# fnothaft/adam

Hardware: AMD Instinct MI355X
Metric: BQSR bases/sec (observe+apply) at 1/2/4/8 MI355X; % HBM roofline (higher is better)
Workload: dtype u8 in, int64 counts, f64 recalibration; 1 GPU; cfg2: synthetic 10M x 100 bp reads, 1 read group, no known sites (per GPU); reads_per_gpu=10000000, bases_per_gpu=1000000000, reads_total=10000000, read_groups=1, known_sites=0, parallelism=dp1: read shards per GPU, RCCL int64 table all-reduce

## Files before the change

adam_amd/_capi.py:

```python
from __future__ import annotations

import ctypes
import os
import threading

_HERE = os.path.dirname(os.path.abspath(__file__))
LIB_PATH = os.environ.get("ADAM_BQSR_LIB") or os.path.join(_HERE, "libadam_bqsr.so")

BQSR_OK = 0
STAGE_RESET, STAGE_KERNEL, STAGE_FOLD, STAGE_PREP, STAGE_LUT, STAGE_NO_LUT = 1, 2, 4, 8, 16, 32
STATUS_NAMES = ["OK", "NULL_RG", "MD_PARSE", "CIGAR_SHORT", "BAD_REVCOMP_BASE", "EMPTY_TABLE", "MISSING_KEY",
                "QUAL_RANGE", "NULL_FIELD", "SEQ_SHORT", "CIGAR_INVALID", "INVALID_ARG", "DEVICE", "UNSUPPORTED",
                "SAM_PARSE", "PILEUP", "ATTRIBUTE"]
(NULL_RG, MD_PARSE, CIGAR_SHORT, BAD_REVCOMP_BASE, EMPTY_TABLE, MISSING_KEY, QUAL_RANGE, NULL_FIELD, SEQ_SHORT,
 CIGAR_INVALID, INVALID_ARG, DEVICE, UNSUPPORTED, SAM_PARSE, PILEUP, ATTRIBUTE) = range(1, 17)

EXPORTS = [
    "bqsr_abi_version", "bqsr_last_error", "bqsr_last_error_read", "bqsr_status_name", "bqsr_context_create",
    "bqsr_context_destroy", "bqsr_context_tune", "bqsr_sites_create", "bqsr_sites_destroy", "bqsr_batch_create", "bqsr_batch_destroy",
    "bqsr_batch_reads", "bqsr_batch_bases", "bqsr_batch_dims", "bqsr_batch_relayout", "bqsr_batch_layout_times", "bqsr_batch_wrap_device", "bqsr_table_words",
    "bqsr_table_create", "bqsr_table_destroy", "bqsr_table_dims", "bqsr_table_device_ptr", "bqsr_table_download",
    "bqsr_table_upload", "bqsr_observe", "bqsr_observe_records", "bqsr_table_merge", "bqsr_finalize",
    "bqsr_lut_destroy", "bqsr_lut_stats", "bqsr_lut_shifts", "bqsr_apply", "bqsr_apply_records",
    "bqsr_stage_records", "bqsr_staged_destroy", "bqsr_staged_bytes", "bqsr_staged_reads", "bqsr_staged_bases",
    "bqsr_batch_create_staged", "bqsr_batch_upload_async", "bqsr_em_fold_async", "bqsr_batch_em_copy_async",
    "bqsr_finalize_device", "bqsr_observe_stage", "bqsr_apply_stage", "bqsr_job_reset_async", "bqsr_job_result", "bqsr_copy_async",
    "bqsr_job_errors_export_async", "bqsr_job_errors_import_async", "bqsr_job_status_async", "bqsr_job_status_get",
    "bqsr_copy_dyn_async", "bqsr_compact_outputs_async", "bqsr_batch_exception_count_ptr",
    "bqsr_sort_order", "bqsr_sam_sort",
    "bqsr_sam_flagstat", "bqsr_flagstat_arrow", "bqsr_flagstat_arrow_device",
    "bqsr_bgzf_inflate", "bqsr_sam_bam_form", "bqsr_sam_markdup_path",
    "bqsr_sam_pileup_prepare", "bqsr_sam_pileup_columns", "bqsr_arrow_pileup_prepare", "bqsr_arrow_pileup_columns",
    "bqsr_pileup_kernel_times",
    "bqsr_pileup_agg_create", "bqsr_pileup_agg_destroy", "bqsr_pileup_agg_add_host", "bqsr_sam_pileup_agg_add",
    "bqsr_arrow_pileup_agg_add", "bqsr_pileup_agg_run", "bqsr_pileup_agg_fetch", "bqsr_pileup_agg_kernel_times",
    "bqsr_sam_bam_prepare", "bqsr_sam_bam_records", "bqsr_sam_bam_header", "bqsr_bgzf_compress",
    "bqsr_bam_kernel_times",
    "bqsr_bgzf_deflate", "bqsr_bgzf_deflate_host", "bqsr_sam_bam_members", "bqsr_deflate_code_lengths",
    "bqsr_bgzf_deflate_times",
    "bqsr_compare_create", "bqsr_compare_destroy", "bqsr_compare_check_terms", "bqsr_compare_sam", "bqsr_compare_sides",
    "bqsr_compare_values", "bqsr_compare_baseqs", "bqsr_compare_rows", "bqsr_compare_kernel_times",
    "bqsr_sam_tag_counts", "bqsr_arrow_tag_counts", "bqsr_sam_tag_values", "bqsr_arrow_tag_values",
    "bqsr_tag_values_fetch", "bqsr_tags_kernel_times",
]


class NativeLibraryMissing(RuntimeError):
    pass


class BQSRError(RuntimeError):

    def __init__(self, status: int, message: str = "", read: int = -1):
        name = STATUS_NAMES[status] if 0 <= status < len(STATUS_NAMES) else str(status)
        super().__init__("%s: %s" % (name, message))
        self.status = status
        self.name = name
        self.read = read


class Dims(ctypes.Structure):
    _fields_ = [("n_rg", ctypes.c_int32), ("max_len", ctypes.c_int32)]


class FinalStats(ctypes.Structure):
    _fields_ = [("average_reported_error", ctypes.c_double), ("global_error", ctypes.c_double),
                ("global_obs", ctypes.c_int64), ("global_mm", ctypes.c_int64), ("n_groups", ctypes.c_int32)]


class DeviceReads(ctypes.Structure):
    _fields_ = [("n_reads", ctypes.c_int64), ("n_slots", ctypes.c_int64), ("meta", ctypes.c_void_p),
                ("align", ctypes.c_void_p), ("qual", ctypes.c_void_p), ("bases", ctypes.c_void_p),
                ("cigar", ctypes.c_void_p), ("md", ctypes.c_void_p), ("dims", Dims),
                ("slots_aligned", ctypes.c_int32)]


_lib = None
_lock = threading.Lock()


def lib():
    global _lib
    if _lib is not None:
        return _lib
    with _lock:
        if _lib is not None:
            return _lib
        if not os.path.exists(LIB_PATH):
            raise NativeLibraryMissing("%s is not built; run __graft_entry__.build()" % LIB_PATH)
        try:
            import torch
            if torch.cuda.is_available():
                torch.cuda.init()
        except ImportError:
            pass
        L = ctypes.CDLL(LIB_PATH)
        vp, i32, i64, dbl = ctypes.c_void_p, ctypes.c_int32, ctypes.c_int64, ctypes.c_double
        pp = ctypes.POINTER(ctypes.c_void_p)
        sig = {
            "bqsr_abi_version": (ctypes.c_int, []),
            "bqsr_last_error": (ctypes.c_char_p, []),
            "bqsr_last_error_read": (i64, []),
            "bqsr_status_name": (ctypes.c_char_p, [ctypes.c_int]),
            "bqsr_context_create": (ctypes.c_int, [ctypes.c_int, pp]),
            "bqsr_context_destroy": (None, [vp]),
            "bqsr_context_tune": (ctypes.c_int, [vp, ctypes.c_int, i64]),
            "bqsr_batch_relayout": (ctypes.c_int, [vp, vp, ctypes.POINTER(dbl)]),
            "bqsr_batch_layout_times": (ctypes.c_int, [vp, ctypes.POINTER(dbl), ctypes.POINTER(dbl)]),
            "bqsr_sites_create": (ctypes.c_int, [vp, vp, vp, vp, i32, pp]),
            "bqsr_sites_destroy": (None, [vp]),
            "bqsr_batch_create": (ctypes.c_int, [vp, vp, vp, pp]),
            "bqsr_batch_destroy": (None, [vp]),
            "bqsr_batch_reads": (i64, [vp]),
            "bqsr_batch_bases": (i64, [vp]),
            "bqsr_batch_slots": (i64, [vp]),
            "bqsr_batch_dims": (Dims, [vp]),
            "bqsr_batch_wrap_device": (ctypes.c_int, [vp, ctypes.POINTER(DeviceReads), pp]),
            "bqsr_stage_records": (ctypes.c_int, [vp, vp, pp]),
            "bqsr_staged_destroy": (None, [vp]),
            "bqsr_staged_bytes": (i64, [vp]),
            "bqsr_staged_reads": (i64, [vp]),
            "bqsr_staged_bases": (i64, [vp]),
            "bqsr_batch_create_staged": (ctypes.c_int, [vp, vp, pp]),
            "bqsr_batch_upload_async": (ctypes.c_int, [vp, vp, vp]),
            "bqsr_batch_set_window": (ctypes.c_int, [vp, i32, i32]),
            "bqsr_batch_reads_per_tile": (i32, [vp]),
            "bqsr_table_words": (i64, [Dims]),
            "bqsr_table_create": (ctypes.c_int, [vp, Dims, vp, pp]),
            "bqsr_table_destroy": (None, [vp]),
            "bqsr_table_dims": (Dims, [vp]),
            "bqsr_table_device_ptr": (vp, [vp]),
            "bqsr_table_download": (ctypes.c_int, [vp, vp]),
            "bqsr_table_upload": (ctypes.c_int, [vp, vp]),
            "bqsr_observe": (ctypes.c_int, [vp, vp, vp, vp, ctypes.POINTER(dbl), vp]),
            "bqsr_observe_async": (ctypes.c_int, [vp, vp, vp, vp, vp]),
            "bqsr_observe_result": (ctypes.c_int, [vp, ctypes.POINTER(dbl), vp]),
            "bqsr_observe_stage": (ctypes.c_int, [vp, vp, vp, vp, i32, vp]),
            "bqsr_table_zero_async": (ctypes.c_int, [vp, vp]),
            "bqsr_batch_em_device_ptr": (vp, [vp]),
            "bqsr_apply_stage": (ctypes.c_int, [vp, vp, vp, vp, vp, vp, vp, i64, i32, vp]),
            "bqsr_observe_records": (ctypes.c_int, [vp, vp, vp, Dims, pp, ctypes.POINTER(dbl)]),
            "bqsr_table_merge": (ctypes.c_int, [vp, vp, ctypes.POINTER(dbl), dbl]),
            "bqsr_finalize": (ctypes.c_int, [vp, vp, dbl, pp]),
            "bqsr_finalize_async": (ctypes.c_int, [vp, vp, dbl, pp, vp]),
            "bqsr_finalize_result": (ctypes.c_int, [vp, vp]),
            "bqsr_finalize_device": (ctypes.c_int, [vp, vp, vp, pp, vp]),
            "bqsr_batch_em_copy_async": (ctypes.c_int, [vp, vp, vp]),
            "bqsr_em_fold_async": (ctypes.c_int, [vp, vp, i64, vp, vp]),
            "bqsr_lut_destroy": (None, [vp]),
            "bqsr_lut_stats": (ctypes.c_int, [vp, ctypes.POINTER(FinalStats)]),
            "bqsr_lut_group": (ctypes.c_int, [vp, i32, ctypes.POINTER(i64), ctypes.POINTER(i64)]),
            "bqsr_lut_shifts": (ctypes.c_int, [vp, i32, i32, i32, i32, vp, ctypes.POINTER(i32)]),
            "bqsr_phred_threshold_table": (i32, [vp, i32, ctypes.POINTER(i32)]),
            "bqsr_apply": (ctypes.c_int, [vp, vp, vp, vp, vp, vp, vp, i64, ctypes.POINTER(i64), vp]),
            "bqsr_apply_async": (ctypes.c_int, [vp, vp, vp, vp, vp, vp, vp, i64, vp]),
            "bqsr_apply_result": (ctypes.c_int, [vp, ctypes.POINTER(i64), vp]),
            "bqsr_apply_records": (ctypes.c_int, [vp, vp, vp, vp, vp]),
            "bqsr_job_reset_async": (ctypes.c_int, [vp, vp, vp]),
            "bqsr_job_result": (ctypes.c_int, [vp, vp, ctypes.POINTER(dbl), ctypes.POINTER(i64), vp]),
            "bqsr_copy_async": (ctypes.c_int, [vp, vp, vp, i64, vp]),
            "bqsr_copy_dyn_async": (ctypes.c_int, [vp, vp, vp, vp, i32, i64, i64, vp]),
            "bqsr_compact_outputs_async": (ctypes.c_int, [vp, vp, vp, vp, vp, vp, i64, vp, vp, vp, vp]),
            "bqsr_batch_exception_count_ptr": (vp, [vp]),
            "bqsr_job_errors_export_async": (ctypes.c_int, [vp, i64, vp, vp]),
            "bqsr_job_errors_import_async": (ctypes.c_int, [vp, vp, vp]),
            "bqsr_job_status_async": (ctypes.c_int, [vp, vp, i32, vp]),
            "bqsr_job_status_get": (ctypes.c_int, [vp, i32, i32, ctypes.POINTER(dbl), ctypes.POINTER(i64)]),
        }
        for name, (res, args) in sig.items():
            f = getattr(L, name)
            f.restype = res
            f.argtypes = args
        _lib = L
    return _lib


def check(status: int):
    if status != BQSR_OK:
        L = lib()
        raise BQSRError(status, L.bqsr_last_error().decode(), L.bqsr_last_error_read())
```

adam_amd/bqsr.py:

```python
from __future__ import annotations

import contextlib
import ctypes
from typing import Dict, Iterable, List, Optional, Sequence, Tuple

import numpy as np

from . import _capi
from ._capi import BQSRError, Dims, check, lib
from .records import (F_DUPLICATE, F_HAS_MD, F_MAPPED, F_PRIMARY, ADAMRecord, RecordBatch)

MAX_REASONABLE_QSCORE = 60


class Context:

    _by_device: Dict[int, "Context"] = {}

    def __init__(self, device: int = 0):
        h = ctypes.c_void_p()
        check(lib().bqsr_context_create(device, ctypes.byref(h)))
        self.handle = h
        self.device = device

    @classmethod
    def get(cls, device: int = 0) -> "Context":
        if device not in cls._by_device:
            cls._by_device[device] = Context(device)
        return cls._by_device[device]

    _KNOBS = {"order": 1, "fronts": 2, "key_major": 3, "bgzf": 5, "flagstat_grid": 6, "pileup_grid": 7}
    _DEFAULTS = {"order": -1, "fronts": -1, "key_major": 0, "bgzf": 1, "flagstat_grid": 0, "pileup_grid": 0}

    def tune(self, **knobs) -> Dict[str, int]:
        cur = getattr(self, "_tuned", dict(self._DEFAULTS))
        prev = {}
        for k, v in knobs.items():
            if v is None:
                continue
            if isinstance(v, str):
                v = {"auto": -1, "read": 0, "group": 1}[v]
            check(lib().bqsr_context_tune(self.handle, self._KNOBS[k], int(v)))
            prev[k] = cur[k]
            cur[k] = int(v)
        self._tuned = cur
        return prev

    @contextlib.contextmanager
    def tuned(self, **knobs):
        prev = self.tune(**knobs)
        try:
            yield self
        finally:
            self.tune(**prev)


class SnpTable:

    def __init__(self, table: Optional[Dict[str, Iterable[int]]] = None):
        self.table = {k: np.unique(np.asarray(list(v), dtype=np.int64)) for k, v in (table or {}).items()}
        self._handles: Dict[int, ctypes.c_void_p] = {}

    @property
    def contigs(self) -> List[str]:
        return list(self.table.keys())

    @staticmethod
    def from_vcf(path: str) -> "SnpTable":
        t: Dict[str, List[int]] = {}
        with open(path, "r", encoding="latin-1") as fh:
            for line in fh:
                line = line.rstrip("\n")
                if line.startswith("#"):
                    continue
                f = line.split("\t")
                t.setdefault(f[0], []).append(int(f[1]))
        return SnpTable(t)

    def handle(self, ctx: Context):
        if ctx.device not in self._handles:
            names = [c.encode() for c in self.contigs]
            arrs = [np.ascontiguousarray(self.table[c]) for c in self.contigs]
            n = len(arrs)
            cnames = (ctypes.c_char_p * max(1, n))(*names)
            cpos = (ctypes.c_void_p * max(1, n))(*[a.ctypes.data for a in arrs])
            cn = np.asarray([len(a) for a in arrs] or [0], dtype=np.uint64)
            h = ctypes.c_void_p()
            check(lib().bqsr_sites_create(ctx.handle, ctypes.cast(cnames, ctypes.c_void_p),
                                          ctypes.cast(cpos, ctypes.c_void_p), cn.ctypes.data, n, ctypes.byref(h)))
            self._handles[ctx.device] = h
        return self._handles[ctx.device]

    def __del__(self):
        L = _capi._lib
        if L is not None:
            for h in getattr(self, "_handles", {}).values():
                L.bqsr_sites_destroy(h)


def dims_of(batches: Sequence[RecordBatch]) -> Dims:
    n_rg = max([b.n_rg() for b in batches] or [1])
    max_len = max([b.max_len() for b in batches] or [1])
    return Dims(n_rg, max_len)


class ErrorCount:

    def __init__(self, bases_observed: int = 0, mismatches: int = 0):
        self.bases_observed = int(bases_observed)
        self.mismatches = int(mismatches)

    def __add__(self, other: "ErrorCount") -> "ErrorCount":
        return ErrorCount(self.bases_observed + other.bases_observed, self.mismatches + other.mismatches)

    def get_error_prob(self) -> Optional[float]:
        if self.bases_observed == 0:
            return None
        return max(10.0 ** (-60 / 10.0), self.mismatches / self.bases_observed)

    def __repr__(self):
        return "ErrorCount(%d, %d)" % (self.bases_observed, self.mismatches)


class RecalTable:

    def __init__(self, dims: Dims, ctx: Optional[Context] = None, expected_mismatch: float = 0.0):
        self.ctx = ctx or Context.get()
        self.dims = Dims(dims.n_rg, dims.max_len)
        h = ctypes.c_void_p()
        check(lib().bqsr_table_create(self.ctx.handle, self.dims, None, ctypes.byref(h)))
        self.handle = h
        self.expected_mismatch = float(expected_mismatch)

    def __del__(self):
        L = _capi._lib
        if L is not None and getattr(self, "handle", None):
            L.bqsr_table_destroy(self.handle)
            self.handle = None

    @property
    def K(self) -> int:
        return 60 * (self.dims.n_rg - 1) + 128

    @property
    def C(self) -> int:
        return 2 * self.dims.max_len + 1

    @property
    def cells(self) -> int:
        return self.C + 21

    def words(self) -> np.ndarray:
        w = np.zeros(lib().bqsr_table_words(self.dims), dtype=np.int64)
        check(lib().bqsr_table_download(self.handle, w.ctypes.data))
        return w

    def set_words(self, w: np.ndarray):
        w = np.ascontiguousarray(w, dtype=np.int64)
        check(lib().bqsr_table_upload(self.handle, w.ctypes.data))

    def counts(self) -> Tuple[np.ndarray, np.ndarray, np.ndarray]:
        w = self.words()
        K, cells = self.K, self.cells
        return w[:K], w[K:K + K * cells].reshape(K, cells), w[K + K * cells:].reshape(K, cells)

    def merge(self, other: "RecalTable") -> "RecalTable":
        out = RecalTable(self.dims, self.ctx)
        out.set_words(self.words())
        em = ctypes.c_double(self.expected_mismatch)
        check(lib().bqsr_table_merge(out.handle, other.handle, ctypes.byref(em), other.expected_mismatch))
        out.expected_mismatch = em.value
        return out

    def merge_into(self, other: "RecalTable"):
        em = ctypes.c_double(self.expected_mismatch)
        check(lib().bqsr_table_merge(self.handle, other.handle, ctypes.byref(em), other.expected_mismatch))
        self.expected_mismatch = em.value

    def finalize_table(self) -> "FinalizedTable":
        return FinalizedTable(self)


class FinalizedTable:

    def __init__(self, table: RecalTable):
        self.table = table
        h = ctypes.c_void_p()
        check(lib().bqsr_finalize(table.ctx.handle, table.handle, table.expected_mismatch, ctypes.byref(h)))
        self.handle = h
        st = _capi.FinalStats()
        check(lib().bqsr_lut_stats(h, ctypes.byref(st)))
        self.average_reported_error = st.average_reported_error
        self.global_error = st.global_error
        self.global_counts = ErrorCount(st.global_obs, st.global_mm)

    def __del__(self):
        L = _capi._lib
        if L is not None and getattr(self, "handle", None):
            L.bqsr_lut_destroy(self.handle)
            self.handle = None

    def read_group_counts(self, r: int) -> Optional[ErrorCount]:
        o, m = ctypes.c_int64(), ctypes.c_int64()
        k = lib().bqsr_lut_group(self.handle, r, ctypes.byref(o), ctypes.byref(m))
        if k < 0:
            check(_capi.DEVICE)
        return ErrorCount(o.value, m.value) if k == 1 else None

    def get_error_rate_shifts(self, qual_by_rg: int, qual: int, cycle: int, context: int):
        sh = np.zeros(4, dtype=np.float64)
        q = ctypes.c_int32()
        check(lib().bqsr_lut_shifts(self.handle, qual_by_rg, qual, cycle, context, sh.ctypes.data, ctypes.byref(q)))
        return sh, q.value

    def get_read_group_delta(self, qual_by_rg: int) -> float:
        num = qual_by_rg - 1
        r = num // MAX_REASONABLE_QSCORE if num >= 0 else -((-num) // MAX_REASONABLE_QSCORE)
        ec = self.read_group_counts(r)
        if ec is None:
            raise BQSRError(_capi.MISSING_KEY, "read group %d" % r)
        p = ec.get_error_prob()
        avg = self.average_reported_error
        return (p if p is not None else avg) - avg


class Partition:

    def __init__(self, batch: RecordBatch, chars: np.ndarray, out_len: np.ndarray):
        self.batch = batch
        self.chars = chars
        self.out_len = out_len

    def qual(self, r: int) -> str:
        o = int(self.batch.qual_offset[r])
        return "".join(map(chr, self.chars[o:o + int(self.out_len[r])]))

    def records(self) -> List[ADAMRecord]:
        recs = self.batch.to_records()
        for r, rec in enumerate(recs):
            if rec.qual is not None or self.out_len[r]:
                rec.qual = self.qual(r)
        return recs


class RecalibrateBaseQualities:

    def __init__(self, ctx: Optional[Context] = None, dims: Optional[Dims] = None):
        self.ctx = ctx or Context.get()
        self.dims = dims

    @staticmethod
    def usable_read(rec: ADAMRecord) -> bool:
        return rec.read_mapped and rec.primary_alignment and not rec.duplicate_read and \
            rec.mismatching_positions is not None

    @classmethod
    def apply(cls, partitions: Sequence[RecordBatch], dbsnp: Optional[SnpTable] = None,
              ctx: Optional[Context] = None) -> List[Partition]:
        parts = list(partitions)
        rbq = cls(ctx, dims_of(parts))
        table = rbq.compute_table(parts, dbsnp or SnpTable())
        return rbq.apply_table(table, parts)

    def _records(self, batch: RecordBatch, dbsnp: Optional[SnpTable]):
        return batch.c_struct(batch.contig_ids_for(dbsnp.contigs if dbsnp else None))

    def compute_table(self, partitions: Sequence[RecordBatch], dbsnp: SnpTable) -> RecalTable:
        dims = self.dims or dims_of(partitions)
        acc = RecalTable(dims, self.ctx)
        sites = dbsnp.handle(self.ctx) if dbsnp is not None else None
        for batch in partitions:
            s, keep = self._records(batch, dbsnp)
            h = ctypes.c_void_p()
            em = ctypes.c_double(0.0)
            check(lib().bqsr_observe_records(self.ctx.handle, ctypes.byref(s), sites, dims, ctypes.byref(h),
                                             ctypes.byref(em)))
            part = RecalTable.__new__(RecalTable)
            part.ctx, part.dims, part.handle, part.expected_mismatch = self.ctx, dims, h, em.value
            acc.merge_into(part)
        return acc

    def apply_table(self, table: RecalTable, partitions: Sequence[RecordBatch]) -> List[Partition]:
        fin = table.finalize_table()
        out = []
        for batch in partitions:
            s, keep = self._records(batch, None)
            chars = np.zeros(max(1, int(batch.qual_offset[-1])), dtype=np.uint16)
            out_len = np.zeros(max(1, batch.n_reads), dtype=np.uint32)
            check(lib().bqsr_apply_records(self.ctx.handle, ctypes.byref(s), fin.handle, chars.ctypes.data,
                                           out_len.ctypes.data))
            out.append(Partition(batch, chars, out_len))
        return out


def adam_bqsr(partitions: Sequence[RecordBatch], dbsnp: Optional[SnpTable] = None,
              ctx: Optional[Context] = None) -> List[Partition]:
    return RecalibrateBaseQualities.apply(partitions, dbsnp, ctx)
```

adam_amd/csrc/bqsr_capi.cpp:

```cpp
#include <hip/hip_runtime.h>

#include <algorithm>
#include <array>
#include <atomic>
#include <chrono>
#include <cmath>
#include <cstdio>
#include <cstdlib>
#include <cstring>
#include <dlfcn.h>
#include <memory>
#include <mutex>
#include <new>
#include <string>
#include <thread>
#include <vector>

#include <rocprim/rocprim.hpp>

#include "bqsr_internal.h"

using namespace bqsr;

#include "bqsr_kernels.hip"
#include "bqsr_observe_lean.hip"
#include "bqsr_fold.hip"
#include "bqsr_transport.hip"


namespace {
thread_local std::string g_err;
thread_local int64_t g_err_read = -1;

bqsr_status fail(bqsr_status s, const std::string& msg, int64_t read = -1) {
  g_err = msg;
  g_err_read = read;
  return s;
}
bqsr_status ok() {
  g_err.clear();
  g_err_read = -1;
  return BQSR_OK;
}

#define HIP_TRY(expr)                                                                          \
  do {                                                                                         \
    hipError_t e_ = (expr);                                                                    \
    if (e_ != hipSuccess)                                                                      \
      return fail(BQSR_ERR_DEVICE, std::string(#expr " failed: ") + hipGetErrorString(e_));    \
  } while (0)

hipStream_t S(void* s) { return s ? (hipStream_t)s : hipStreamPerThread; }

const char* kStatusNames[] = {"OK",          "NULL_RG",      "MD_PARSE",       "CIGAR_SHORT", "BAD_REVCOMP_BASE",
                              "EMPTY_TABLE", "MISSING_KEY",  "QUAL_RANGE",     "NULL_FIELD",  "SEQ_SHORT",
                              "CIGAR_INVALID", "INVALID_ARG", "DEVICE",        "UNSUPPORTED", "SAM_PARSE",
                              "PILEUP",      "ATTRIBUTE"};

bqsr_status from_err_key(unsigned long long k, int64_t read_base) {
  if (k == kNoError) return ok();
  const int code = (int)(k & 0xF);
  const int64_t read = (int64_t)(k >> 28) + read_base;
  const uint32_t o = (uint32_t)((k >> 8) & 0xFFFFF);
  char buf[160];
  snprintf(buf, sizeof buf, "%s at read %lld, read offset %u", kStatusNames[code], (long long)read, o);
  return fail((bqsr_status)code, buf, read);
}


struct Pow10 {
  double v[256];
  Pow10() {
    for (int p = 0; p < 256; ++p) v[p] = std::pow(10.0, (double)(-p) / 10.0);
  }
};
const Pow10& pow10tab() {
  static Pow10 t;
  return t;
}

double cr_log10(double x) { return (double)log10l((long double)x); }
int32_t java_d2i(double d) {
  if (std::isnan(d)) return 0;
  if (d >= 2147483647.0) return INT32_MAX;
  if (d <= -2147483648.0) return INT32_MIN;
  return (int32_t)d;
}
int32_t phred_of(double p) { return java_d2i(-10.0 * cr_log10(p)); }

struct PhredThresholds {
  std::vector<double> thr;
  PhredThresholds() {
    thr.resize(kThrN);
    const uint64_t lo_bits = 1, hi_bits = 0x7FEFFFFFFFFFFFFFull;
    auto val = [](uint64_t b) {
      double d;
      memcpy(&d, &b, 8);
      return d;
    };
    for (int i = 0; i < kThrN; ++i) {
      const int n = kThrQmin + i;
      if (phred_of(val(hi_bits)) >= n) {
        thr[i] = val(hi_bits);
        continue;
      }
      if (phred_of(val(lo_bits)) < n) {
        thr[i] = 0.0;
        continue;
      }
      uint64_t a = lo_bits, b = hi_bits;
      while (b - a > 1) {
        const uint64_t m = a + (b - a) / 2;
        if (phred_of(val(m)) >= n) a = m; else b = m;
      }
      thr[i] = val(a);
    }
  }
};
const PhredThresholds& thresholds() {
  static PhredThresholds t;
  return t;
}

struct PhredBuckets {
  std::vector<double> thr;
  std::vector<int16_t> q;
  PhredBuckets() {
    thr.resize(kQbN);
    q.resize(kQbN);
    const auto& T = thresholds().thr;
    for (int i = 0; i < kQbN; ++i) {
      const int e = kQbElo + (i >> kQbBits), m = i & ((1 << kQbBits) - 1);
      const double lo = std::ldexp(1.0 + (double)m / (1 << kQbBits), e);
      const double hi = std::ldexp(1.0 + (double)(m + 1) / (1 << kQbBits), e);
      const double last = std::nextafter(hi, 0.0);
      const int qhi = phred_of(lo), qlo = phred_of(last);
      if (qhi - qlo > 1 || qhi - kThrQmin < 0 || qhi - kThrQmin >= kThrN || qhi > 32767 || qhi < -32767) {
        q[(size_t)i] = -32768;
        thr[(size_t)i] = 0.0;
      } else {
        q[(size_t)i] = (int16_t)qhi;
        thr[(size_t)i] = T[(size_t)(qhi - kThrQmin)];
      }
    }
  }
};
const PhredBuckets& buckets() {
  static PhredBuckets b;
  return b;
}

int64_t table_words(const bqsr_dims& d) {
  const int64_t K = 60LL * (d.n_rg - 1) + 128, cells = 2LL * d.max_len + 1 + kCtxSlots;
  return K + 2 * K * cells;
}
TableGeom geom(const bqsr_dims& d) {
  TableGeom g;
  g.K = 60 * (d.n_rg - 1) + 128;
  g.L = d.max_len;
  g.C = 2 * d.max_len + 1;
  g.cells = g.C + kCtxSlots;
  return g;
}

constexpr size_t kLdsMax = 163840;
size_t observe_lds(int qw, int wcells, bool table) {
  return (table ? (size_t)kCtxTabBytes : 0) + (size_t)qw * wcells * 8 + (size_t)qw * 4 + kQBins * 4 +
         (size_t)kMkWords * 4;
}
int64_t piece_bytes(int qw, int cw) { return ((int64_t)qw * cw * kCtxSlots + 15) & ~(int64_t)15; }
size_t apply_lds(int qw, int cw) { return 16 + (size_t)kMkWords * 4 + kCtxTabBytes + (size_t)piece_bytes(qw, cw); }
int lean_orow(int nc, int cw) {
  int o = nc * (cw + kCtxCells);
  while ((o & 3) != 2) ++o;
  return o;
}
size_t lean_lds(int qw, int orow, int wcells) { return ((size_t)qw * (orow + wcells) + qw + kQBins + 1) * 4; }
constexpr int kLeanCopiesMax = 4;
int observe_rows(int wcells, bool table) {
  int qw = kQBins;
  while (qw > 1 && observe_lds(qw, wcells, table) > kLdsMax) --qw;
  return qw;
}
constexpr bool align_slots() { return true; }
int fronts(int n_base, int n_cu, int64_t n_reads, int forced) {
  if (forced == 0) return 0;
  int f = forced;
  if (f < 0) {
    if (n_base > 4 * n_cu) return 0;
    f = (int)std::min<int64_t>((8 * n_cu + n_base - 1) / n_base, n_reads / (8192 * (int64_t)n_base));
    if ((int64_t)std::max(f, 1) * n_base < n_cu) return 0;
    f = std::max(f, 1);
  }
  while (f > 1 && (int64_t)f * n_base > 4096) --f;
  return f;
}
int apply_rows(int cw) {
  int qw = kQBins;
  while (qw > 1 && apply_lds(qw, cw) > kLdsMax) --qw;
  return qw;
}

}


struct bqsr_context {
  int device = 0;
  int n_cu = 256;
  double* d_pow10 = nullptr;
  double* d_thr = nullptr;
  double* d_qbt = nullptr;
  int16_t* d_qbq = nullptr;
  std::mutex stage_mu;
  uint8_t* stage[2] = {nullptr, nullptr};
  hipEvent_t stage_ev[2] = {nullptr, nullptr};
  int tune_order = -1;
  int tune_fronts = -1;
  int tune_keymajor = 0;
  int tune_bgzf = 1;
  int tune_flagstat_grid = 0;
  int tune_pileup_grid = 0;
  std::mutex flagstat_mu;
  unsigned long long* d_flagstat = nullptr;
};

namespace {
constexpr size_t kStageChunk = 64ull << 20;
bqsr_status stage_ring(bqsr_context* ctx) {
  for (int i = 0; i < 2; ++i) {
    if (!ctx->stage[i]) HIP_TRY(hipHostMalloc((void**)&ctx->stage[i], kStageChunk, hipHostMallocDefault));
    if (!ctx->stage_ev[i]) HIP_TRY(hipEventCreateWithFlags(&ctx->stage_ev[i], hipEventDisableTiming));
  }
  return BQSR_OK;
}
bqsr_status upload_staged(bqsr_context* ctx, void* dst, const void* src, size_t n, hipStream_t s) {
  hipPointerAttribute_t attr{};
  const bool pinned = hipPointerGetAttributes(&attr, src) == hipSuccess && attr.type == hipMemoryTypeHost;
  (void)hipGetLastError();
  if (pinned || n < 2 * kStageChunk) {
    HIP_TRY(hipMemcpyAsync(dst, src, n, hipMemcpyHostToDevice, s));
    HIP_TRY(hipStreamSynchronize(s));
    return BQSR_OK;
  }
  std::lock_guard<std::mutex> lock(ctx->stage_mu);
  bqsr_status st = stage_ring(ctx);
  if (st != BQSR_OK) return st;
  const int nth = (int)std::max(1u, std::min(8u, std::thread::hardware_concurrency()));
  const uint8_t* p = (const uint8_t*)src;
  uint8_t* d = (uint8_t*)dst;
  int k = 0;
  for (size_t off = 0; off < n; off += kStageChunk, k ^= 1) {
    const size_t len = std::min(kStageChunk, n - off);
    HIP_TRY(hipEventSynchronize(ctx->stage_ev[k]));
    std::vector<std::thread> th;
    for (int t = 0; t < nth; ++t)
      th.emplace_back([&, t] {
        const size_t a = len * (size_t)t / (size_t)nth, b = len * (size_t)(t + 1) / (size_t)nth;
        memcpy(ctx->stage[k] + a, p + off + a, b - a);
      });
    for (auto& x : th) x.join();
    HIP_TRY(hipMemcpyAsync(d + off, ctx->stage[k], len, hipMemcpyHostToDevice, s));
    HIP_TRY(hipEventRecord(ctx->stage_ev[k], s));
  }
  HIP_TRY(hipStreamSynchronize(s));
  return BQSR_OK;
}
}

struct bqsr_sites {
  bqsr_context* ctx = nullptr;
  std::vector<std::string> names;
  int64_t* pos = nullptr;
  uint64_t* off = nullptr;
  uint32_t* bucket = nullptr;
  uint64_t* bucket_off = nullptr;
  int64_t* bucket_base = nullptr;
  uint64_t* bm = nullptr;
  uint64_t* bm_off = nullptr;
  int64_t* bm_base = nullptr;
  int32_t n = 0;
  int32_t shift = 8;
  SitesDev dev() const { return SitesDev{pos, off, bucket, bucket_off, bucket_base, bm, bm_off, bm_base, n, shift}; }
};

struct bqsr_batch {
  bqsr_context* ctx = nullptr;
  bool owned = false;
  ReadsDev rd{};
  bqsr_dims dims{1, 1};
  int64_t n_slots = 0;
  int64_t n_bases = 0;
  int32_t q_lo = 0, rg_lo = 0;
  bool have_qhist = false;
  int64_t qhist[kQBins] = {0};
  int64_t qhigh = 0;
  std::vector<void*> allocs;
  std::vector<size_t> staged_cnt;
  const bqsr_staged* staged_src = nullptr;
  uint8_t* d_bases2 = nullptr;
  uint64_t* d_bexc = nullptr;
  uint64_t* d_qcodes = nullptr;
  uint8_t* d_qbase = nullptr;
  uint64_t* d_qexc = nullptr;
  ReadInfo* d_info = nullptr;
  uint64_t* d_sbits = nullptr;
  uint32_t* d_work = nullptr;
  int64_t sbits_words = 0;
  bool err_fresh = false;
  bool prepped = false;
  const bqsr_sites* prep_sites = nullptr;
  uint32_t* d_hq = nullptr;
  uint32_t* d_qmask = nullptr;
  bool hq_valid = false;
  FoldParams fold{};
  uint32_t* d_part = nullptr;
  size_t part_words = 0;
  uint8_t* d_chars = nullptr;
  const bqsr_lut* chars_lut = nullptr;
  uint64_t* d_off64 = nullptr;
  int64_t off64_n = -1;
  size_t chars_bytes = 0;
  unsigned long long* d_err = nullptr;
  double* d_em = nullptr;
  int32_t n_blocks = 0;
  bool bucketed = false;
  int32_t n_keys = 1;
  int32_t n_base = 1;
  int32_t fronts = 0;
  uint32_t* d_perm = nullptr;
  int64_t* d_key_off = nullptr;
  uint32_t* d_key_cnt = nullptr;
  uint32_t* d_cursor = nullptr;
  uint8_t *k_qual = nullptr, *k_bases = nullptr;
  uint64_t* d_kslot = nullptr;
  uint64_t* d_kspan = nullptr;
  void* d_ktemp = nullptr;
  size_t ktemp_bytes = 0;
  bool km_ready = false;
  double km_alloc_ms = -1.0, km_build_ms = -1.0;
  bool perm_static = false;
  OrderDev order() const {
    return bucketed ? OrderDev{d_perm, d_key_off, n_keys, fronts > 0 ? n_base : 0, km_ready ? d_kslot : nullptr}
                    : OrderDev{nullptr, nullptr, 1};
  }
  ReadsDev pass_rd() const {
    ReadsDev r = rd;
    if (bucketed && km_ready) {
      r.qual = k_qual;
      r.bases = k_bases;
    }
    return r;
  }
  int32_t pass_blocks() const { return bucketed && fronts > 0 ? n_keys : n_blocks; }
  uint64_t* h_status = nullptr;
  hipStream_t side = nullptr;
  hipEvent_t ev_obs = nullptr, ev_fold = nullptr;
  bool obs_pending = false;
  ~bqsr_batch() {
    if (side) (void)hipStreamDestroy(side);
    for (hipEvent_t e : {ev_obs, ev_fold})
      if (e) (void)hipEventDestroy(e);
    if (d_part) (void)hipFree(d_part);
    if (d_off64) (void)hipFree(d_off64);
    if (d_chars) (void)hipFree(d_chars);
    if (h_status) (void)hipHostFree(h_status);
    for (void* p : allocs) (void)hipFree(p);
  }
};

struct bqsr_table {
  bqsr_context* ctx = nullptr;
  bqsr_dims dims{1, 1};
  int64_t* words = nullptr;
  bool owned = false;
  ~bqsr_table() {
    if (owned && words) (void)hipFree(words);
  }
  TableGeom g() const { return geom(dims); }
  int64_t* touched() const { return words; }
  int64_t* obs() const { return words + g().K; }
  int64_t* mm() const { return words + g().K + (int64_t)g().K * g().cells; }
};

struct bqsr_lut {
  bqsr_context* ctx = nullptr;
  bqsr_dims dims{1, 1};
  int32_t n_groups = 0;
  std::vector<void*> allocs;
  int64_t *qk_obs = nullptr, *qk_mm = nullptr, *grp_obs = nullptr, *grp_mm = nullptr;
  uint8_t *grp_ok = nullptr, *key_ok = nullptr, *rq_ok = nullptr;
  double *a2 = nullptr, *s1 = nullptr, *d2 = nullptr;
  FinalOut* d_out = nullptr;
  FinalOut out{};
  bool out_pending = false;
  bool host_ready = false;
  std::vector<int64_t> h_words, h_qk_obs, h_qk_mm, h_grp_obs, h_grp_mm;
  std::vector<uint8_t> h_grp_ok;
  const bqsr_table* src = nullptr;
  ~bqsr_lut() {
    for (void* p : allocs) (void)hipFree(p);
  }
};

namespace {
template <class T>
bqsr_status dalloc(std::vector<void*>& v, T** p, size_t n) {
  void* q = nullptr;
  HIP_TRY(hipMalloc(&q, std::max<size_t>(n, 1) * sizeof(T)));
  v.push_back(q);
  *p = (T*)q;
  return BQSR_OK;
}
}


extern "C" {

int bqsr_abi_version(void) { return BQSR_ABI_VERSION; }
const char* bqsr_last_error(void) { return g_err.c_str(); }
int64_t bqsr_last_error_read(void) { return g_err_read; }
const char* bqsr_status_name(bqsr_status s) {
  if ((int)s < 0 || (int)s > 16) return "UNKNOWN";
  return kStatusNames[(int)s];
}

bqsr_status bqsr_context_tune(bqsr_context* ctx, int knob, int64_t value) {
  if (!ctx) return fail(BQSR_ERR_INVALID_ARG, "bqsr_context_tune: null context");
  switch (knob) {
    case BQSR_TUNE_ORDER:
      if (value < -1 || value > 1) break;
      ctx->tune_order = (int)value;
      return BQSR_OK;
    case BQSR_TUNE_FRONTS:
      if (value < -1 || value > 4096) break;
      ctx->tune_fronts = (int)value;
      return BQSR_OK;
    case BQSR_TUNE_KEYMAJOR:
      if (value < 0 || value > 1) break;
      ctx->tune_keymajor = (int)value;
      return BQSR_OK;
    case BQSR_TUNE_FUSED_PREP:
      if (value != 0) break;
      return BQSR_OK;
    case BQSR_TUNE_BGZF:
      if (value < 0 || value > 1) break;
      ctx->tune_bgzf = (int)value;
      return BQSR_OK;
    case BQSR_TUNE_FLAGSTAT_GRID:
      if (value < 0 || value > (1 << 20)) break;
      ctx->tune_flagstat_grid = (int)value;
      return BQSR_OK;
    case BQSR_TUNE_PILEUP_GRID:
      if (value < 0 || value > (1 << 20)) break;
      ctx->tune_pileup_grid = (int)value;
      return BQSR_OK;
    default:
      return fail(BQSR_ERR_INVALID_ARG, "bqsr_context_tune: unknown knob");
  }
  return fail(BQSR_ERR_INVALID_ARG, "bqsr_context_tune: value out of range");
}

bqsr_status bqsr_context_create(int device, bqsr_context** out) {
  if (!out) return fail(BQSR_ERR_INVALID_ARG, "null out");
  HIP_TRY(hipSetDevice(device));
  hipDeviceProp_t prop;
  HIP_TRY(hipGetDeviceProperties(&prop, device));
  bqsr_context* c = new bqsr_context;
  c->device = device;
  c->n_cu = prop.multiProcessorCount;
  hipError_t e = hipMalloc(&c->d_pow10, 256 * sizeof(double));
  if (e == hipSuccess) e = hipMalloc(&c->d_thr, kThrN * sizeof(double));
  if (e == hipSuccess) e = hipMemcpy(c->d_pow10, pow10tab().v, 256 * sizeof(double), hipMemcpyHostToDevice);
  if (e == hipSuccess) e = hipMemcpy(c->d_thr, thresholds().thr.data(), kThrN * sizeof(double), hipMemcpyHostToDevice);
  if (e == hipSuccess) e = hipMalloc(&c->d_qbt, kQbN * sizeof(double));
  if (e == hipSuccess) e = hipMalloc(&c->d_qbq, kQbN * sizeof(int16_t));
  if (e == hipSuccess) e = hipMemcpy(c->d_qbt, buckets().thr.data(), kQbN * sizeof(double), hipMemcpyHostToDevice);
  if (e == hipSuccess) e = hipMemcpy(c->d_qbq, buckets().q.data(), kQbN * sizeof(int16_t), hipMemcpyHostToDevice);
  for (const void* f : {(const void*)bqsr_apply_kernel, (const void*)bqsr_observe_chunks,
                        (const void*)bqsr_observe_lean<true, false>, (const void*)bqsr_observe_lean<true, true>})
    if (e == hipSuccess) e = hipFuncSetAttribute(f, hipFuncAttributeMaxDynamicSharedMemorySize, (int)kLdsMax);
  if (e == hipSuccess)
    e = hipFuncSetAttribute((const void*)bqsr_fold_hist, hipFuncAttributeMaxDynamicSharedMemorySize, (int)fold_hist_lds());
  if (e == hipSuccess)
    e = hipFuncSetAttribute((const void*)bqsr_fold_chain, hipFuncAttributeMaxDynamicSharedMemorySize,
                            (int)chain_lds(kMaxFoldBlocks));
  if (e != hipSuccess) {
    bqsr_context_destroy(c);
    return fail(BQSR_ERR_DEVICE, std::string("context: ") + hipGetErrorString(e));
  }
  *out = c;
  return ok();
}

void bqsr_context_destroy(bqsr_context* c) {
  if (!c) return;
  if (c->d_pow10) (void)hipFree(c->d_pow10);
  if (c->d_thr) (void)hipFree(c->d_thr);
  if (c->d_qbt) (void)hipFree(c->d_qbt);
  if (c->d_qbq) (void)hipFree(c->d_qbq);
  if (c->d_flagstat) (void)hipFree(c->d_flagstat);
  for (int i = 0; i < 2; ++i) {
    if (c->stage[i]) (void)hipHostFree(c->stage[i]);
    if (c->stage_ev[i]) (void)hipEventDestroy(c->stage_ev[i]);
  }
  delete c;
}


bqsr_status bqsr_sites_create(bqsr_context* ctx, const char* const* contigs, const int64_t* const* pos,
                              const uint64_t* n, int32_t n_contigs, bqsr_sites** out) {
  if (!ctx || !out || n_contigs < 0 || (n_contigs > 0 && (!contigs || !pos || !n)))
    return fail(BQSR_ERR_INVALID_ARG, "bqsr_sites_create: bad arguments");
  HIP_TRY(hipSetDevice(ctx->device));
  bqsr_sites* s = new bqsr_sites;
  s->ctx = ctx;
  s->n = n_contigs;
  std::vector<int64_t> all;
  std::vector<uint64_t> off(1, 0);
  std::vector<uint32_t> bucket;
  std::vector<uint64_t> boff(1, 0);
  std::vector<int64_t> bbase;
  std::vector<uint64_t> bm, bmoff(1, 0);
  std::vector<int64_t> bmbase;
  for (int32_t c = 0; c < n_contigs; ++c) {
    s->names.emplace_back(contigs[c] ? contigs[c] : "");
    std::vector<int64_t> v(pos[c], pos[c] + n[c]);
    std::sort(v.begin(), v.end());
    v.erase(std::unique(v.begin(), v.end()), v.end());
    const int64_t base = v.empty() ? 0 : v.front();
    const int64_t nb = v.empty() ? 0 : ((v.back() - base) >> s->shift) + 1;
    size_t j = 0;
    for (int64_t b = 0; b < nb; ++b) {
      const int64_t lo = base + (b << s->shift);
      while (j < v.size() && v[j] < lo) ++j;
      bucket.push_back((uint32_t)j);
    }
    bbase.push_back(base);
    boff.push_back(bucket.size());
    const int64_t b0 = v.empty() ? 0 : (int64_t)((uint64_t)base & ~(uint64_t)63);
    const int64_t nw = v.empty() ? 0 : ((v.back() - b0) >> 6) + 1;
    const bool dense = nw > 0 && nw <= 64 * (int64_t)v.size() + 64 && nw <= (int64_t(1) << 28);
    if (dense) {
      const size_t w0 = bm.size();
      bm.resize(w0 + (size_t)nw, 0ull);
      for (const int64_t p : v) bm[w0 + (size_t)((p - b0) >> 6)] |= 1ull << ((p - b0) & 63);
    }
    bmbase.push_back(dense ? b0 : 0);
    bmoff.push_back(bm.size());
    all.insert(all.end(), v.begin(), v.end());
    off.push_back(all.size());
  }
  std::vector<void*> keep;
  auto up = [&](auto** dst, const auto& src) -> hipError_t {
    using T = typename std::remove_reference<decltype(src[0])>::type;
    hipError_t e = hipMalloc((void**)dst, std::max<size_t>(src.size(), 1) * sizeof(T));
    if (e != hipSuccess) return e;
    if (!src.empty()) e = hipMemcpy(*dst, src.data(), src.size() * sizeof(T), hipMemcpyHostToDevice);
    return e;
  };
  hipError_t e = up(&s->pos, all);
  if (e == hipSuccess) e = up(&s->off, off);
  if (e == hipSuccess) e = up(&s->bucket, bucket);
  if (e == hipSuccess) e = up(&s->bucket_off, boff);
  if (e == hipSuccess) e = up(&s->bucket_base, bbase);
  if (e == hipSuccess) e = up(&s->bm, bm);
  if (e == hipSuccess) e = up(&s->bm_off, bmoff);
  if (e == hipSuccess) e = up(&s->bm_base, bmbase);
  if (e != hipSuccess) {
    bqsr_sites_destroy(s);
    return fail(BQSR_ERR_DEVICE, std::string("sites upload: ") + hipGetErrorString(e));
  }
  *out = s;
  return ok();
}

void bqsr_sites_destroy(bqsr_sites* s) {
  if (!s) return;
  for (void* p : {(void*)s->pos, (void*)s->off, (void*)s->bucket, (void*)s->bucket_off, (void*)s->bucket_base,
                  (void*)s->bm, (void*)s->bm_off, (void*)s->bm_base})
    if (p) (void)hipFree(p);
  delete s;
}


namespace {

inline uint8_t code_of(uint8_t c) {
  switch (c) {
    case 'A': return kCodeA;
    case 'C': return kCodeC;
    case 'G': return kCodeG;
    case 'T': return kCodeT;
    case 'N': return kCodeN;
    default: return kCodeOther;
  }
}

Window window_rows(const bqsr_batch* b, int max_rows);

bqsr_status finish_batch(bqsr_batch* b, int64_t max_slot_len) {
  if (max_slot_len > kMaxReadLen)
    return fail(BQSR_ERR_UNSUPPORTED, "reads longer than " + std::to_string(kMaxReadLen) + " bases are not supported");
  const int64_t n = b->rd.n_reads;
  b->rd.reads_per_tile = (int32_t)std::max<int64_t>(1, std::min<int64_t>(kMaxTileReads, kTileSlots / std::max<int64_t>(1, max_slot_len)));
  b->rd.n_tiles = (n + b->rd.reads_per_tile - 1) / b->rd.reads_per_tile;
  b->n_blocks = std::min(b->ctx->n_cu, kMaxFoldBlocks);
  bqsr_status st;
  if ((st = dalloc(b->allocs, &b->d_hq, (size_t)b->n_blocks * kQBins)) != BQSR_OK) return st;
  if ((st = dalloc(b->allocs, &b->d_qmask, 4)) != BQSR_OK) return st;
  {
    FoldParams& F = b->fold;
    const size_t nt = (size_t)std::max<int64_t>(1, b->rd.n_tiles), nbk = (size_t)b->n_blocks;
    F.stream_cap = std::max<int64_t>(1 << 20, std::min<int64_t>(16 << 20, b->rd.n_slots));
    if ((st = dalloc(b->allocs, &F.blk, nbk)) != BQSR_OK || (st = dalloc(b->allocs, &F.cand_list, nbk)) != BQSR_OK ||
        (st = dalloc(b->allocs, &F.n_cand, 1)) != BQSR_OK || (st = dalloc(b->allocs, &F.delta, 1)) != BQSR_OK ||
        (st = dalloc(b->allocs, &F.rtile, nt)) != BQSR_OK || (st = dalloc(b->allocs, &F.ntile, nt)) != BQSR_OK ||
        (st = dalloc(b->allocs, &F.dtile, nt * kSegBinades)) != BQSR_OK ||
        (st = dalloc(b->allocs, &F.seg, nbk * kFoldMaxSegs)) != BQSR_OK ||
        (st = dalloc(b->allocs, &F.seg_base, nbk)) != BQSR_OK || (st = dalloc(b->allocs, &F.nseg, nbk)) != BQSR_OK ||
        (st = dalloc(b->allocs, &F.seg_used, 1)) != BQSR_OK ||
        (st = dalloc(b->allocs, &F.streams, (size_t)F.stream_cap + 64)) != BQSR_OK ||
        (st = dalloc(b->allocs, &F.csum, (size_t)F.stream_cap / 64 * 2 + 2)) != BQSR_OK ||
        (st = dalloc(b->allocs, &F.stream_used, 1)) != BQSR_OK)
      return st;
  }
  if ((st = dalloc(b->allocs, &b->d_err, kErrWords)) != BQSR_OK) return st;
  if ((st = dalloc(b->allocs, &b->d_info, (size_t)std::max<int64_t>(1, n))) != BQSR_OK) return st;
  b->sbits_words = b->rd.slots_aligned ? (b->rd.n_slots / 16 + 8 + 1) / 2 : b->rd.n_slots / 32 + 5;
  if ((st = dalloc(b->allocs, &b->d_sbits, (size_t)b->sbits_words)) != BQSR_OK) return st;
  if ((st = dalloc(b->allocs, &b->d_em, 2)) != BQSR_OK) return st;
  if ((st = dalloc(b->allocs, &b->d_work,
                   (size_t)(n + kPrepChunk) + (size_t)std::max<int64_t>(n / kPrepChunk + 1, kMaxFoldBlocks))) != BQSR_OK)
    return st;
  if (b->ctx->tune_order >= 0) {
    b->bucketed = b->ctx->tune_order == 1;
  } else {
    b->bucketed = b->dims.n_rg > 1;
    if (!b->bucketed && b->have_qhist) {
      const int cw = geom(b->dims).C;
      const Window w = window_rows(b, apply_rows(cw));
      int64_t in = 0, all = 0;
      for (int q = 0; q < kQBins; ++q) {
        all += b->qhist[q];
        if (q >= w.q_lo && q < w.q_lo + w.qw) in += b->qhist[q];
      }
      b->bucketed = (double)(all - in) > 1e-3 * (double)all;
    }
  }
  if (b->bucketed) {
    b->n_base = 2 * std::max<int32_t>(1, b->dims.n_rg);
    b->fronts = fronts(b->n_base, b->ctx->n_cu, n, b->ctx->tune_fronts);
    b->n_keys = b->n_base * std::max(1, b->fronts);
    if ((st = dalloc(b->allocs, &b->d_perm, (size_t)std::max<int64_t>(1, n))) != BQSR_OK) return st;
    if ((st = dalloc(b->allocs, &b->d_key_off, (size_t)b->n_keys + 1)) != BQSR_OK) return st;
    if ((st = dalloc(b->allocs, &b->d_key_cnt, (size_t)b->n_keys)) != BQSR_OK) return st;
    if ((st = dalloc(b->allocs, &b->d_cursor, (size_t)b->n_keys)) != BQSR_OK) return st;
  }
  return BQSR_OK;
}

bool layout_wanted(const bqsr_batch* b) { return b->bucketed && b->rd.slots_aligned && b->rd.n_reads > 0; }
bool key_major_wanted(const bqsr_batch* b) { return layout_wanted(b) && b->ctx->tune_keymajor; }
bqsr_status key_major_alloc(bqsr_batch* b) {
  if (b->k_qual) return BQSR_OK;
  const int64_t n = b->rd.n_reads;
  bqsr_status st;
  size_t tb = 0;
  HIP_TRY(rocprim::exclusive_scan(nullptr, tb, (const uint64_t*)nullptr, (uint64_t*)nullptr, (uint64_t)0, (size_t)n + 1,
                                  rocprim::plus<uint64_t>(), (hipStream_t)0));
  b->ktemp_bytes = std::max<size_t>(tb, 1);
  if ((st = dalloc(b->allocs, &b->d_kslot, (size_t)(n + 1))) != BQSR_OK ||
      (st = dalloc(b->allocs, &b->d_kspan, (size_t)(n + 1))) != BQSR_OK ||
      (st = dalloc(b->allocs, (uint8_t**)&b->d_ktemp, b->ktemp_bytes)) != BQSR_OK ||
      (st = dalloc(b->allocs, &b->k_qual, (size_t)b->rd.n_slots + kColumnPad)) != BQSR_OK ||
      (st = dalloc(b->allocs, &b->k_bases, (size_t)b->rd.n_slots / 2 + 1 + kColumnPad)) != BQSR_OK)
    return st;
  return BQSR_OK;
}
void launch_key_sort(bqsr_batch* b, uint64_t* span, hipStream_t s) {
  const int64_t n = b->rd.n_reads;
  const int n_cu = b->ctx->n_cu;
  (void)hipMemsetAsync(b->d_key_cnt, 0, (size_t)b->n_keys * 4, s);
  const unsigned cb = (unsigned)std::min<int64_t>((n + 255) / 256, (int64_t)n_cu * 4);
  hipLaunchKernelGGL(bqsr_key_count, dim3(cb), dim3(256), 0, s, (const ReadMeta*)b->rd.meta, n, b->n_keys, b->n_base,
                     std::max(1, b->fronts), b->d_key_cnt);
  hipLaunchKernelGGL(bqsr_key_scan, dim3(1), dim3(1024), 0, s, (const uint32_t*)b->d_key_cnt, b->n_keys, b->d_key_off,
                     b->d_cursor);
  const unsigned sb = (unsigned)std::min<int64_t>((n + 4095) / 4096, (int64_t)n_cu * 8);
  hipLaunchKernelGGL(bqsr_key_scatter, dim3(sb), dim3(256), 0, s, (const ReadMeta*)b->rd.meta, n, b->n_keys, b->n_base,
                     std::max(1, b->fronts), b->d_cursor, b->d_perm, span);
}
bqsr_status layout_build(bqsr_batch* b, hipStream_t s) {
  if (!layout_wanted(b)) return BQSR_OK;
  const int64_t n = b->rd.n_reads;
  bqsr_context* ctx = b->ctx;
  const bool km = key_major_wanted(b);
  b->km_ready = false;
  const auto t0 = std::chrono::steady_clock::now();
  bqsr_status st = km ? key_major_alloc(b) : BQSR_OK;
  if (st != BQSR_OK) return st;
  const auto t1 = std::chrono::steady_clock::now();
  if (km) HIP_TRY(hipMemsetAsync(b->d_kspan + n, 0, 8, s));
  launch_key_sort(b, km ? b->d_kspan : nullptr, s);
  HIP_TRY(hipGetLastError());
  if (km) {
    size_t tb = b->ktemp_bytes;
    HIP_TRY(rocprim::exclusive_scan(b->d_ktemp, tb, b->d_kspan, b->d_kslot, (uint64_t)0, (size_t)n + 1,
                                    rocprim::plus<uint64_t>(), s));
    HIP_TRY(hipMemsetAsync(b->k_qual + b->rd.n_slots, 0, kColumnPad, s));
    HIP_TRY(hipMemsetAsync(b->k_bases + b->rd.n_slots / 2, 0, 1 + kColumnPad, s));
    const unsigned gw = (unsigned)std::min<int64_t>((n + 16 * kKmPer - 1) / (16 * kKmPer), (int64_t)ctx->n_cu * 64 / kKmPer);
    hipLaunchKernelGGL(bqsr_km_gather, dim3(gw), dim3(256), 0, s, b->rd, (const uint32_t*)b->d_perm,
                       (const uint64_t*)b->d_kslot, b->k_qual, b->k_bases);
    HIP_TRY(hipGetLastError());
  }
  HIP_TRY(hipStreamSynchronize(s));
  const auto t2 = std::chrono::steady_clock::now();
  b->km_alloc_ms = std::chrono::duration<double, std::milli>(t1 - t0).count();
  b->km_build_ms = std::chrono::duration<double, std::milli>(t2 - t1).count();
  b->km_ready = km;
  b->perm_static = true;
  return BQSR_OK;
}

struct Packed {
  std::vector<ReadMeta> meta;
  std::vector<ReadAlign> align;
  std::vector<uint8_t> qual, bases, md;
  std::vector<uint32_t> cigar;
  int64_t n_slots = 0, n_bases = 0, max_slot = 0;
  int32_t n_rg = 1, max_len = 1;
  int64_t qhist[256] = {0};
  std::vector<int64_t> rghist;
};

bqsr_status pack(const bqsr_records* R, Packed& P) {
  const int64_t n = R->n_reads;
  P.meta.resize((size_t)n);
  P.align.resize((size_t)n);
  uint64_t slot = 0, md_tot = 0, cig_tot = 0;
  for (int64_t r = 0; r < n; ++r) {
    const uint32_t f = R->flags[r];
    const uint64_t lq = (f & BQSR_F_HAS_QUAL) ? R->qual_offset[r + 1] - R->qual_offset[r] : 0;
    const uint64_t ls = (f & BQSR_F_HAS_SEQ) ? R->seq_offset[r + 1] - R->seq_offset[r] : 0;
    const uint64_t nmd = (f & BQSR_F_HAS_MD) ? R->md_offset[r + 1] - R->md_offset[r] : 0;
    const uint64_t ncig = (f & BQSR_F_HAS_CIGAR) ? R->cigar_offset[r + 1] - R->cigar_offset[r] : 0;
    if (lq > 65535 || ls > 65535 || nmd > 65535 || ncig > 65535)
      return fail(BQSR_ERR_UNSUPPORTED, "read field longer than 65535", r);
    if ((f & BQSR_F_HAS_RG) && (R->rg_id[r] < 0 || R->rg_id[r] > 65535))
      return fail(BQSR_ERR_UNSUPPORTED, "recordGroupId outside [0, 65535]", r);
    ReadMeta& m = P.meta[(size_t)r];
    m.slot = slot;
    m.lq = (uint16_t)lq;
    m.ls = (uint16_t)ls;
    m.flags = (uint16_t)(f & 0x7FFF);
    m.rg = (f & BQSR_F_HAS_RG) ? (uint16_t)R->rg_id[r] : 0;
    ReadAlign& a = P.align[(size_t)r];
    a.start = R->start[r];
    a.cigar_off = (uint32_t)cig_tot;
    a.md_off = (uint32_t)md_tot;
    a.contig = R->contig_id[r];
    a.n_cigar = (uint16_t)ncig;
    a.md_len = (uint16_t)nmd;
    const uint64_t sl = align_slots() ? slot_span(lq, ls) : std::max(lq, ls);
    slot += sl;
    P.max_slot = std::max<int64_t>(P.max_slot, (int64_t)sl);
    md_tot += nmd;
    cig_tot += ncig;
    P.n_bases += (int64_t)(R->seq_offset[r + 1] - R->seq_offset[r]);
    if (f & BQSR_F_HAS_RG) P.n_rg = std::max<int32_t>(P.n_rg, R->rg_id[r] + 1);
    P.max_len = std::max<int32_t>(P.max_len, (int32_t)ls);
  }
  if (md_tot > 0xFFFFFFFFull || cig_tot > 0xFFFFFFFFull)
    return fail(BQSR_ERR_UNSUPPORTED, "partition MD / CIGAR columns exceed 4 GiB");
  P.n_slots = (int64_t)slot;
  P.qual.assign((size_t)slot + kColumnPad, 0);
  P.bases.assign((size_t)slot / 2 + 1 + kColumnPad, 0);
  P.md.resize(md_tot + kColumnPad);
  P.cigar.resize(cig_tot + kColumnPad / 4);
  P.rghist.assign((size_t)P.n_rg, 0);
  const int nth = (int)std::max<int64_t>(1, std::min<int64_t>(16, n / 65536));
  std::vector<std::thread> th;
  std::vector<std::array<int64_t, 256>> qh((size_t)nth);
  for (auto& h : qh) h.fill(0);
  auto work = [&](int t) {
    const int64_t r0 = n * t / nth, r1 = n * (t + 1) / nth;
    for (int64_t r = r0; r < r1; ++r) {
      const ReadMeta& m = P.meta[(size_t)r];
      const ReadAlign& a = P.align[(size_t)r];
      const uint8_t* q = R->qual + R->qual_offset[r];
      for (uint32_t i = 0; i < m.lq; ++i) {
        const uint8_t v = (uint8_t)(q[i] - 33);
        P.qual[m.slot + i] = v;
        qh[(size_t)t][v]++;
      }
      const uint8_t* s = R->seq + R->seq_offset[r];
      bool other = false;
      for (uint32_t i = 0; i < m.ls; ++i) {
        const uint8_t c = code_of(s[i]);
        other |= c == kCodeOther;
        const uint64_t k = m.slot + i;
        if (k & 1) __atomic_fetch_or(&P.bases[k >> 1], (uint8_t)(c << 4), __ATOMIC_RELAXED);
        else __atomic_fetch_or(&P.bases[k >> 1], c, __ATOMIC_RELAXED);
      }
      if (other) P.meta[(size_t)r].flags |= kSeqOther;
      if (m.flags & BQSR_F_HAS_MD) memcpy(&P.md[a.md_off], R->md + R->md_offset[r], a.md_len);
      if (m.flags & BQSR_F_HAS_CIGAR) memcpy(&P.cigar[a.cigar_off], R->cigar + R->cigar_offset[r], a.n_cigar * 4u);
    }
  };
  for (int t = 0; t < nth; ++t) th.emplace_back(work, t);
  for (auto& x : th) x.join();
  for (auto& h : qh)
    for (int i = 0; i < 256; ++i) P.qhist[i] += h[(size_t)i];
  for (int64_t r = 0; r < n; ++r)
    if (P.meta[(size_t)r].flags & BQSR_F_HAS_RG) P.rghist[P.meta[(size_t)r].rg]++;
  return BQSR_OK;
}

int32_t best_q_lo(const int64_t* qhist, int qw) {
  int best = 0;
  int64_t bestv = -1;
  for (int lo = 0; lo + 1 <= kQBins; ++lo) {
    int64_t v = 0;
    for (int q = lo; q < std::min(kQBins, lo + qw); ++q) v += qhist[q];
    if (v > bestv) {
      bestv = v;
      best = lo;
    }
    if (lo + qw >= kQBins) break;
  }
  return best;
}

}

bqsr_status bqsr_batch_create(bqsr_context* ctx, const bqsr_records* R, void* stream, bqsr_batch** out) {
  if (!ctx || !R || !out || R->n_reads < 0) return fail(BQSR_ERR_INVALID_ARG, "bqsr_batch_create: bad arguments");
  HIP_TRY(hipSetDevice(ctx->device));
  Packed P;
  bqsr_status st = pack(R, P);
  if (st != BQSR_OK) return st;
  bqsr_batch* b = new bqsr_batch;
  b->ctx = ctx;
  b->owned = true;
  b->rd.n_reads = R->n_reads;
  b->rd.n_slots = P.n_slots;
  b->n_slots = P.n_slots;
  b->n_bases = P.n_bases;
  b->dims = bqsr_dims{P.n_rg, P.max_len};
  int32_t rg_lo = 0;
  for (int32_t i = 0; i < (int32_t)P.rghist.size(); ++i)
    if (P.rghist[(size_t)i] > P.rghist[(size_t)rg_lo]) rg_lo = i;
  b->rg_lo = rg_lo;
  b->q_lo = best_q_lo(P.qhist, 40);
  b->have_qhist = true;
  for (int q = 0; q < kQBins; ++q) b->qhist[q] = P.qhist[q];
  for (int q = kQBins; q < 256; ++q) b->qhigh += P.qhist[q];
  ReadMeta* meta;
  ReadAlign* align;
  uint8_t *qual, *bases, *md;
  uint32_t* cigar;
  hipStream_t s = S(stream);
  auto up = [&](auto** dst, const auto& v) -> bqsr_status {
    using T = typename std::remove_reference<decltype(v[0])>::type;
    bqsr_status x = dalloc(b->allocs, dst, v.size());
    if (x != BQSR_OK) return x;
    if (!v.empty()) HIP_TRY(hipMemcpyAsync(*dst, v.data(), v.size() * sizeof(T), hipMemcpyHostToDevice, s));
    return BQSR_OK;
  };
  if ((st = up(&meta, P.meta)) != BQSR_OK || (st = up(&align, P.align)) != BQSR_OK || (st = up(&qual, P.qual)) != BQSR_OK ||
      (st = up(&bases, P.bases)) != BQSR_OK || (st = up(&md, P.md)) != BQSR_OK || (st = up(&cigar, P.cigar)) != BQSR_OK) {
    delete b;
    return st;
  }
  b->rd.meta = meta;
  b->rd.align = align;
  b->rd.qual = qual;
  b->rd.bases = bases;
  b->rd.md = md;
  b->rd.cigar = cigar;
  b->rd.slots_aligned = align_slots();
  if ((st = finish_batch(b, P.max_slot)) != BQSR_OK || (st = layout_build(b, s)) != BQSR_OK) {
    delete b;
    return st;
  }
  hipError_t e = hipStreamSynchronize(s);
  if (e != hipSuccess) {
    delete b;
    return fail(BQSR_ERR_DEVICE, hipGetErrorString(e));
  }
  *out = b;
  return ok();
}

constexpr int kStagedCols = 11;
constexpr uint32_t kQCodeZero = 15u, kQCodeExc = 14u;
static void encode_qual_chunk(const uint8_t* q, int n, uint64_t slot0, uint8_t& base, uint64_t& codes,
                              std::vector<uint64_t>& exc) {
  int mn = 256, mx = -1;
  for (int k = 0; k < n; ++k)
    if (q[k]) {
      mn = std::min(mn, (int)q[k]);
      mx = std::max(mx, (int)q[k]);
    }
  int b = mn + 7;
  if (mx >= 0 && mx - mn > 13) {
    const int cand[3] = {mn, mx - 13, (mn + mx) / 2 - 7};
    int best = -1;
    for (int c : cand) {
      int cnt = 0;
      for (int k = 0; k < n; ++k) cnt += q[k] && q[k] >= c && q[k] <= c + 13;
      if (cnt > best) {
        best = cnt;
        b = c + 7;
      }
    }
  }
  b = std::min(std::max(b, 0), 255);
  uint64_t w = 0;
  for (int k = 0; k < 16; ++k) {
    uint32_t c = kQCodeZero;
    if (k < n && q[k]) {
      const int d = (int)q[k] - b;
      if (d >= -7 && d <= 6) {
        c = (uint32_t)(d + 7);
// ... 203 lines not shown
  bqsr_status st = finish_batch(b, b->rd.slots_aligned ? (int64_t)slot_span(0, (uint64_t)dev->dims.max_len)
                                                       : (int64_t)dev->dims.max_len);
  if (st != BQSR_OK) {
    delete b;
    return st;
  }
  *out = b;
  return ok();
}

void bqsr_batch_destroy(bqsr_batch* b) { delete b; }
int64_t bqsr_batch_reads(const bqsr_batch* b) { return b ? b->rd.n_reads : -1; }
int64_t bqsr_batch_bases(const bqsr_batch* b) { return b ? b->n_bases : -1; }
int64_t bqsr_batch_slots(const bqsr_batch* b) { return b ? b->n_slots : -1; }
bqsr_dims bqsr_batch_dims(const bqsr_batch* b) { return b ? b->dims : bqsr_dims{0, 0}; }

bqsr_status bqsr_batch_relayout(bqsr_batch* b, void* stream, double* ms) {
  if (!b) return fail(BQSR_ERR_INVALID_ARG, "bqsr_batch_relayout: null batch");
  hipStream_t s = (hipStream_t)stream;
  HIP_TRY(hipStreamSynchronize(s));
  const auto t0 = std::chrono::steady_clock::now();
  const bool has = b->perm_static;
  if (has) {
    b->perm_static = false;
    bqsr_status st = layout_build(b, s);
    if (st != BQSR_OK) return st;
  }
  HIP_TRY(hipStreamSynchronize(s));
  if (ms) *ms = has ? std::chrono::duration<double, std::milli>(std::chrono::steady_clock::now() - t0).count() : -1.0;
  return ok();
}

bqsr_status bqsr_batch_layout_times(const bqsr_batch* b, double* alloc_ms, double* build_ms) {
  if (!b) return fail(BQSR_ERR_INVALID_ARG, "bqsr_batch_layout_times: null batch");
  if (alloc_ms) *alloc_ms = b->km_alloc_ms;
  if (build_ms) *build_ms = b->km_build_ms;
  return ok();
}

bqsr_status bqsr_batch_set_window(bqsr_batch* b, int32_t q_lo, int32_t rg_lo) {
  if (!b || q_lo < 0 || q_lo >= kQBins || rg_lo < 0) return fail(BQSR_ERR_INVALID_ARG, "bad window");
  b->q_lo = q_lo;
  b->rg_lo = rg_lo;
  b->have_qhist = false;
  return ok();
}
int32_t bqsr_batch_reads_per_tile(const bqsr_batch* b) { return b ? b->rd.reads_per_tile : -1; }


int64_t bqsr_table_words(bqsr_dims d) { return (d.n_rg < 1 || d.max_len < 1) ? -1 : table_words(d); }

bqsr_status bqsr_table_create(bqsr_context* ctx, bqsr_dims d, void* device_words, bqsr_table** out) {
  if (!ctx || !out || d.n_rg < 1 || d.max_len < 1 || d.max_len > 65535)
    return fail(BQSR_ERR_INVALID_ARG, "bqsr_table_create: bad arguments");
  HIP_TRY(hipSetDevice(ctx->device));
  bqsr_table* t = new bqsr_table;
  t->ctx = ctx;
  t->dims = d;
  const size_t bytes = (size_t)table_words(d) * 8;
  if (device_words) {
    t->words = (int64_t*)device_words;
  } else {
    hipError_t e = hipMalloc((void**)&t->words, bytes);
    if (e != hipSuccess) {
      delete t;
      return fail(BQSR_ERR_DEVICE, hipGetErrorString(e));
    }
    t->owned = true;
  }
  hipError_t e = hipMemset(t->words, 0, bytes);
  if (e != hipSuccess) {
    delete t;
    return fail(BQSR_ERR_DEVICE, hipGetErrorString(e));
  }
  *out = t;
  return ok();
}
void bqsr_table_destroy(bqsr_table* t) { delete t; }
bqsr_dims bqsr_table_dims(const bqsr_table* t) { return t ? t->dims : bqsr_dims{0, 0}; }
void* bqsr_table_device_ptr(bqsr_table* t) { return t ? t->words : nullptr; }

bqsr_status bqsr_table_download(const bqsr_table* t, int64_t* host) {
  if (!t || !host) return fail(BQSR_ERR_INVALID_ARG, "null");
  HIP_TRY(hipSetDevice(t->ctx->device));
  HIP_TRY(hipMemcpy(host, t->words, (size_t)table_words(t->dims) * 8, hipMemcpyDeviceToHost));
  return ok();
}
bqsr_status bqsr_table_upload(bqsr_table* t, const int64_t* host) {
  if (!t || !host) return fail(BQSR_ERR_INVALID_ARG, "null");
  HIP_TRY(hipSetDevice(t->ctx->device));
  HIP_TRY(hipMemcpy(t->words, host, (size_t)table_words(t->dims) * 8, hipMemcpyHostToDevice));
  return ok();
}

bqsr_status bqsr_table_merge(bqsr_table* acc, const bqsr_table* part, double* acc_em, double part_em) {
  if (!acc || !part || !acc_em) return fail(BQSR_ERR_INVALID_ARG, "null");
  if (acc->dims.n_rg != part->dims.n_rg || acc->dims.max_len != part->dims.max_len)
    return fail(BQSR_ERR_INVALID_ARG, "table dims differ");
  HIP_TRY(hipSetDevice(acc->ctx->device));
  const int64_t n = table_words(acc->dims);
  hipLaunchKernelGGL(bqsr_table_add, dim3((unsigned)std::min<int64_t>(4096, (n + 255) / 256)), dim3(256), 0,
                     hipStreamPerThread, acc->words, part->words, n);
  HIP_TRY(hipGetLastError());
  HIP_TRY(hipStreamSynchronize(hipStreamPerThread));
  *acc_em = *acc_em + part_em;
  return ok();
}


namespace {
Window window_rows(const bqsr_batch* b, int max_rows) {
  Window w{max_rows, std::min(b->q_lo, kQBins - 1), b->rg_lo};
  if (!b->have_qhist) {
    w.qw = std::min(w.qw, kQBins - w.q_lo);
    return w;
  }
  int lo = 0, hi = kQBins - 1;
  while (lo < kQBins - 1 && b->qhist[lo] == 0) ++lo;
  while (hi > lo && b->qhist[hi] == 0) --hi;
  if (hi - lo + 1 <= max_rows) {
    w.q_lo = lo;
    w.qw = hi - lo + 1;
  } else {
    w.q_lo = best_q_lo(b->qhist, max_rows);
  }
  w.qw = std::min(w.qw, kQBins - w.q_lo);
  return w;
}
int window_cw(const bqsr_batch* b, const TableGeom& g) { return b->bucketed ? g.L : g.C; }
int qual_span(const bqsr_batch* b) {
  if (!b->have_qhist) return kQBins;
  int lo = 0, hi = kQBins - 1;
  while (lo < kQBins - 1 && b->qhist[lo] == 0) ++lo;
  while (hi > lo && b->qhist[hi] == 0) --hi;
  return hi - lo + 1;
}
int lane_shift(const bqsr_batch* b) {
  const int c = (b->dims.max_len + kSuper - 1) / kSuper;
  int s = 0;
  while ((1 << s) < c && s < 6) ++s;
  return s;
}
bqsr_status check_dims(const bqsr_batch* b, const bqsr_table* t) {
  if (b->dims.n_rg > t->dims.n_rg || b->dims.max_len > t->dims.max_len)
    return fail(BQSR_ERR_INVALID_ARG, "table dims smaller than the batch's (n_rg / max_len)");
  return BQSR_OK;
}
}

namespace {
bqsr_status launch_prep(bqsr_context* ctx, bqsr_batch* b, const bqsr_sites* sites, hipStream_t s) {
  if (!b->err_fresh) HIP_TRY(hipMemsetAsync(b->d_err + kErrAppPrep, 0xFF, 8, s));
  b->err_fresh = false;
  b->hq_valid = false;
  if (b->rd.n_reads > 0) {
    PrepParams P{};
    P.rd = b->rd;
    if (sites) P.sites = sites->dev();
    const bool w32 = b->rd.slots_aligned;
    const bool store = w32 && b->dims.max_len <= 128 && P.sites.n_contigs > 0;
    P.info = b->d_info;
    P.sbits = b->d_sbits;
    P.err = b->d_err;
    P.work = b->d_work;
    P.n_work = b->d_work + b->rd.n_reads + kPrepChunk;
    const int64_t blocks = (b->rd.n_reads + kPrepChunk - 1) / kPrepChunk;
    if (store) {
      hipLaunchKernelGGL(bqsr_prep_kernel<kPrepStore>, dim3((unsigned)blocks), dim3(kPrepThreads), 0, s, P);
      hipLaunchKernelGGL(bqsr_prep_complex, dim3((unsigned)blocks), dim3(kComplexThreads), 0, s, P);
    } else if (w32) {
      hipLaunchKernelGGL(bqsr_prep_kernel<kPrepW32>, dim3((unsigned)blocks), dim3(kPrepThreads), 0, s, P);
    } else {
      hipLaunchKernelGGL(bqsr_prep_kernel<kPrepU64>, dim3((unsigned)blocks), dim3(kPrepThreads), 0, s, P);
    }
    HIP_TRY(hipGetLastError());
    if (b->bucketed && !b->perm_static) {
      launch_key_sort(b, nullptr, s);
      HIP_TRY(hipGetLastError());
    }
  }
  b->prepped = true;
  b->prep_sites = sites;
  return BQSR_OK;
}
}

bqsr_status bqsr_observe_stage(bqsr_context* ctx, bqsr_batch* b, const bqsr_sites* sites, bqsr_table* t,
                               int32_t stages, void* stream) {
  if (!ctx || !b || !t) return fail(BQSR_ERR_INVALID_ARG, "null");
  bqsr_status st = check_dims(b, t);
  if (st != BQSR_OK) return st;
  HIP_TRY(hipSetDevice(ctx->device));
  hipStream_t s = S(stream);
  if (stages & BQSR_STAGE_RESET) HIP_TRY(hipMemsetAsync(b->d_err + kErrObs, 0xFF, 8, s));
  if (stages & BQSR_STAGE_PREP) {
    if ((st = launch_prep(ctx, b, sites, s)) != BQSR_OK) return st;
  }
  if (b->rd.n_reads == 0) {
    if (stages & BQSR_STAGE_FOLD) HIP_TRY(hipMemsetAsync(b->d_em, 0, 8, s));
    return ok();
  }
  if ((stages & BQSR_STAGE_KERNEL) && (!b->prepped || b->prep_sites != sites))
    return fail(BQSR_ERR_INVALID_ARG, "observe kernel before the prep stage (or with other known sites)");
  if (stages & BQSR_STAGE_KERNEL) {
    ObserveParams P{};
    P.rd = b->pass_rd();
    P.ord = b->order();
    P.info = b->d_info;
    P.sbits = b->d_sbits;
    P.g = geom(t->dims);
    const bool lean = !b->bucketed;
    P.wcells = window_cw(b, P.g) + (lean ? kCtxCells : kCtxSlots);
    while ((P.wcells & 3) != 2) ++P.wcells;
    if (lean) {
      const int cw = window_cw(b, P.g), span = qual_span(b);
      int best_rows = 0;
      for (int nc = kLeanCopiesMax; nc >= 1 && best_rows < span; --nc) {
        const int orow = lean_orow(nc, cw);
        int qw = kQBins;
        while (qw > 1 && lean_lds(qw, orow, P.wcells) > kLdsMax) --qw;
        if (qw > best_rows) {
          best_rows = qw;
          P.nc = nc;
          P.orow = orow;
        }
      }
      P.w = window_rows(b, best_rows);
      P.rows_all = b->have_qhist && b->qhigh == 0;
      for (int q = 0; q < kQBins && P.rows_all; ++q)
        if (b->qhist[q] && (q < P.w.q_lo || q >= P.w.q_lo + P.w.qw)) P.rows_all = 0;
    } else {
      P.w = window_rows(b, observe_rows(P.wcells, true));
    }
    P.touched = t->touched();
    P.obs = t->obs();
    P.mm = t->mm();
    P.part_stride = 2 * P.w.qw * P.wcells + P.w.qw;
    if (!lean) {
      if (!b->side) {
        HIP_TRY(hipStreamCreateWithFlags(&b->side, hipStreamNonBlocking));
        HIP_TRY(hipEventCreateWithFlags(&b->ev_obs, hipEventDisableTiming));
        HIP_TRY(hipEventCreateWithFlags(&b->ev_fold, hipEventDisableTiming));
      }
      HIP_TRY(hipEventRecord(b->ev_obs, s));
      b->obs_pending = true;
    }
    const size_t need = (size_t)P.part_stride * (b->pass_blocks() + b->n_keys - 1);
    if (b->part_words < need) {
      if (b->d_part) {
        HIP_TRY(hipStreamSynchronize(s));
        (void)hipFree(b->d_part);
        b->d_part = nullptr;
        b->part_words = 0;
      }
      HIP_TRY(hipMalloc((void**)&b->d_part, need * sizeof(uint32_t)));
      b->part_words = need;
    }
    P.part = b->d_part;
    P.hq_block = b->d_hq;
    P.err = b->d_err + kErrObs;
    P.n_blocks = lean ? b->n_blocks : b->pass_blocks();
    const size_t lds = lean ? lean_lds(P.w.qw, P.orow, P.wcells) : observe_lds(P.w.qw, P.wcells, true);
    if (lean) {
      if (P.rd.slots_aligned)
        hipLaunchKernelGGL((bqsr_observe_lean<true, true>), dim3(P.n_blocks), dim3(kBlockThreads), lds, s, P);
      else
        hipLaunchKernelGGL((bqsr_observe_lean<true, false>), dim3(P.n_blocks), dim3(kBlockThreads), lds, s, P);
    } else {
      hipLaunchKernelGGL(bqsr_observe_chunks, dim3(P.n_blocks), dim3(kBlockThreads), lds, s, P);
    }
    HIP_TRY(hipGetLastError());
    const int rb = (int)std::min<int64_t>(4096, ((int64_t)P.part_stride * (b->bucketed ? b->n_base : 1) + 255) / 256);
    const unsigned ry = b->bucketed ? 1u : (unsigned)((b->n_blocks + kRedSlabs - 1) / kRedSlabs);
    hipLaunchKernelGGL(bqsr_window_reduce, dim3(rb, ry), dim3(256), 0, s, (const uint32_t*)b->d_part, b->rd, P.ord,
                       P.n_blocks, P.part_stride, P.wcells, P.w, P.g, P.touched, P.obs, P.mm, lean ? kCtxJunk : 0);
    HIP_TRY(hipGetLastError());
  }
  if (stages & BQSR_STAGE_FOLD) {
    const hipStream_t caller = s;
    const bool fork = b->obs_pending;
    if (fork) {
      HIP_TRY(hipStreamWaitEvent(b->side, b->ev_obs, 0));
      s = b->side;
      b->obs_pending = false;
    }
    if (b->bucketed) {
      HIP_TRY(hipMemsetAsync(b->d_hq, 0, (size_t)b->n_blocks * kQBins * 4, s));
      hipLaunchKernelGGL(bqsr_fold_hist, dim3(b->n_blocks * kFhSplit), dim3(kFhWaves * 64), fold_hist_lds(), s, b->rd, (const ReadInfo*)b->d_info,
                         b->n_blocks, lane_shift(b), b->d_hq);
      HIP_TRY(hipGetLastError());
    }
    FoldParams F = b->fold;
    F.rd = b->rd;
    F.info = b->d_info;
    F.hq_block = b->d_hq;
    F.pow10 = ctx->d_pow10;
    F.n_blocks = b->n_blocks;
    F.em_out = b->d_em;
    F.qmask = b->d_qmask;
    hipLaunchKernelGGL(bqsr_fold_plan, dim3(1), dim3(1024), 0, s, F);
    const int64_t max_tpb = (b->rd.n_tiles + b->n_blocks - 1) / b->n_blocks + 1;
    hipLaunchKernelGGL(bqsr_fold_tiles, dim3(ctx->n_cu * 4), dim3(kFtWaves * 64), 0, s, F, max_tpb);
    hipLaunchKernelGGL(bqsr_fold_segs, dim3(b->n_blocks), dim3(kSegThreads), 0, s, F);
    hipLaunchKernelGGL(bqsr_fold_chain, dim3(1), dim3(1024), chain_lds(b->n_blocks), s, F);
    HIP_TRY(hipGetLastError());
    b->hq_valid = true;
    if (fork) {
      HIP_TRY(hipEventRecord(b->ev_fold, s));
      HIP_TRY(hipStreamWaitEvent(caller, b->ev_fold, 0));
    }
  }
  return ok();
}

bqsr_status bqsr_observe_async(bqsr_context* ctx, bqsr_batch* b, const bqsr_sites* sites, bqsr_table* t, void* stream) {
  return bqsr_observe_stage(ctx, b, sites, t, BQSR_STAGE_RESET | BQSR_STAGE_PREP | BQSR_STAGE_KERNEL | BQSR_STAGE_FOLD,
                            stream);
}

bqsr_status bqsr_table_zero_async(bqsr_table* t, void* stream) {
  if (!t) return fail(BQSR_ERR_INVALID_ARG, "null");
  HIP_TRY(hipSetDevice(t->ctx->device));
  HIP_TRY(hipMemsetAsync(t->words, 0, (size_t)table_words(t->dims) * 8, S(stream)));
  return ok();
}

void* bqsr_batch_em_device_ptr(bqsr_batch* b) { return b ? (void*)b->d_em : nullptr; }

bqsr_status bqsr_observe_result(bqsr_batch* b, double* em, void* stream) {
  HIP_TRY(hipSetDevice(b->ctx->device));
  hipStream_t s = S(stream);
  unsigned long long err = 0;
  double e = 0;
  HIP_TRY(hipMemcpyAsync(&err, b->d_err + kErrObs, 8, hipMemcpyDeviceToHost, s));
  HIP_TRY(hipMemcpyAsync(&e, b->d_em, 8, hipMemcpyDeviceToHost, s));
  HIP_TRY(hipStreamSynchronize(s));
  if (em) *em = e;
  return from_err_key(err, 0);
}

bqsr_status bqsr_observe(bqsr_context* ctx, bqsr_batch* b, const bqsr_sites* sites, bqsr_table* t,
                         double* expected_mismatch, void* stream) {
  bqsr_status st = bqsr_observe_async(ctx, b, sites, t, stream);
  if (st != BQSR_OK) return st;
  return bqsr_observe_result(b, expected_mismatch, stream);
}

bqsr_status bqsr_observe_records(bqsr_context* ctx, const bqsr_records* recs, const bqsr_sites* sites, bqsr_dims dims,
                                 bqsr_table** out_partial, double* out_em) {
  if (!out_partial || !out_em) return fail(BQSR_ERR_INVALID_ARG, "null out");
  bqsr_batch* b = nullptr;
  bqsr_status st = bqsr_batch_create(ctx, recs, nullptr, &b);
  if (st != BQSR_OK) return st;
  bqsr_table* t = nullptr;
  st = bqsr_table_create(ctx, dims, nullptr, &t);
  if (st == BQSR_OK) st = bqsr_observe(ctx, b, sites, t, out_em, nullptr);
  bqsr_batch_destroy(b);
  if (st != BQSR_OK) {
    bqsr_table_destroy(t);
    return st;
  }
  *out_partial = t;
  return ok();
}


namespace {
bqsr_status finalize_impl(bqsr_context* ctx, const bqsr_table* t, double em, const double* em_dev, bqsr_lut** out,
                          void* stream) {
  if (!ctx || !t || !out) return fail(BQSR_ERR_INVALID_ARG, "null");
  HIP_TRY(hipSetDevice(ctx->device));
  hipStream_t s = S(stream);
  const TableGeom g = geom(t->dims);
  const int n_rg = t->dims.n_rg;
  bqsr_lut* L = *out;
  const bool reuse = L && L->ctx == ctx && L->dims.n_rg == t->dims.n_rg && L->dims.max_len == t->dims.max_len;
  if (L && !reuse) {
    (void)hipStreamSynchronize(s);
    delete L;
    *out = nullptr;
  }
  if (!reuse) L = new bqsr_lut;
  L->ctx = ctx;
  L->dims = t->dims;
  L->src = t;
  L->host_ready = false;
  L->n_groups = (g.K - 1) / kMaxQ + 2;
  bqsr_status st;
  if (!reuse && ((st = dalloc(L->allocs, &L->qk_obs, g.K)) != BQSR_OK || (st = dalloc(L->allocs, &L->qk_mm, g.K)) != BQSR_OK ||
      (st = dalloc(L->allocs, &L->grp_obs, L->n_groups)) != BQSR_OK ||
      (st = dalloc(L->allocs, &L->grp_mm, L->n_groups)) != BQSR_OK ||
      (st = dalloc(L->allocs, &L->grp_ok, L->n_groups)) != BQSR_OK || (st = dalloc(L->allocs, &L->key_ok, g.K)) != BQSR_OK ||
      (st = dalloc(L->allocs, &L->rq_ok, (size_t)n_rg * kQBins)) != BQSR_OK ||
      (st = dalloc(L->allocs, &L->a2, (size_t)n_rg * kQBins)) != BQSR_OK ||
      (st = dalloc(L->allocs, &L->s1, (size_t)n_rg * kQBins * g.C)) != BQSR_OK ||
      (st = dalloc(L->allocs, &L->d2, (size_t)n_rg * kQBins * kCtxSlots)) != BQSR_OK ||
      (st = dalloc(L->allocs, &L->d_out, 1)) != BQSR_OK)) {
    delete L;
    return st;
  }
  hipLaunchKernelGGL(bqsr_final_keys, dim3((g.K + 3) / 4), dim3(256), 0, s, t->touched(), t->obs(), t->mm(), g, L->qk_obs,
                     L->qk_mm);
  hipLaunchKernelGGL(bqsr_final_groups, dim3(1), dim3(256), 0, s, t->touched(), L->qk_obs, L->qk_mm, g, n_rg, em,
                     em_dev, ctx->d_pow10, L->n_groups, L->grp_obs, L->grp_mm, L->grp_ok, L->key_ok, L->a2, L->rq_ok, L->d_out);
  const int64_t ncell = (int64_t)n_rg * kQBins * (g.C + kCtxSlots);
  hipLaunchKernelGGL(bqsr_final_tables, dim3((unsigned)std::min<int64_t>(8192, (ncell + 255) / 256)), dim3(256), 0, s,
                     t->obs(), t->mm(), g, n_rg, L->a2, L->rq_ok, pow10tab().v[kMaxQ], L->s1, L->d2);
  hipError_t e = hipGetLastError();
  L->out_pending = em_dev != nullptr;
  if (e == hipSuccess && !em_dev) e = hipMemcpyAsync(&L->out, L->d_out, sizeof(FinalOut), hipMemcpyDeviceToHost, s);
  if (e != hipSuccess) {
    if (!reuse) delete L;
    return fail(BQSR_ERR_DEVICE, hipGetErrorString(e));
  }
  *out = L;
  return ok();
}
}

bqsr_status bqsr_finalize_async(bqsr_context* ctx, const bqsr_table* t, double em, bqsr_lut** out, void* stream) {
  return finalize_impl(ctx, t, em, nullptr, out, stream);
}

bqsr_status bqsr_finalize_device(bqsr_context* ctx, const bqsr_table* t, const double* em_device, bqsr_lut** out,
                                 void* stream) {
  if (!em_device) return fail(BQSR_ERR_INVALID_ARG, "null em_device");
  return finalize_impl(ctx, t, 0.0, em_device, out, stream);
}

bqsr_status bqsr_em_fold_async(bqsr_context* ctx, const double* ems, int64_t n, double* out, void* stream) {
  if (!ctx || !out || n < 0 || (n > 0 && !ems)) return fail(BQSR_ERR_INVALID_ARG, "bqsr_em_fold_async: bad arguments");
  HIP_TRY(hipSetDevice(ctx->device));
  hipLaunchKernelGGL(bqsr_em_fold, dim3(1), dim3(64), 0, S(stream), ems, n, out);
  HIP_TRY(hipGetLastError());
  return ok();
}

bqsr_status bqsr_batch_em_copy_async(bqsr_batch* b, double* dst, void* stream) {
  if (!b || !dst) return fail(BQSR_ERR_INVALID_ARG, "null");
  HIP_TRY(hipSetDevice(b->ctx->device));
  HIP_TRY(hipMemcpyAsync(dst, b->d_em, sizeof(double), hipMemcpyDeviceToDevice, S(stream)));
  return ok();
}

bqsr_status bqsr_finalize_result(bqsr_lut* L, void* stream) {
  HIP_TRY(hipSetDevice(L->ctx->device));
  HIP_TRY(hipStreamSynchronize(S(stream)));
  if (L->out_pending) {
    HIP_TRY(hipMemcpy(&L->out, L->d_out, sizeof(FinalOut), hipMemcpyDeviceToHost));
    L->out_pending = false;
  }
  if (!L->out.any_key)
    return fail(BQSR_ERR_EMPTY_TABLE, "empty.reduceLeft: no usable base was observed");
  return ok();
}

bqsr_status bqsr_finalize(bqsr_context* ctx, const bqsr_table* t, double em, bqsr_lut** out) {
  if (!out) return fail(BQSR_ERR_INVALID_ARG, "null out");
  bqsr_lut* L = nullptr;
  bqsr_status st = bqsr_finalize_async(ctx, t, em, &L, nullptr);
  if (st != BQSR_OK) return st;
  st = bqsr_finalize_result(L, nullptr);
  if (st != BQSR_OK) {
    delete L;
    return st;
  }
  *out = L;
  return ok();
}

void bqsr_lut_destroy(bqsr_lut* l) { delete l; }

namespace {
bqsr_status lut_host(bqsr_lut* L) {
  if (L->host_ready) return BQSR_OK;
  HIP_TRY(hipSetDevice(L->ctx->device));
  if (L->out_pending) {
    HIP_TRY(hipDeviceSynchronize());
    HIP_TRY(hipMemcpy(&L->out, L->d_out, sizeof(FinalOut), hipMemcpyDeviceToHost));
    L->out_pending = false;
  }
  const TableGeom g = geom(L->dims);
  L->h_words.resize((size_t)table_words(L->dims));
  L->h_qk_obs.resize((size_t)g.K);
  L->h_qk_mm.resize((size_t)g.K);
  L->h_grp_obs.resize((size_t)L->n_groups);
  L->h_grp_mm.resize((size_t)L->n_groups);
  L->h_grp_ok.resize((size_t)L->n_groups);
  HIP_TRY(hipMemcpy(L->h_words.data(), L->src->words, L->h_words.size() * 8, hipMemcpyDeviceToHost));
  HIP_TRY(hipMemcpy(L->h_qk_obs.data(), L->qk_obs, (size_t)g.K * 8, hipMemcpyDeviceToHost));
  HIP_TRY(hipMemcpy(L->h_qk_mm.data(), L->qk_mm, (size_t)g.K * 8, hipMemcpyDeviceToHost));
  HIP_TRY(hipMemcpy(L->h_grp_obs.data(), L->grp_obs, (size_t)L->n_groups * 8, hipMemcpyDeviceToHost));
  HIP_TRY(hipMemcpy(L->h_grp_mm.data(), L->grp_mm, (size_t)L->n_groups * 8, hipMemcpyDeviceToHost));
  HIP_TRY(hipMemcpy(L->h_grp_ok.data(), L->grp_ok, (size_t)L->n_groups, hipMemcpyDeviceToHost));
  L->host_ready = true;
  return BQSR_OK;
}
bool eprob(int64_t obs, int64_t mm, double* v) {
  if (obs == 0) return false;
  const double x = (double)mm / (double)obs;
  *v = std::max(pow10tab().v[kMaxQ], x);
  return true;
}
}

bqsr_status bqsr_lut_stats(const bqsr_lut* lc, bqsr_final_stats* out) {
  bqsr_lut* L = const_cast<bqsr_lut*>(lc);
  if (!L || !out) return fail(BQSR_ERR_INVALID_ARG, "null");
  if (L->out_pending) {
    HIP_TRY(hipDeviceSynchronize());
    HIP_TRY(hipMemcpy(&L->out, L->d_out, sizeof(FinalOut), hipMemcpyDeviceToHost));
    L->out_pending = false;
  }
  out->average_reported_error = L->out.avg;
  out->global_error = L->out.global_error;
  out->global_obs = L->out.g_obs;
  out->global_mm = L->out.g_mm;
  out->n_groups = L->n_groups;
  return ok();
}

int bqsr_lut_group(const bqsr_lut* lc, int32_t r, int64_t* obs, int64_t* mm) {
  bqsr_lut* L = const_cast<bqsr_lut*>(lc);
  if (!L || lut_host(L) != BQSR_OK) return -1;
  if (r + 1 < 0 || r + 1 >= L->n_groups || !L->h_grp_ok[(size_t)(r + 1)]) return 0;
  *obs = L->h_grp_obs[(size_t)(r + 1)];
  *mm = L->h_grp_mm[(size_t)(r + 1)];
  return 1;
}

bqsr_status bqsr_lut_shifts(const bqsr_lut* lc, int32_t key, int32_t qual, int32_t cyc, int32_t ctx, double sh[4],
                            int32_t* new_q) {
  bqsr_lut* L = const_cast<bqsr_lut*>(lc);
  if (!L || !sh || !new_q) return fail(BQSR_ERR_INVALID_ARG, "null");
  bqsr_status st = lut_host(L);
  if (st != BQSR_OK) return st;
  const TableGeom g = geom(L->dims);
  if (cyc < -g.L || cyc > g.L || ctx < -4 || ctx > 16) return fail(BQSR_ERR_INVALID_ARG, "covariate out of range");
  const int64_t r = ((int64_t)key - 1) / kMaxQ;
  if (r + 1 < 0 || r + 1 >= L->n_groups || !L->h_grp_ok[(size_t)(r + 1)])
    return fail(BQSR_ERR_MISSING_KEY, "read group missing");
  const double avg = L->out.avg;
  double v;
  const double rgd = (eprob(L->h_grp_obs[(size_t)(r + 1)], L->h_grp_mm[(size_t)(r + 1)], &v) ? v : avg) - avg;
  if (key < 0 || key >= g.K || L->h_words[(size_t)key] == 0) return fail(BQSR_ERR_MISSING_KEY, "key missing");
  if (qual < 0 || qual > 255) return fail(BQSR_ERR_QUAL_RANGE, "qual out of range");
  const double e = pow10tab().v[qual];
  const double a1 = e + rgd;
  const double qd = (eprob(L->h_qk_obs[(size_t)key], L->h_qk_mm[(size_t)key], &v) ? v : a1) - a1;
  const double a2 = a1 + qd;
  const int64_t* obs = L->h_words.data() + g.K;
  const int64_t* mm = obs + (int64_t)g.K * g.cells;
  const int64_t c1 = (int64_t)key * g.cells + cyc + g.L, c2 = (int64_t)key * g.cells + g.C + ctx + 4;
  const double cd = (eprob(obs[c1], mm[c1], &v) ? v : a2) - a2;
  const double xd = (eprob(obs[c2], mm[c2], &v) ? v : a2) - a2;
  sh[0] = rgd;
  sh[1] = qd;
  sh[2] = cd;
  sh[3] = xd;
  double p = e;
  for (int i = 0; i < 4; ++i) p = p + sh[i];
  *new_q = phred_of(p);
  return ok();
}

int32_t bqsr_phred_threshold_table(double* out, int32_t cap, int32_t* qmin) {
  const auto& t = thresholds().thr;
  if (qmin) *qmin = kThrQmin;
  if (out) memcpy(out, t.data(), sizeof(double) * (size_t)std::min<int32_t>(cap, (int32_t)t.size()));
  return (int32_t)t.size();
}



bqsr_status bqsr_apply_stage(bqsr_context* ctx, bqsr_batch* b, const bqsr_lut* L, uint8_t* out_qual,
                             uint32_t* out_start, uint32_t* out_len, uint64_t* exceptions, int64_t max_exceptions,
                             int32_t stages, void* stream) {
  if (!ctx || !b || !L || !out_qual || !out_start || !out_len) return fail(BQSR_ERR_INVALID_ARG, "null");
  if (b->dims.n_rg > L->dims.n_rg || b->dims.max_len > L->dims.max_len)
    return fail(BQSR_ERR_INVALID_ARG, "table dims smaller than the batch's");
  HIP_TRY(hipSetDevice(ctx->device));
  hipStream_t s = S(stream);
  if (stages & BQSR_STAGE_RESET) {
    HIP_TRY(hipMemsetAsync(b->d_err + kErrAppKern, 0xFF, 8, s));
    HIP_TRY(hipMemsetAsync(b->d_err + kNExc, 0, 8, s));
  }
  if (!b->prepped || (stages & BQSR_STAGE_PREP)) {
    bqsr_status st = launch_prep(ctx, b, nullptr, s);
    if (st != BQSR_OK) return st;
  }
  if (b->rd.n_reads == 0 || !(stages & (BQSR_STAGE_KERNEL | BQSR_STAGE_LUT))) return ok();
  ApplyParams P{};
  P.rd = b->pass_rd();
  P.ord = b->order();
  P.info = b->d_info;
  P.g = geom(L->dims);
  const int cw = window_cw(b, P.g);
  P.w = window_rows(b, apply_rows(cw));
  P.n_rg = L->dims.n_rg;
  P.s1 = L->s1;
  P.d2 = L->d2;
  P.rq_ok = L->rq_ok;
  P.key_ok = L->key_ok;
  P.grp_ok = L->grp_ok;
  P.n_groups = L->n_groups;
  P.thr = ctx->d_thr;
  P.thr_qmin = kThrQmin;
// ... 307 lines not shown
```

adam_amd/csrc/bqsr_fold.hip:

```cpp

namespace bqsr {

constexpr double kFoldSeqLimit = 0.0625;
constexpr double kTwo53 = 9007199254740992.0;
constexpr int kChainLdsSegs = 384;
constexpr int kSegThreads = 1024, kSegWaves = kSegThreads / 64;
constexpr int kChainLdsStream = 80 * 1024;
constexpr size_t chain_lds(int n_blocks) {
  return kChainLdsStream + 64 + (size_t)kChainLdsStream / 64 * 2 * sizeof(double) + (size_t)kChainLdsSegs * sizeof(FoldSeg) +
         (size_t)n_blocks * sizeof(FoldBlock);
}

__device__ __forceinline__ int expo(double x) {
  return (int)(((uint64_t)__double_as_longlong(x) >> 52) & 0x7FF) - 1023;
}
__device__ __forceinline__ double pow2i(int k) { return __longlong_as_double((long long)(1023 + k) << 52); }

__device__ __forceinline__ double fold_inc(double t, int e, bool* tie) {
  const double x = t * pow2i(52 - e);
  const double r = rint(x);
  *tie = (x - floor(x)) == 0.5;
  return r;
}

__device__ __forceinline__ int block_eb0(const FoldBlock& B, double delta) {
  return expo(fmax(B.r0 * (1.0 - delta), kFoldSeqLimit));
}
__device__ __forceinline__ int block_nbin(const FoldBlock& B, double delta) {
  return min(expo(fmax(B.r1 * (1.0 + delta), kFoldSeqLimit)) - block_eb0(B, delta) + 1, kSegBinades);
}

extern "C" __global__ void __launch_bounds__(1024) bqsr_fold_plan(FoldParams P) {
  __shared__ double t[kQBins];
  __shared__ double sre[kMaxFoldBlocks];
  __shared__ int64_t scn[kMaxFoldBlocks];
  __shared__ double pre[kMaxFoldBlocks];
  __shared__ int32_t cnd[kMaxFoldBlocks];
  __shared__ double wsum[16];
  __shared__ int64_t wcnt[16];
  __shared__ int32_t wc[16];
  __shared__ uint32_t qm[4];
  const int tid = threadIdx.x, lane = tid & 63, wave = tid >> 6;
  for (int q = tid; q < kQBins; q += 1024) t[q] = P.pow10[q];
  if (tid < 4) qm[tid] = 0;
  __syncthreads();
  const int nb = P.n_blocks;
  for (int b0 = 0; b0 < nb; b0 += 256) {
    const int b = b0 + (tid >> 2), part = tid & 3;
    double re = 0.0;
    int64_t n = 0;
    if (b < nb) {
      const uint4* row = (const uint4*)(P.hq_block + (int64_t)b * kQBins + part * 32);
      uint4 v[8];
#pragma unroll
      for (int i = 0; i < 8; ++i) v[i] = row[i];
      uint32_t used = 0;
#pragma unroll
      for (int i = 0; i < 8; ++i) {
        const uint32_t h[4] = {v[i].x, v[i].y, v[i].z, v[i].w};
#pragma unroll
        for (int j = 0; j < 4; ++j) {
          re += (double)h[j] * t[part * 32 + i * 4 + j];
          n += h[j];
          used |= (h[j] != 0u ? 1u : 0u) << (i * 4 + j);
        }
      }
      if (used) atomicOr(&qm[part], used);
    }
    re += __shfl_xor(re, 1);
    re += __shfl_xor(re, 2);
    n += __shfl_xor(n, 1);
    n += __shfl_xor(n, 2);
    if (b < nb && part == 0) {
      sre[b] = re;
      scn[b] = n;
    }
  }
  __syncthreads();
  if (tid < 4 && P.qmask) P.qmask[tid] = qm[tid];
  {
    const double v0 = tid < nb ? sre[tid] : 0.0;
    const int64_t c0 = tid < nb ? scn[tid] : 0;
    double v = v0;
    int64_t c = c0;
    for (int off = 1; off < 64; off <<= 1) {
      const double x = __shfl_up(v, off);
      const int64_t y = __shfl_up(c, off);
      if (lane >= off) {
        v += x;
        c += y;
      }
    }
    if (lane == 63) {
      wsum[wave] = v;
      wcnt[wave] = c;
    }
    __syncthreads();
    double base = 0.0;
    for (int w = 0; w < wave; ++w) base += wsum[w];
    if (tid < nb) pre[tid] = base + (v - v0);
  }
  double total_n = 0.0;
  for (int w = 0; w < 16; ++w) total_n += (double)wcnt[w];
  const double delta = (total_n + 64.0) * 0x1p-52 + 1e-12;
  __syncthreads();
  for (int b0 = 0; b0 < nb; b0 += 256) {
    const int b = b0 + (tid >> 2), part = tid & 3;
    const bool live = b < nb && scn[min(b, nb - 1)] > 0;
    const double R0 = b < nb ? pre[b] : 0.0, R1 = b < nb ? pre[b] + sre[b] : 0.0;
    const double lo = R0 * (1.0 - delta), hi = R1 * (1.0 + delta);
    bool cand = live && (lo < kFoldSeqLimit * (1.0 + delta) || expo(lo) != expo(hi));
    const int e = (live && !cand) ? expo(lo) : 0;
    double inc = 0.0;
    bool tie = false;
    if (live && !cand) {
      const uint32_t* row = P.hq_block + (int64_t)b * kQBins + part * 32;
      for (int i = 0; i < 32; ++i) {
        const uint32_t h = row[i];
        bool tq;
        const double d = fold_inc(t[part * 32 + i], e, &tq);
        if (h) {
          inc += (double)h * d;
          tie |= tq;
        }
      }
    }
    inc += __shfl_xor(inc, 1);
    inc += __shfl_xor(inc, 2);
    tie |= __shfl_xor((int)tie, 1) != 0;
    tie |= __shfl_xor((int)tie, 2) != 0;
    if (live && !cand && (tie || !(inc < 0x1p52))) cand = true;
    if (b < nb && part == 0) {
      cnd[b] = cand;
      if (!live) P.blk[b] = FoldBlock{R0, R1, 0.0, kFoldNoBase, -1};
      else if (!cand) P.blk[b] = FoldBlock{R0, R1, inc, e, -1};
      else P.blk[b] = FoldBlock{R0, R1, 0.0, 0, 0};
    }
  }
  __syncthreads();
  const int cand = tid < nb ? cnd[tid] : 0;
  const uint64_t m = __builtin_amdgcn_ballot_w64(cand != 0);
  if (lane == 0) wc[wave] = __popcll(m);
  __syncthreads();
  int cb = 0, ctot = 0;
  for (int w = 0; w < 16; ++w) {
    if (w < wave) cb += wc[w];
    ctot += wc[w];
  }
  if (cand) {
    const int ci = cb + __popcll(m & ((1ull << lane) - 1ull));
    P.cand_list[ci] = tid;
    P.blk[tid].cidx = ci;
  }
  if (tid == 0) {
    *P.n_cand = ctot;
    *P.delta = delta;
    *P.stream_used = 0ull;
    *P.seg_used = 0u;
  }
  __shared__ unsigned long long rsum[kMaxFoldBlocks];
  __shared__ int32_t rkey[kMaxFoldBlocks], rlen[kMaxFoldBlocks];
  __syncthreads();
  const bool blive = tid < nb;
  FoldBlock mine{};
  if (blive) mine = P.blk[tid];
  const int key = !blive ? INT32_MIN : (mine.cidx >= 0 ? INT32_MIN + 1 : (mine.e == kFoldNoBase ? INT32_MIN + 2 : mine.e));
  rkey[tid] = key;
  rsum[tid] = 0ull;
  rlen[tid] = 0;
  __syncthreads();
  const bool evfree = blive && mine.cidx < 0 && mine.e != kFoldNoBase;
  const bool rstart = evfree && (tid == 0 || rkey[tid - 1] != key);
  int f = rstart ? tid : -1;
  for (int off = 1; off < 64; off <<= 1) {
    const int x = __shfl_up(f, off);
    if (lane >= off) f = max(f, x);
  }
  if (lane == 63) wc[wave] = f;
  __syncthreads();
  for (int w = 0; w < wave; ++w) f = max(f, wc[w]);
  if (evfree) {
    atomicAdd(&rsum[f], (unsigned long long)mine.inc);
    atomicAdd(&rlen[f], 1);
  }
  __syncthreads();
  if (rstart) P.blk[tid] = FoldBlock{mine.r0, mine.r1, (double)rsum[tid], mine.e, -rlen[tid]};
}

constexpr int kFtWaves = 4, kFtCopies = 8, kFtStride = kQBins + 1;
extern "C" __global__ void __launch_bounds__(kFtWaves * 64) bqsr_fold_tiles(FoldParams P, int64_t max_tpb) {
  __shared__ double t[kQBins];
  __shared__ uint32_t hist[kFtWaves][kFtCopies * kFtStride];
  __shared__ uint32_t bm[kFtWaves][kTileSlots / 32];
  for (int q = threadIdx.x; q < kQBins; q += blockDim.x) t[q] = P.pow10[q];
  __syncthreads();
  const int lane = threadIdx.x & 63, wv = threadIdx.x >> 6;
  const ReadsDev& rd = P.rd;
  const int64_t nt = rd.n_tiles;
  const int64_t total = (int64_t)(*P.n_cand) * max_tpb;
  uint32_t* hw = &hist[wv][(lane & (kFtCopies - 1)) * kFtStride];
  for (int64_t v = (int64_t)blockIdx.x * kFtWaves + wv; v < total; v += (int64_t)gridDim.x * kFtWaves) {
    const int64_t b = P.cand_list[v / max_tpb];
    const int64_t tl = nt * b / P.n_blocks + v % max_tpb;
    if (tl >= nt * (b + 1) / P.n_blocks) continue;
    const int64_t r0 = tl * (int64_t)rd.reads_per_tile;
    const int nr = (int)min((int64_t)rd.reads_per_tile, rd.n_reads - r0);
    ReadMeta m{0, 0, 0, 0, 0};
    ReadInfo inf{0, 0, 0, 0};
    if (lane < nr) {
      m = rd.meta[r0 + lane];
      inf = resolve_info(rd, info_load(P.info + r0 + lane), m.slot, m.lq);
    }
    const uint64_t ts0 = __shfl(m.slot, 0);
    const int nslots = (int)(__shfl(m.slot + max(m.lq, m.ls), nr - 1) - ts0);
    for (int i = lane; i < kTileSlots / 32; i += 64) bm[wv][i] = 0;
    for (int i = lane; i < kFtCopies * kFtStride; i += 64) hist[wv][i] = 0;
    wave_sync();
    if (lane < nr && (inf.fl & kInfoObs) && inf.en > inf.st) {
      int lo = (int)(m.slot - ts0) + inf.st;
      const int hi = (int)(m.slot - ts0) + inf.en;
      while (lo < hi) {
        const int n = min(32 - (lo & 31), hi - lo);
        atomicOr(&bm[wv][lo >> 5], (n == 32 ? 0xFFFFFFFFu : ((1u << n) - 1u)) << (lo & 31));
        lo += n;
      }
    }
    wave_sync();
    const uint8_t* qt = rd.qual + ts0;
    constexpr int kSteps = kTileSlots / (64 * 16);
    uint4 qv[kSteps];
#pragma unroll
    for (int i = 0; i < kSteps; ++i) {
      const int s0 = 16 * (lane + 64 * i);
      qv[i] = s0 < nslots ? *(const uint4*)(qt + s0) : make_uint4(0, 0, 0, 0);
    }
#pragma unroll
    for (int i = 0; i < kSteps; ++i) {
      const int s0 = 16 * (lane + 64 * i);
      if (s0 >= nslots) continue;
      const uint32_t bits = (bm[wv][s0 >> 5] >> (s0 & 31)) & 0xFFFFu;
      const uint32_t w[4] = {qv[i].x, qv[i].y, qv[i].z, qv[i].w};
#pragma unroll
      for (int k = 0; k < 16; ++k)
        if (((bits >> k) & 1u) && s0 + k < nslots) atomicAdd(&hw[(w[k >> 2] >> (8 * (k & 3))) & 0x7Fu], 1u);
    }
    wave_sync();
    double re = 0.0;
    uint32_t cnt = 0, h2[2];
#pragma unroll
    for (int i = 0; i < 2; ++i) {
      const int q = lane + 64 * i;
      uint32_t h = 0;
#pragma unroll
      for (int c = 0; c < kFtCopies; ++c) h += hist[wv][c * kFtStride + q];
      h2[i] = h;
      re += (double)h * t[q];
      cnt += h;
    }
    for (int off = 32; off > 0; off >>= 1) {
      re += __shfl_xor(re, off);
      cnt += __shfl_xor(cnt, off);
    }
    if (lane == 0) {
      P.rtile[tl] = re;
      P.ntile[tl] = (int32_t)cnt;
    }
    const FoldBlock B = P.blk[b];
    const int eb0 = block_eb0(B, *P.delta), nbin = block_nbin(B, *P.delta);
    for (int k = 0; k < nbin; ++k) {
      double d = 0.0;
      bool tie = false;
#pragma unroll
      for (int i = 0; i < 2; ++i) {
        bool tq;
        const double iq = fold_inc(t[lane + 64 * i], eb0 + k, &tq);
        d += (double)h2[i] * iq;
        tie |= h2[i] != 0 && tq;
      }
      for (int off = 32; off > 0; off >>= 1) d += __shfl_xor(d, off);
      const bool anytie = __builtin_amdgcn_ballot_w64(tie) != 0;
      if (lane == 0) P.dtile[tl * kSegBinades + k] = anytie ? kFoldTie : (d < 0x1p52 ? d : kFoldUnknown);
    }
    wave_sync();
  }
}


__device__ void fold_copy_tile(const FoldParams& P, int64_t tl, uint8_t* dst, int lane) {
  const ReadsDev& rd = P.rd;
  const int64_t r0 = tl * (int64_t)rd.reads_per_tile;
  const int nr = (int)min((int64_t)rd.reads_per_tile, rd.n_reads - r0);
  int len = 0;
  uint64_t src = 0;
  if (lane < nr) {
    const ReadMeta m = rd.meta[r0 + lane];
    const ReadInfo inf = resolve_info(rd, info_load(P.info + r0 + lane), m.slot, m.lq);
    if ((inf.fl & kInfoObs) && inf.en > inf.st) {
      len = inf.en - inf.st;
      src = m.slot + inf.st;
    }
  }
  int pre = len;
  for (int off = 1; off < 64; off <<= 1) {
    const int x = __shfl_up(pre, off);
    if (lane >= off) pre += x;
  }
  uint8_t* __restrict__ d = dst + (pre - len);
  const uint8_t* __restrict__ sp = rd.qual + src;
  const int full = len & ~15;
#pragma unroll 4
  for (int i = 0; i < full; i += 16) *(uint4*)(d + i) = *(const uint4*)(sp + i);
  for (int i = full; i < len; ++i) d[i] = sp[i];
}

extern "C" __global__ void __launch_bounds__(kSegThreads) bqsr_fold_segs(FoldParams P) {
  const int c = blockIdx.x;
  if (c >= *P.n_cand) return;
  __shared__ double t[kQBins];
  __shared__ double wsum[kSegWaves];
  __shared__ int32_t wcount[kSegWaves], wev[kSegWaves];
  __shared__ int32_t keys[kSegThreads];
  __shared__ unsigned long long s_inc[kFoldMaxSegs];
  __shared__ int32_t s_n[kFoldMaxSegs], s_t0[kFoldMaxSegs], s_t1[kFoldMaxSegs], s_key[kFoldMaxSegs];
  __shared__ int32_t s_e0[kFoldMaxSegs], s_epos0[kFoldMaxSegs];
  __shared__ int64_t s_off[kFoldMaxSegs];
  __shared__ int32_t carry_sid, chunk_sid0;
  __shared__ double carry_r;
  __shared__ int32_t ev_tile[kSegThreads];
  __shared__ int64_t ev_dst[kSegThreads];
  __shared__ int32_t seg0;
  const int tid = threadIdx.x, lane = tid & 63, wave = tid >> 6;
  for (int q = tid; q < kQBins; q += kSegThreads) t[q] = P.pow10[q];
  const int b = P.cand_list[c];
  const FoldBlock B = P.blk[b];
  const double delta = *P.delta;
  const int eb0 = block_eb0(B, delta), nbin = block_nbin(B, delta);
  const int64_t nt = P.rd.n_tiles;
  const int64_t c0 = nt * b / P.n_blocks, c1 = nt * (b + 1) / P.n_blocks;
  constexpr int kEvent = INT32_MIN + 1;
  constexpr int kLast = kFoldMaxSegs - 1;
  if (tid < kFoldMaxSegs) {
    s_inc[tid] = 0;
    s_n[tid] = 0;
    s_t0[tid] = INT32_MAX;
    s_t1[tid] = -1;
    s_key[tid] = kEvent;
    s_off[tid] = -1;
  }
  if (tid == 0) {
    carry_sid = -1;
    carry_r = B.r0;
  }
  __syncthreads();
  for (int64_t k0 = c0; k0 < c1; k0 += kSegThreads) {
    const int64_t tl = k0 + tid;
    const bool live = tl < c1;
    const double re = live ? P.rtile[tl] : 0.0;
    const int32_t cnt = live ? P.ntile[tl] : 0;
    double v = re;
    for (int off = 1; off < 64; off <<= 1) {
      const double x = __shfl_up(v, off);
      if (lane >= off) v += x;
    }
    if (lane == 63) wsum[wave] = v;
    __syncthreads();
    double base = carry_r;
    for (int w = 0; w < wave; ++w) base += wsum[w];
    const double Rt = base + (v - re), Re = base + v;
    int key = kEvent;
    int64_t inc = 0;
    if (live) {
      const double lo = Rt * (1.0 - delta), hi = Re * (1.0 + delta);
      const int e = expo(lo), k = e - eb0;
      if (lo >= kFoldSeqLimit * (1.0 + delta) && e == expo(hi) && k >= 0 && k < nbin) {
        const double d = P.dtile[tl * kSegBinades + k];
        if (d >= 0.0) {
          key = e;
          inc = (int64_t)d;
        }
      }
    }
    keys[tid] = live ? key : INT32_MIN;
    __syncthreads();
    const int prev = tid > 0 ? keys[tid - 1] : INT32_MIN;
    const bool start = live && key != prev;
    const bool ev = live && key == kEvent;
    const uint64_t sm = __builtin_amdgcn_ballot_w64(start);
    int ecnt = ev ? cnt : 0;
    for (int off = 1; off < 64; off <<= 1) {
      const int x = __shfl_up(ecnt, off);
      if (lane >= off) ecnt += x;
    }
    if (lane == 0) wcount[wave] = __popcll(sm);
    if (lane == 63) wev[wave] = ecnt;
    __syncthreads();
    int sid = carry_sid, ebase = 0;
    for (int w = 0; w < wave; ++w) {
      sid += wcount[w];
      ebase += wev[w];
    }
    sid += __popcll(sm & ((2ull << lane) - 1ull));
    const int epos = ebase + ecnt - (ev ? cnt : 0);
    if (tid == 0) chunk_sid0 = carry_sid + 1;
    if (live) {
      const int s = min(sid, kLast);
      atomicMin(&s_t0[s], (int32_t)tl);
      atomicMax(&s_t1[s], (int32_t)tl);
      if (sid >= kLast) {
        s_key[kLast] = INT32_MAX;
      } else {
        if (start) {
          s_key[s] = key;
          s_epos0[s] = epos;
          s_e0[s] = expo(fmax(Rt * (1.0 - delta), kFoldSeqLimit));
        }
        if (ev) atomicAdd(&s_n[s], cnt);
        else atomicAdd(&s_inc[s], (unsigned long long)inc);
      }
    }
    const int last = (int)(min(c1, k0 + kSegThreads) - k0) - 1;
    __syncthreads();
    if (tid == last) carry_sid = sid;
    __syncthreads();
    const int s_lo = chunk_sid0, s_hi = min(carry_sid, kLast - 1);
    if (tid <= s_hi - s_lo) {
      const int s = s_lo + tid;
      if (s_key[s] == kEvent) {
        const unsigned long long need = ((unsigned long long)s_n[s] + 63ull) & ~63ull;
        const unsigned long long o = atomicAdd(P.stream_used, need);
        s_off[s] = (o + need <= (unsigned long long)P.stream_cap) ? (int64_t)o : -1;
      }
    }
    __syncthreads();
    const bool cp = ev && sid < kLast && s_off[min(sid, kLast)] >= 0;
    const uint64_t cm = __builtin_amdgcn_ballot_w64(cp);
    if (lane == 0) wcount[wave] = __popcll(cm);
    __syncthreads();
    int cb = 0, ctot = 0;
    for (int w = 0; w < kSegWaves; ++w) {
      if (w < wave) cb += wcount[w];
      ctot += wcount[w];
    }
    if (cp) {
      const int i = cb + __popcll(cm & ((1ull << lane) - 1ull));
      ev_tile[i] = (int32_t)tl;
      ev_dst[i] = s_off[sid] + (epos - s_epos0[sid]);
    }
    __syncthreads();
    for (int k = wave; k < ctot; k += kSegWaves) fold_copy_tile(P, ev_tile[k], P.streams + ev_dst[k], lane);
    __syncthreads();
    int64_t tot = 0;
    for (int s = s_lo; s <= s_hi; ++s)
      if (s_key[s] == kEvent && s_off[s] >= 0) tot += (s_n[s] + 63) / 64;
    for (int64_t f = tid; f < tot; f += kSegThreads) {
      int s = s_lo;
      int64_t j = f;
      for (; s <= s_hi; ++s) {
        if (!(s_key[s] == kEvent && s_off[s] >= 0)) continue;
        const int64_t nch = (s_n[s] + 63) / 64;
        if (j < nch) break;
        j -= nch;
      }
      const int64_t o = s_off[s] + 64 * j;
      const int m = (int)min((int64_t)64, (int64_t)s_n[s] - 64 * j);
      const int e0 = s_e0[s];
      uint4 w4[4];
#pragma unroll
      for (int i = 0; i < 4; ++i) w4[i] = *(const uint4*)(P.streams + o + 16 * i);
      double d0 = 0.0, d1 = 0.0;
      bool t0 = false, t1 = false;
#pragma unroll
      for (int i = 0; i < 64; ++i) {
        const uint4 v4 = w4[i >> 4];
        const uint32_t word = ((i >> 2) & 3) == 0 ? v4.x : ((i >> 2) & 3) == 1 ? v4.y : ((i >> 2) & 3) == 2 ? v4.z : v4.w;
        const int q = (int)((word >> (8 * (i & 3))) & 0x7Fu);
        bool a0, a1;
        const double i0 = fold_inc(t[q], e0, &a0), i1 = fold_inc(t[q], e0 + 1, &a1);
        if (i < m) {
          d0 += i0;
          d1 += i1;
          t0 |= a0;
          t1 |= a1;
        }
      }
      P.csum[(o / 64) * 2] = t0 ? kFoldTie : (d0 < 0x1p52 ? d0 : kFoldUnknown);
      P.csum[(o / 64) * 2 + 1] = t1 ? kFoldTie : (d1 < 0x1p52 ? d1 : kFoldUnknown);
    }
    if (tid == last) carry_r = Re;
    __syncthreads();
  }
  const int ns = min(carry_sid + 1, kFoldMaxSegs);
  if (tid == 0) {
    seg0 = (int32_t)atomicAdd(P.seg_used, (uint32_t)ns);
    P.seg_base[c] = seg0;
    P.nseg[c] = ns;
  }
  __syncthreads();
  if (tid < ns) {
    FoldSeg g;
    g.t0 = s_t0[tid];
    g.t1 = s_t1[tid];
    g.e = 0;
    g.off = 0;
    const int key = s_key[tid];
    if (key == INT32_MAX) {
      g.kind = kSegGlobal;
      g.inc = 0;
    } else if (key == kEvent) {
      g.inc = s_n[tid];
      g.off = s_off[tid];
      g.e = s_e0[tid];
      g.kind = g.off >= 0 ? kSegEvent : kSegGlobal;
    } else {
      g.kind = kSegRun;
      g.e = key;
      g.inc = (int64_t)s_inc[tid];
    }
    P.seg[seg0 + tid] = g;
  }
}


template <int kCtrl, int kRowMask = 0xF>
__device__ __forceinline__ double dpp_f64(double x) {
  const uint64_t b = (uint64_t)__double_as_longlong(x);
  const uint32_t lo = (uint32_t)__builtin_amdgcn_update_dpp(0, (int)(uint32_t)b, kCtrl, kRowMask, 0xF, false);
  const uint32_t hi = (uint32_t)__builtin_amdgcn_update_dpp(0, (int)(uint32_t)(b >> 32), kCtrl, kRowMask, 0xF, false);
  return __longlong_as_double((long long)(((uint64_t)hi << 32) | lo));
}
__device__ __forceinline__ double wave_incl_scan(double x) {
  x += dpp_f64<0x111>(x);
  x += dpp_f64<0x112>(x);
  x += dpp_f64<0x114>(x);
  x += dpp_f64<0x118>(x);
  x += dpp_f64<0x142, 0xA>(x);
  x += dpp_f64<0x143, 0xC>(x);
  return x;
}
__device__ __forceinline__ double wave_shr1(double x) { return dpp_f64<0x138>(x); }
__device__ __forceinline__ double readlane_f64(double x, int l) {
  const uint64_t b = (uint64_t)__double_as_longlong(x);
  const uint32_t lo = __builtin_amdgcn_readlane((uint32_t)b, l), hi = __builtin_amdgcn_readlane((uint32_t)(b >> 32), l);
  return __longlong_as_double((long long)(((uint64_t)hi << 32) | lo));
}

#define FPF(i, v) (void)0
#define LDS __attribute__((address_space(3)))
__device__ __noinline__ double wave_fold(double S, const LDS uint8_t* q, int n, const LDS double* cs, int e0,
                                         const LDS double* t, LDS double* inc, LDS int* cur_ep, int lane) {
  int cur_e = *cur_ep;
  int pos = 0;
  while (pos < n) {
    if (S < kFoldSeqLimit) {
      const int k = pos + lane;
      const double x = k < n ? t[q[k] & 0x7F] : 0.0;
      const int m = min(64, n - pos);
      int j = 0;
      for (; j < m && S < kFoldSeqLimit; ++j) S = S + readlane_f64(x, j);
      pos += j;
      FPF(0, j);
      FPF(1, clock64() - c0);
      continue;
    }
    const int e = expo(S);
    if (e != cur_e) {
      FPF(6, 1);
      for (int k = lane; k < kQBins; k += 64) {
        bool tq;
        const double d = fold_inc(t[k], e, &tq);
        inc[k] = tq ? -1.0 : d;
      }
      cur_e = e;
      wave_sync();
    }
    const double N0 = S * pow2i(52 - e);
    const double head = kTwo53 - N0;
    int g0 = pos;
    int gn = 64;
    double excl = 0.0;
    bool element_step = false;
    if ((pos & 63) != 0) {
      gn = 64 - (pos & 63);
      element_step = true;
    } else {
      double sum = 0.0;
      bool bad = false;
      const int a = pos + 64 * lane;
      if (cs && (e == e0 || e == e0 + 1)) {
        if (a < n) {
          const double d = cs[(a >> 6) * 2 + (e - e0)];
          bad = d < 0.0;
          sum = bad ? 0.0 : d;
        }
        FPF(7, 1);
      } else if (a < n) {
        double s4[4] = {0.0, 0.0, 0.0, 0.0};
#pragma unroll
        for (int i0 = 0; i0 < 64; i0 += 16) {
          int qq[16];
#pragma unroll
          for (int j = 0; j < 16; ++j) qq[j] = q[a + i0 + j];
#pragma unroll
          for (int j = 0; j < 16; ++j) {
            const double d = inc[qq[j] & 0x7F];
            const bool ok = a + i0 + j < n;
            bad |= ok && d < 0.0;
            s4[j & 3] += ok ? fmax(d, 0.0) : 0.0;
          }
        }
        sum = (s4[0] + s4[1]) + (s4[2] + s4[3]);
      }
      const double incl = wave_incl_scan(sum);
      const uint64_t hit = __builtin_amdgcn_ballot_w64(a < n && (incl >= head || bad));
      if (!hit) {
        S = (N0 + readlane_f64(incl, 63)) * pow2i(e - 52);
        pos = min(n, pos + 64 * 64);
        FPF(2, 1);
        FPF(3, clock64() - c0);
        continue;
      }
      const int L = (int)__builtin_ctzll(hit);
      excl = L > 0 ? readlane_f64(incl, L - 1) : 0.0;
      g0 = pos + 64 * L;
      element_step = true;
    }
    if (element_step) {
      const int k = g0 + lane;
      const bool valid = lane < gn && k < n;
      const int qk = (int)q[k] & 0x7F;
      const double d = inc[qk];
      const bool tk = valid && d < 0.0;
      const double v = valid ? fmax(d, 0.0) : 0.0;
      const double sc = wave_incl_scan(v);
      const double scx = wave_shr1(sc);
      const uint64_t evm = __builtin_amdgcn_ballot_w64(valid && (tk || excl + sc >= head));
      if (!evm) {
        S = (N0 + excl + readlane_f64(sc, 63)) * pow2i(e - 52);
        pos = min(n, g0 + gn);
        FPF(5, clock64() - c0);
        continue;
      }
      const int j = (int)__builtin_ctzll(evm);
      const double before = N0 + excl + readlane_f64(scx, j);
      S = before * pow2i(e - 52) + t[__builtin_amdgcn_readlane((uint32_t)qk, j)];
      pos = g0 + j + 1;
      FPF(4, 1);
      FPF(5, clock64() - c0);
    }
  }
  *cur_ep = cur_e;
  return S;
}

__device__ __noinline__ double fold_tile_global(const FoldParams& P, double S, int64_t tl, LDS uint8_t* scratch,
                                                const LDS double* t, LDS double* inc, LDS int* cur_e, int lane) {
  const ReadsDev& rd = P.rd;
  const int64_t r0 = tl * (int64_t)rd.reads_per_tile;
  const int nr = (int)min((int64_t)rd.reads_per_tile, rd.n_reads - r0);
  int len = 0;
  if (lane < nr) {
    const ReadMeta m = rd.meta[r0 + lane];
    const ReadInfo inf = resolve_info(rd, info_load(P.info + r0 + lane), m.slot, m.lq);
    if ((inf.fl & kInfoObs) && inf.en > inf.st) len = inf.en - inf.st;
  }
  int tot = len;
  for (int off = 32; off > 0; off >>= 1) tot += __shfl_xor(tot, off);
  fold_copy_tile(P, tl, (uint8_t*)scratch, lane);
  wave_sync();
  S = wave_fold(S, scratch, tot, nullptr, 0, t, inc, cur_e, lane);
  wave_sync();
  return S;
}

extern "C" __global__ void __launch_bounds__(1024) bqsr_fold_chain(FoldParams P) {
  extern __shared__ __align__(16) unsigned char chain_smem[];
  __shared__ double t[kQBins];
  __shared__ double inc[kQBins];
  __shared__ __align__(16) uint8_t scratch[kTileSlots + 64];
  __shared__ int32_t nseg_l[kMaxFoldBlocks], sbase_l[kMaxFoldBlocks];
  const int tid = threadIdx.x, lane = tid & 63;
  const int nb = P.n_blocks, nc = *P.n_cand;
  uint8_t* streams = chain_smem;
  double* csum = (double*)(chain_smem + kChainLdsStream + 64);
  FoldSeg* segs = (FoldSeg*)(csum + kChainLdsStream / 64 * 2);
  FoldBlock* blk = (FoldBlock*)(segs + kChainLdsSegs);
  const int64_t used = (int64_t)*P.stream_used;
  const int64_t sl = min(used, (int64_t)kChainLdsStream);
  const int nsl = min((int)*P.seg_used, kChainLdsSegs);
  typedef const __attribute__((address_space(1))) uint64_t* G64;
  typedef const __attribute__((address_space(1))) double* GF64;
  typedef const __attribute__((address_space(1))) int32_t* G32;
  for (int q = tid; q < kQBins; q += 1024) t[q] = ((GF64)P.pow10)[q];
  for (int i = tid; i < nc; i += 1024) {
    nseg_l[i] = ((G32)P.nseg)[i];
    sbase_l[i] = ((G32)P.seg_base)[i];
  }
  {
    const G64 src = (G64)P.blk;
    uint64_t* dst = (uint64_t*)blk;
    const int nw = nb * (int)(sizeof(FoldBlock) / 8);
    for (int i = tid; i < nw; i += 1024) dst[i] = src[i];
    const G64 ss = (G64)P.seg;
    uint64_t* sd = (uint64_t*)segs;
    const int sw = nsl * (int)(sizeof(FoldSeg) / 8);
    for (int i = tid; i < sw; i += 1024) sd[i] = ss[i];
    const G64 s8 = (G64)P.streams;
    uint64_t* d8 = (uint64_t*)streams;
    const int64_t n16 = (sl + 15) / 16;
#pragma unroll 4
    for (int64_t i = tid; i < n16; i += 1024) {
      const uint64_t a = s8[2 * i], b = s8[2 * i + 1];
      d8[2 * i] = a;
      d8[2 * i + 1] = b;
    }
    const int64_t nc2 = sl / 64 * 2;
    const GF64 cs = (GF64)P.csum;
#pragma unroll 2
    for (int64_t i = tid; i < nc2; i += 1024) csum[i] = cs[i];
  }
  __syncthreads();
  if (tid >= 64) return;
  double S = 0.0;
  __shared__ int cur_e_s;
  if (lane == 0) cur_e_s = INT32_MIN;
  wave_sync();
  LDS int* cur_e = (LDS int*)&cur_e_s;
  const LDS uint8_t* lstreams = (const LDS uint8_t*)streams;
  const LDS double* lcsum = (const LDS double*)csum;
  const LDS double* lt = (const LDS double*)t;
  LDS double* linc = (LDS double*)inc;
  LDS uint8_t* lscratch = (LDS uint8_t*)scratch;
  const int64_t nt = P.rd.n_tiles;
#define PF(x)
  for (int b = 0; b < nb; ++b) {
    const FoldBlock B = blk[b];
    if (B.cidx < 0) {
      if (B.e == kFoldNoBase) continue;
      const int nrun = -B.cidx;
      if (S >= kFoldSeqLimit && expo(S) == B.e) {
        const double N0 = S * pow2i(52 - B.e);
        if (N0 + B.inc < kTwo53) {
          S = (N0 + B.inc) * pow2i(B.e - 52);
          b += nrun - 1;
          PF(++pf_blk; pf_nc += clock64() - bt0);
          continue;
        }
      }
      PF(++pf_blk_fb);
      for (int64_t tl = nt * b / nb; tl < nt * (b + nrun) / nb; ++tl)
        S = fold_tile_global(P, S, tl, lscratch, lt, linc, cur_e, lane);
      b += nrun - 1;
      continue;
    }
    const int c = B.cidx;
    const int ns = nseg_l[c];
    for (int s = 0; s < ns; ++s) {
      const int64_t si = (int64_t)sbase_l[c] + s;
      FoldSeg G;
      if (si < nsl) G = segs[si];
      else G = P.seg[si];
      if (G.kind == kSegRun) {
        if (S >= kFoldSeqLimit && expo(S) == G.e) {
          const double N0 = S * pow2i(52 - G.e);
          if (N0 + (double)G.inc < kTwo53) {
            S = (N0 + (double)G.inc) * pow2i(G.e - 52);
            PF(++pf_run);
            continue;
          }
        }
        PF(++pf_run_fb);
      } else if (G.kind == kSegEvent) {
        if (G.off + G.inc <= sl) {
          S = wave_fold(S, lstreams + G.off, (int)G.inc, lcsum + G.off / 64 * 2, G.e, lt, linc, cur_e, lane);
          PF(pf_glob_tiles += clock64() - w0);
        } else {
          for (int64_t o = 0; o < G.inc; o += kTileSlots) {
            const int m = (int)min((int64_t)kTileSlots, G.inc - o);
            for (int i = lane; i < m; i += 64) scratch[i] = P.streams[G.off + o + i];
            wave_sync();
            S = wave_fold(S, lscratch, m, nullptr, 0, lt, linc, cur_e, lane);
            wave_sync();
          }
        }
        PF(++pf_ev; pf_ev_el += G.inc);
        continue;
      }
      PF(++pf_glob);
      for (int64_t tl = G.t0; tl <= G.t1; ++tl) S = fold_tile_global(P, S, tl, lscratch, lt, linc, cur_e, lane);
    }
    PF(pf_cb += clock64() - bt0);
  }
  if (lane == 0) P.em_out[0] = S;
}

}
```

adam_amd/csrc/bqsr_internal.h:

```cpp
#pragma once
#include <hip/hip_runtime.h>
#include <stdint.h>

#include "../../include/adam_bqsr.h"

namespace bqsr {

struct ReadMeta {
  uint64_t slot;
  uint16_t lq;
  uint16_t ls;
  uint16_t flags;
  uint16_t rg;
};
static_assert(sizeof(ReadMeta) == 16, "ReadMeta must be 16 B");

struct ReadAlign {
  int64_t start;
  uint32_t cigar_off;
  uint32_t md_off;
  int32_t contig;
  uint16_t n_cigar;
  uint16_t md_len;
};
static_assert(sizeof(ReadAlign) == 24, "ReadAlign must be 24 B");

struct alignas(8) ReadInfo {
  uint16_t st;
  uint16_t en;
  uint16_t fl;
  uint16_t pad;
};
static_assert(sizeof(ReadInfo) == 8 && alignof(ReadInfo) == 8, "ReadInfo must be one aligned 8-B word");
__device__ __forceinline__ ReadInfo info_load(const ReadInfo* p) {
  const uint64_t v = __hip_atomic_load((const uint64_t*)p, __ATOMIC_RELAXED, __HIP_MEMORY_SCOPE_WORKGROUP);
  return ReadInfo{(uint16_t)v, (uint16_t)(v >> 16), (uint16_t)(v >> 32), (uint16_t)(v >> 48)};
}
__device__ __forceinline__ void info_store(ReadInfo* p, ReadInfo x) {
  const uint64_t v = (uint64_t)x.st | ((uint64_t)x.en << 16) | ((uint64_t)x.fl << 32) | ((uint64_t)x.pad << 48);
  __hip_atomic_store((uint64_t*)p, v, __ATOMIC_RELAXED, __HIP_MEMORY_SCOPE_WORKGROUP);
}
constexpr uint16_t kInfoObs = 1;
constexpr uint16_t kInfoObsCheck = 2;
constexpr uint16_t kInfoApp = 4;
constexpr uint16_t kInfoAppCheck = 8;
constexpr uint16_t kInfoNeg = 16;
constexpr uint16_t kInfoSecond = 32;
constexpr uint16_t kInfoPass = 64;
constexpr uint16_t kInfoCycNeg = 128;
constexpr uint16_t kInfoTrim = 256;
constexpr uint16_t kInfoNoBits = 512;

constexpr uint16_t kSeqOther = 1u << 15;

constexpr uint8_t kCodeA = 0, kCodeC = 1, kCodeG = 2, kCodeT = 3, kCodeN = 4, kCodeOther = 5;

constexpr int kMaxQ = 60;
constexpr int kCtxSlots = 21;
constexpr uint32_t kCtxTab = 4096;
constexpr int kCtxTabBytes = 2 * kCtxTab * 2;
constexpr int kQBins = 128;

constexpr int kTileSlots = 4096;
constexpr int kMaxTileReads = 64;
constexpr int kMaxFoldBlocks = 1024;
constexpr int kWaves = 16;
constexpr int kBlockThreads = 64 * kWaves;
constexpr int kMkWords = kWaves * 64;
constexpr int kMaxReadLen = 4096;
constexpr int kColumnPad = 32;
constexpr int kRedSlabs = 16;

constexpr uint64_t kNoError = ~0ull;
__host__ __device__ inline uint64_t err_key(uint64_t read, uint32_t o, uint32_t rank, uint32_t code) {
  return (read << 28) | ((uint64_t)(o & 0xFFFFF) << 8) | ((uint64_t)(rank & 0xF) << 4) | (code & 0xF);
}
enum : uint32_t {
  kRankCtor = 0,
  kRankCigar = 1,
  kRankMd = 2,
  kRankSnp = 3,
  kRankCov = 4,
  kRankTable = 5
};
enum { kErrObs = 0, kErrAppPrep = 1, kErrAppKern = 2, kNExc = 3, kErrWords = 4 };
constexpr int kJobStatusWords = 16;
constexpr int kStatusSlots = 4;

struct SitesDev {
  const int64_t* pos;
  const uint64_t* off;
  const uint32_t* bucket;
  const uint64_t* bucket_off;
  const int64_t* bucket_base;
  const uint64_t* bm;
  const uint64_t* bm_off;
  const int64_t* bm_base;
  int32_t n_contigs;
  int32_t shift;
};

struct TableGeom {
  int32_t K;
  int32_t C;
  int32_t L;
  int32_t cells;
};

struct Window {
  int32_t qw;
  int32_t q_lo;
  int32_t rg_lo;
};

struct ReadsDev {
  const ReadMeta* meta;
  const ReadAlign* align;
  const uint8_t* qual;
  const uint8_t* bases;
  const uint32_t* cigar;
  const uint8_t* md;
  int64_t n_reads;
  int64_t n_slots;
  int32_t reads_per_tile;
  int64_t n_tiles;
  int32_t slots_aligned;
};
__host__ __device__ inline uint64_t slot_span(uint64_t lq, uint64_t ls) {
  const uint64_t sl = lq > ls ? lq : ls;
  return (sl + 15) & ~(uint64_t)15;
}

struct PrepParams {
  ReadsDev rd;
  SitesDev sites;
  ReadInfo* info;
  uint64_t* sbits;
  unsigned long long* err;
  uint32_t* work;
  uint32_t* n_work;
};

struct OrderDev {
  const uint32_t* perm;
  const int64_t* key_off;
  int32_t n_keys;
  int32_t n_base = 0;
  const uint64_t* kslot = nullptr;
};

struct ObserveParams {
  ReadsDev rd;
  OrderDev ord;
  ReadInfo* info;
  const uint64_t* sbits;
  TableGeom g;
  Window w;
  int64_t* touched;
  int64_t* obs;
  int64_t* mm;
  uint32_t* part;
  int32_t part_stride;
  uint32_t* hq_block;
  unsigned long long* err;
  int32_t n_blocks;
  int32_t wcells;
  int32_t lane_shift;
  int32_t orow;
  int32_t nc;
  int32_t rows_all;
};

constexpr int32_t kFoldNoBase = INT32_MIN;
constexpr int kSegBinades = 32;
constexpr double kFoldTie = -1.0, kFoldUnknown = -2.0;
constexpr int kFoldMaxSegs = 64;
enum : int32_t { kSegRun = 0, kSegEvent = 1, kSegGlobal = 2 };

struct FoldBlock {
  double r0, r1;
  double inc;
  int32_t e;
  int32_t cidx;
};
static_assert(sizeof(FoldBlock) == 32, "FoldBlock is 4 words");

struct FoldSeg {
  int64_t inc;
  int32_t t0, t1;
  int32_t e;
  int32_t kind;
  int64_t off;
};
static_assert(sizeof(FoldSeg) == 32, "FoldSeg is 4 words");

struct FoldParams {
  ReadsDev rd;
  const ReadInfo* info;
  const uint32_t* hq_block;
  const double* pow10;
  int32_t n_blocks;
  FoldBlock* blk;
  int32_t* cand_list;
  int32_t* n_cand;
  double* delta;
  double* rtile;
  int32_t* ntile;
  double* dtile;
  FoldSeg* seg;
  int32_t* seg_base;
  int32_t* nseg;
  uint32_t* seg_used;
  uint8_t* streams;
  double* csum;
  int64_t stream_cap;
  unsigned long long* stream_used;
  double* em_out;
  uint32_t* qmask;
};

constexpr int kQbElo = -48;
constexpr int kQbEhi = 3;
constexpr int kQbBits = 5;
constexpr int kQbN = (kQbEhi - kQbElo + 1) << kQbBits;

struct ApplyParams {
  ReadsDev rd;
  OrderDev ord;
  const ReadInfo* info;
  TableGeom g;
  Window w;
  int32_t n_rg;
  const double* s1;
  const double* d2;
  const uint8_t* rq_ok;
  const uint8_t* key_ok;
  const uint8_t* grp_ok;
  int32_t n_groups;
  const double* thr;
  int32_t thr_qmin;
  int32_t thr_n;
  const double* qb_thr;
  const int16_t* qb_q;
  uint8_t* out_qual;
  uint32_t* out_start;
  uint32_t* out_len;
  unsigned long long* exc;
  int64_t max_exc;
  unsigned long long* n_exc;
  unsigned long long* err;
  int32_t lane_shift;
  int32_t outs_apart;
  const uint8_t* chars;
  int64_t piece_stride;
  uint32_t* rowbad;
  const uint32_t* qmask;
};

struct FinalOut {
  int64_t g_obs, g_mm;
  double avg, global_error;
  int32_t any_key;
  int32_t pad;
};
static_assert(kErrWords + 1 + sizeof(FinalOut) / 8 <= (size_t)kJobStatusWords, "job status words overflow");
static_assert(sizeof(FinalOut) % 8 == 0, "FinalOut is whole words");

constexpr int kThrQmin = -3100;
constexpr int kThrQmax = 3300;
constexpr int kThrN = kThrQmax - kThrQmin + 1;

}
```

include/adam_bqsr.h:

```cpp
#ifndef ADAM_BQSR_H
#define ADAM_BQSR_H

#include <stddef.h>
#include <stdint.h>

#ifdef __cplusplus
extern "C" {
#endif

#define BQSR_ABI_VERSION 1

typedef enum bqsr_status {
  BQSR_OK = 0,
  BQSR_ERR_NULL_RG = 1,
  BQSR_ERR_MD_PARSE = 2,
  BQSR_ERR_CIGAR_SHORT = 3,
  BQSR_ERR_BAD_REVCOMP_BASE = 4,
  BQSR_ERR_EMPTY_TABLE = 5,
  BQSR_ERR_MISSING_KEY = 6,
  BQSR_ERR_QUAL_RANGE = 7,
  BQSR_ERR_NULL_FIELD = 8,
  BQSR_ERR_SEQ_SHORT = 9,
  BQSR_ERR_CIGAR_INVALID = 10,
  BQSR_ERR_INVALID_ARG = 11,
  BQSR_ERR_DEVICE = 12,
  BQSR_ERR_UNSUPPORTED = 13,
  BQSR_ERR_SAM_PARSE = 14,
  BQSR_ERR_PILEUP = 15,
  BQSR_ERR_ATTRIBUTE = 16
} bqsr_status;

enum {
  BQSR_F_PAIRED = 1u << 0,
  BQSR_F_MAPPED = 1u << 1,
  BQSR_F_NEG_STRAND = 1u << 2,
  BQSR_F_SECOND_OF_PAIR = 1u << 3,
  BQSR_F_PRIMARY = 1u << 4,
  BQSR_F_DUPLICATE = 1u << 5,
  BQSR_F_HAS_RG = 1u << 8,
  BQSR_F_HAS_MD = 1u << 9,
  BQSR_F_HAS_QUAL = 1u << 10,
  BQSR_F_HAS_SEQ = 1u << 11,
  BQSR_F_HAS_CIGAR = 1u << 12,
  BQSR_F_HAS_START = 1u << 13,
  BQSR_F_HAS_REFNAME = 1u << 14
};

enum { BQSR_CIGAR_M = 0, BQSR_CIGAR_I = 1, BQSR_CIGAR_D = 2, BQSR_CIGAR_N = 3, BQSR_CIGAR_S = 4,
       BQSR_CIGAR_H = 5, BQSR_CIGAR_P = 6, BQSR_CIGAR_EQ = 7, BQSR_CIGAR_X = 8 };

#define BQSR_CONTIG_UNKNOWN (-1)

typedef struct bqsr_records {
  int64_t n_reads;
  const uint32_t* flags;
  const int32_t* rg_id;
  const int32_t* contig_id;
  const int64_t* start;
  const uint64_t* seq_offset;
  const uint8_t* seq;
  const uint64_t* qual_offset;
  const uint8_t* qual;
  const uint64_t* cigar_offset;
  const uint32_t* cigar;
  const uint64_t* md_offset;
  const uint8_t* md;
} bqsr_records;

typedef struct bqsr_dims {
  int32_t n_rg;
  int32_t max_len;
} bqsr_dims;

typedef struct bqsr_context bqsr_context;
typedef struct bqsr_sites bqsr_sites;
typedef struct bqsr_batch bqsr_batch;
typedef struct bqsr_table bqsr_table;
typedef struct bqsr_lut bqsr_lut;

int bqsr_abi_version(void);
const char* bqsr_last_error(void);
int64_t bqsr_last_error_read(void);
const char* bqsr_status_name(bqsr_status s);

bqsr_status bqsr_context_create(int device, bqsr_context** out);
void bqsr_context_destroy(bqsr_context* ctx);

enum {
  BQSR_TUNE_ORDER = 1,
  BQSR_TUNE_FRONTS = 2,
  BQSR_TUNE_KEYMAJOR = 3,
  BQSR_TUNE_FUSED_PREP = 4,
  BQSR_TUNE_BGZF = 5,
  BQSR_TUNE_FLAGSTAT_GRID = 6,
  BQSR_TUNE_PILEUP_GRID = 7
};
bqsr_status bqsr_context_tune(bqsr_context* ctx, int knob, int64_t value);

bqsr_status bqsr_sites_create(bqsr_context* ctx, const char* const* contigs, const int64_t* const* pos,
                              const uint64_t* n, int32_t n_contigs, bqsr_sites** out);
void bqsr_sites_destroy(bqsr_sites* s);

bqsr_status bqsr_batch_create(bqsr_context* ctx, const bqsr_records* recs, void* stream, bqsr_batch** out);
void bqsr_batch_destroy(bqsr_batch* b);
int64_t bqsr_batch_reads(const bqsr_batch* b);
int64_t bqsr_batch_bases(const bqsr_batch* b);
bqsr_dims bqsr_batch_dims(const bqsr_batch* b);
bqsr_status bqsr_batch_relayout(bqsr_batch* b, void* stream, double* ms);
bqsr_status bqsr_batch_layout_times(const bqsr_batch* b, double* alloc_ms, double* build_ms);

typedef struct bqsr_device_reads {
  int64_t n_reads;
  int64_t n_slots;
  const void* meta;
  const void* align;
  const uint8_t* qual;
  const uint8_t* bases;
  const uint32_t* cigar;
  const uint8_t* md;
  bqsr_dims dims;
  int32_t slots_aligned;
} bqsr_device_reads;
bqsr_status bqsr_batch_wrap_device(bqsr_context* ctx, const bqsr_device_reads* dev, bqsr_batch** out);

typedef struct bqsr_staged bqsr_staged;
bqsr_status bqsr_stage_records(bqsr_context* ctx, const bqsr_records* recs, bqsr_staged** out);
void bqsr_staged_destroy(bqsr_staged* s);
int64_t bqsr_staged_bytes(const bqsr_staged* s);
int64_t bqsr_staged_reads(const bqsr_staged* s);
int64_t bqsr_staged_bases(const bqsr_staged* s);
bqsr_status bqsr_batch_create_staged(bqsr_context* ctx, const bqsr_staged* s, bqsr_batch** out);
bqsr_status bqsr_batch_upload_async(bqsr_batch* b, const bqsr_staged* s, void* stream);

int64_t bqsr_table_words(bqsr_dims d);
bqsr_status bqsr_table_create(bqsr_context* ctx, bqsr_dims d, void* device_words, bqsr_table** out);
void bqsr_table_destroy(bqsr_table* t);
bqsr_dims bqsr_table_dims(const bqsr_table* t);
void* bqsr_table_device_ptr(bqsr_table* t);
bqsr_status bqsr_table_download(const bqsr_table* t, int64_t* host_words);
bqsr_status bqsr_table_upload(bqsr_table* t, const int64_t* host_words);

bqsr_status bqsr_observe(bqsr_context* ctx, bqsr_batch* b, const bqsr_sites* sites, bqsr_table* table,
                         double* expected_mismatch, void* stream);

bqsr_status bqsr_observe_records(bqsr_context* ctx, const bqsr_records* recs, const bqsr_sites* sites,
                                 bqsr_dims dims, bqsr_table** out_partial, double* out_expected_mismatch);

bqsr_status bqsr_table_merge(bqsr_table* acc, const bqsr_table* part, double* acc_em, double part_em);

bqsr_status bqsr_finalize(bqsr_context* ctx, const bqsr_table* t, double expected_mismatch, bqsr_lut** out);
void bqsr_lut_destroy(bqsr_lut* l);
typedef struct bqsr_final_stats {
  double average_reported_error;
  double global_error;
  int64_t global_obs, global_mm;
  int32_t n_groups;
} bqsr_final_stats;
bqsr_status bqsr_lut_stats(const bqsr_lut* l, bqsr_final_stats* out);
bqsr_status bqsr_lut_shifts(const bqsr_lut* l, int32_t qual_by_rg, int32_t qual, int32_t cycle, int32_t context,
                            double shifts[4], int32_t* new_q);

bqsr_status bqsr_apply(bqsr_context* ctx, bqsr_batch* b, const bqsr_lut* l, uint8_t* out_qual,
                       uint32_t* out_start, uint32_t* out_len, uint64_t* exceptions, int64_t max_exceptions,
                       int64_t* n_exceptions, void* stream);

bqsr_status bqsr_apply_records(bqsr_context* ctx, const bqsr_records* recs, const bqsr_lut* l,
                               uint16_t* out_qual, uint32_t* out_len);

enum { BQSR_STAGE_RESET = 1, BQSR_STAGE_KERNEL = 2, BQSR_STAGE_FOLD = 4, BQSR_STAGE_PREP = 8,
       BQSR_STAGE_LUT = 16, BQSR_STAGE_NO_LUT = 32 };
bqsr_status bqsr_observe_stage(bqsr_context* ctx, bqsr_batch* b, const bqsr_sites* sites, bqsr_table* t,
                               int32_t stages, void* stream);
bqsr_status bqsr_observe_async(bqsr_context* ctx, bqsr_batch* b, const bqsr_sites* sites, bqsr_table* t,
                               void* stream);
bqsr_status bqsr_observe_result(bqsr_batch* b, double* expected_mismatch, void* stream);
void* bqsr_batch_em_device_ptr(bqsr_batch* b);
bqsr_status bqsr_table_zero_async(bqsr_table* t, void* stream);
bqsr_status bqsr_finalize_async(bqsr_context* ctx, const bqsr_table* t, double expected_mismatch, bqsr_lut** out,
                                void* stream);
bqsr_status bqsr_finalize_result(bqsr_lut* l, void* stream);
bqsr_status bqsr_finalize_device(bqsr_context* ctx, const bqsr_table* t, const double* em_device, bqsr_lut** out,
                                 void* stream);
bqsr_status bqsr_batch_em_copy_async(bqsr_batch* b, double* dst_device, void* stream);
bqsr_status bqsr_em_fold_async(bqsr_context* ctx, const double* ems_device, int64_t n, double* out_device,
                               void* stream);
bqsr_status bqsr_apply_stage(bqsr_context* ctx, bqsr_batch* b, const bqsr_lut* l, uint8_t* out_qual,
                             uint32_t* out_start, uint32_t* out_len, uint64_t* exceptions, int64_t max_exceptions,
                             int32_t stages, void* stream);
bqsr_status bqsr_apply_async(bqsr_context* ctx, bqsr_batch* b, const bqsr_lut* l, uint8_t* out_qual,
                             uint32_t* out_start, uint32_t* out_len, uint64_t* exceptions, int64_t max_exceptions,
                             void* stream);
bqsr_status bqsr_apply_result(bqsr_batch* b, int64_t* n_exceptions, void* stream);

bqsr_status bqsr_batch_set_window(bqsr_batch* b, int32_t q_lo, int32_t rg_lo);
int32_t bqsr_batch_reads_per_tile(const bqsr_batch* b);
int64_t bqsr_batch_slots(const bqsr_batch* b);
int bqsr_lut_group(const bqsr_lut* l, int32_t r, int64_t* obs, int64_t* mm);
int32_t bqsr_phred_threshold_table(double* out, int32_t cap, int32_t* qmin);

bqsr_status bqsr_copy_async(bqsr_context* ctx, void* dst, const void* src, int64_t bytes, void* stream);
bqsr_status bqsr_copy_dyn_async(bqsr_context* ctx, void* dst, const void* src, const void* count, int32_t count_bytes,
                                int64_t scale, int64_t max_bytes, void* stream);
bqsr_status bqsr_compact_outputs_async(bqsr_context* ctx, bqsr_batch* b, const uint8_t* out_qual,
                                       const uint32_t* out_start, const uint32_t* out_len, uint64_t* exceptions,
                                       int64_t max_exceptions, uint8_t* chars, uint32_t* offsets, uint16_t* lengths,
                                       void* stream);
const void* bqsr_batch_exception_count_ptr(const bqsr_batch* b);

bqsr_status bqsr_job_reset_async(bqsr_batch* b, bqsr_table* t, void* stream);
bqsr_status bqsr_job_result(bqsr_batch* b, bqsr_lut* l, double* expected_mismatch, int64_t* n_exceptions,
                            void* stream);
bqsr_status bqsr_job_status_async(bqsr_batch* b, bqsr_lut* l, int32_t slot, void* stream);
bqsr_status bqsr_job_status_get(const bqsr_batch* b, int32_t slot, int32_t part, double* expected_mismatch,
                                int64_t* n_exceptions);
bqsr_status bqsr_job_errors_export_async(bqsr_batch* b, int64_t read_base, int64_t* dst_device, void* stream);
bqsr_status bqsr_job_errors_import_async(bqsr_batch* b, const int64_t* src_device, void* stream);

#ifdef __cplusplus
}
#endif
#endif
```

Before: 522.6 billion bases/s.

## Rework fold kernels: parallel tile binade sums, multi-tile seg scan, chain increment tables

Result: no change. 526.7 billion bases/s, median of 6 (+0.8%).

```diff
diff --git a/adam_amd/_capi.py b/adam_amd/_capi.py
--- a/adam_amd/_capi.py
+++ b/adam_amd/_capi.py
@@ -17,7 +17,7 @@
 
 EXPORTS = [
     "bqsr_abi_version", "bqsr_last_error", "bqsr_last_error_read", "bqsr_status_name", "bqsr_context_create",
-    "bqsr_context_destroy", "bqsr_context_tune", "bqsr_sites_create", "bqsr_sites_destroy", "bqsr_batch_create", "bqsr_batch_destroy",
+    "bqsr_context_destroy", "bqsr_context_tune", "bqsr_context_fold_stats", "bqsr_sites_create", "bqsr_sites_destroy", "bqsr_batch_create", "bqsr_batch_destroy",
     "bqsr_batch_reads", "bqsr_batch_bases", "bqsr_batch_dims", "bqsr_batch_relayout", "bqsr_batch_layout_times", "bqsr_batch_wrap_device", "bqsr_table_words",
     "bqsr_table_create", "bqsr_table_destroy", "bqsr_table_dims", "bqsr_table_device_ptr", "bqsr_table_download",
     "bqsr_table_upload", "bqsr_observe", "bqsr_observe_records", "bqsr_table_merge", "bqsr_finalize",
diff --git a/adam_amd/bqsr.py b/adam_amd/bqsr.py
--- a/adam_amd/bqsr.py
+++ b/adam_amd/bqsr.py
@@ -29,8 +29,20 @@
             cls._by_device[device] = Context(device)
         return cls._by_device[device]
 
-    _KNOBS = {"order": 1, "fronts": 2, "key_major": 3, "bgzf": 5, "flagstat_grid": 6, "pileup_grid": 7}
-    _DEFAULTS = {"order": -1, "fronts": -1, "key_major": 0, "bgzf": 1, "flagstat_grid": 0, "pileup_grid": 0}
+    _KNOBS = {"order": 1, "fronts": 2, "key_major": 3, "bgzf": 5, "flagstat_grid": 6, "pileup_grid": 7,
+              "fold_blocks": 8, "fold_limits": 9}
+    _DEFAULTS = {"order": -1, "fronts": -1, "key_major": 0, "bgzf": 1, "flagstat_grid": 0, "pileup_grid": 0,
+                 "fold_blocks": 0, "fold_limits": 0}
+    FOLD_LIMITS = {"stream": 1, "segs": 2, "lds_segs": 4, "lds_stream": 8, "tables": 16}
+    FOLD_STATS = ("tables_rebuilt", "segs_from_global", "scratch_segments", "no_room_segments", "overflow_segments",
+                  "bound_failed", "events", "carried")
+
+    def fold_stats(self) -> Dict[str, int]:
+        out = (ctypes.c_uint64 * len(self.FOLD_STATS))()
+        f = lib().bqsr_context_fold_stats
+        f.restype, f.argtypes = ctypes.c_int, [ctypes.c_void_p, ctypes.POINTER(ctypes.c_uint64)]
+        check(f(self.handle, out))
+        return dict(zip(self.FOLD_STATS, (int(v) for v in out)))
 
     def tune(self, **knobs) -> Dict[str, int]:
         cur = getattr(self, "_tuned", dict(self._DEFAULTS))
diff --git a/adam_amd/csrc/bqsr_capi.cpp b/adam_amd/csrc/bqsr_capi.cpp
--- a/adam_amd/csrc/bqsr_capi.cpp
+++ b/adam_amd/csrc/bqsr_capi.cpp
@@ -220,6 +220,9 @@
   int tune_bgzf = 1;
   int tune_flagstat_grid = 0;
   int tune_pileup_grid = 0;
+  int tune_fold_blocks = 0;
+  int tune_fold_limits = 0;
+  unsigned long long* d_fold_stats = nullptr;
   std::mutex flagstat_mu;
   unsigned long long* d_flagstat = nullptr;
 };
@@ -454,10 +457,26 @@
       if (value < 0 || value > (1 << 20)) break;
       ctx->tune_pileup_grid = (int)value;
       return BQSR_OK;
+    case BQSR_TUNE_FOLD_BLOCKS:
+      if (value < 0 || value > kMaxFoldBlocks) break;
+      ctx->tune_fold_blocks = (int)value;
+      return BQSR_OK;
+    case BQSR_TUNE_FOLD_LIMITS:
+      if (value < 0 || value > 31) break;
+      ctx->tune_fold_limits = (int)value;
+      return BQSR_OK;
     default:
       return fail(BQSR_ERR_INVALID_ARG, "bqsr_context_tune: unknown knob");
   }
   return fail(BQSR_ERR_INVALID_ARG, "bqsr_context_tune: value out of range");
+}
+
+bqsr_status bqsr_context_fold_stats(bqsr_context* ctx, uint64_t* out) {
+  if (!ctx || !out) return fail(BQSR_ERR_INVALID_ARG, "bqsr_context_fold_stats: bad arguments");
+  static_assert(kFoldStats == BQSR_FOLD_STATS, "adam_bqsr.h lists FoldParams::stats");
+  HIP_TRY(hipDeviceSynchronize());
+  HIP_TRY(hipMemcpy(out, ctx->d_fold_stats, kFoldStats * sizeof(uint64_t), hipMemcpyDeviceToHost));
+  return ok();
 }
 
 bqsr_status bqsr_context_create(int device, bqsr_context** out) {
@@ -472,6 +491,8 @@
   if (e == hipSuccess) e = hipMalloc(&c->d_thr, kThrN * sizeof(double));
   if (e == hipSuccess) e = hipMemcpy(c->d_pow10, pow10tab().v, 256 * sizeof(double), hipMemcpyHostToDevice);
   if (e == hipSuccess) e = hipMemcpy(c->d_thr, thresholds().thr.data(), kThrN * sizeof(double), hipMemcpyHostToDevice);
+  if (e == hipSuccess) e = hipMalloc(&c->d_fold_stats, kFoldStats * sizeof(unsigned long long));
+  if (e == hipSuccess) e = hipMemset(c->d_fold_stats, 0, kFoldStats * sizeof(unsigned long long));
   if (e == hipSuccess) e = hipMalloc(&c->d_qbt, kQbN * sizeof(double));
   if (e == hipSuccess) e = hipMalloc(&c->d_qbq, kQbN * sizeof(int16_t));
   if (e == hipSuccess) e = hipMemcpy(c->d_qbt, buckets().thr.data(), kQbN * sizeof(double), hipMemcpyHostToDevice);
@@ -483,7 +504,7 @@
     e = hipFuncSetAttribute((const void*)bqsr_fold_hist, hipFuncAttributeMaxDynamicSharedMemorySize, (int)fold_hist_lds());
   if (e == hipSuccess)
     e = hipFuncSetAttribute((const void*)bqsr_fold_chain, hipFuncAttributeMaxDynamicSharedMemorySize,
-                            (int)chain_lds(kMaxFoldBlocks));
+                            (int)std::min(chain_lds(kMaxFoldBlocks, kChainTabs), kLdsMax - kChainStatic));
   if (e != hipSuccess) {
     bqsr_context_destroy(c);
     return fail(BQSR_ERR_DEVICE, std::string("context: ") + hipGetErrorString(e));
@@ -499,6 +520,7 @@
   if (c->d_qbt) (void)hipFree(c->d_qbt);
   if (c->d_qbq) (void)hipFree(c->d_qbq);
   if (c->d_flagstat) (void)hipFree(c->d_flagstat);
+  if (c->d_fold_stats) (void)hipFree(c->d_fold_stats);
   for (int i = 0; i < 2; ++i) {
     if (c->stage[i]) (void)hipHostFree(c->stage[i]);
     if (c->stage_ev[i]) (void)hipEventDestroy(c->stage_ev[i]);
@@ -605,6 +627,7 @@
   b->rd.reads_per_tile = (int32_t)std::max<int64_t>(1, std::min<int64_t>(kMaxTileReads, kTileSlots / std::max<int64_t>(1, max_slot_len)));
   b->rd.n_tiles = (n + b->rd.reads_per_tile - 1) / b->rd.reads_per_tile;
   b->n_blocks = std::min(b->ctx->n_cu, kMaxFoldBlocks);
+  if (b->ctx->tune_fold_blocks > 0) b->n_blocks = std::min(b->n_blocks, b->ctx->tune_fold_blocks);
   bqsr_status st;
   if ((st = dalloc(b->allocs, &b->d_hq, (size_t)b->n_blocks * kQBins)) != BQSR_OK) return st;
   if ((st = dalloc(b->allocs, &b->d_qmask, 4)) != BQSR_OK) return st;
@@ -612,6 +635,14 @@
     FoldParams& F = b->fold;
     const size_t nt = (size_t)std::max<int64_t>(1, b->rd.n_tiles), nbk = (size_t)b->n_blocks;
     F.stream_cap = std::max<int64_t>(1 << 20, std::min<int64_t>(16 << 20, b->rd.n_slots));
+    const int64_t stream_alloc = F.stream_cap;
+    const int lim = b->ctx->tune_fold_limits;
+    if (lim & BQSR_FOLD_LIMIT_STREAM) F.stream_cap = 4096;
+    F.max_segs = (lim & BQSR_FOLD_LIMIT_SEGS) ? 3 : kFoldMaxSegs;
+    F.lds_segs = (lim & BQSR_FOLD_LIMIT_LDS_SEGS) ? 2 : kChainLdsSegs;
+    F.lds_stream = (lim & BQSR_FOLD_LIMIT_LDS_STREAM) ? 4096 : kChainLdsStream;
+    F.n_tab = std::min((lim & BQSR_FOLD_LIMIT_TABLES) ? 2 : kChainTabs, chain_tabs(b->n_blocks, kLdsMax));
+    F.stats = b->ctx->d_fold_stats;
     if ((st = dalloc(b->allocs, &F.blk, nbk)) != BQSR_OK || (st = dalloc(b->allocs, &F.cand_list, nbk)) != BQSR_OK ||
         (st = dalloc(b->allocs, &F.n_cand, 1)) != BQSR_OK || (st = dalloc(b->allocs, &F.delta, 1)) != BQSR_OK ||
         (st = dalloc(b->allocs, &F.rtile, nt)) != BQSR_OK || (st = dalloc(b->allocs, &F.ntile, nt)) != BQSR_OK ||
@@ -619,8 +650,8 @@
         (st = dalloc(b->allocs, &F.seg, nbk * kFoldMaxSegs)) != BQSR_OK ||
         (st = dalloc(b->allocs, &F.seg_base, nbk)) != BQSR_OK || (st = dalloc(b->allocs, &F.nseg, nbk)) != BQSR_OK ||
         (st = dalloc(b->allocs, &F.seg_used, 1)) != BQSR_OK ||
-        (st = dalloc(b->allocs, &F.streams, (size_t)F.stream_cap + 64)) != BQSR_OK ||
-        (st = dalloc(b->allocs, &F.csum, (size_t)F.stream_cap / 64 * 2 + 2)) != BQSR_OK ||
+        (st = dalloc(b->allocs, &F.streams, (size_t)stream_alloc + 64)) != BQSR_OK ||
+        (st = dalloc(b->allocs, &F.csum, (size_t)stream_alloc / 64 * 2 + 2)) != BQSR_OK ||
         (st = dalloc(b->allocs, &F.stream_used, 1)) != BQSR_OK)
       return st;
   }
@@ -1430,7 +1461,7 @@
     const int64_t max_tpb = (b->rd.n_tiles + b->n_blocks - 1) / b->n_blocks + 1;
     hipLaunchKernelGGL(bqsr_fold_tiles, dim3(ctx->n_cu * 4), dim3(kFtWaves * 64), 0, s, F, max_tpb);
     hipLaunchKernelGGL(bqsr_fold_segs, dim3(b->n_blocks), dim3(kSegThreads), 0, s, F);
-    hipLaunchKernelGGL(bqsr_fold_chain, dim3(1), dim3(1024), chain_lds(b->n_blocks), s, F);
+    hipLaunchKernelGGL(bqsr_fold_chain, dim3(1), dim3(1024), chain_lds(b->n_blocks, F.n_tab), s, F);
     HIP_TRY(hipGetLastError());
     b->hq_valid = true;
     if (fork) {
diff --git a/adam_amd/csrc/bqsr_fold.hip b/adam_amd/csrc/bqsr_fold.hip
--- a/adam_amd/csrc/bqsr_fold.hip
+++ b/adam_amd/csrc/bqsr_fold.hip
@@ -5,10 +5,18 @@
 constexpr double kTwo53 = 9007199254740992.0;
 constexpr int kChainLdsSegs = 384;
 constexpr int kSegThreads = 1024, kSegWaves = kSegThreads / 64;
+constexpr int kSegTpt = 2, kSegChunk = kSegThreads * kSegTpt;
 constexpr int kChainLdsStream = 80 * 1024;
-constexpr size_t chain_lds(int n_blocks) {
+constexpr int kChainTab0 = -4;
+constexpr int kChainTabs = 24;
+constexpr size_t kChainStatic = 15 * 1024;
+constexpr size_t chain_lds(int n_blocks, int n_tab) {
   return kChainLdsStream + 64 + (size_t)kChainLdsStream / 64 * 2 * sizeof(double) + (size_t)kChainLdsSegs * sizeof(FoldSeg) +
-         (size_t)n_blocks * sizeof(FoldBlock);
+         (size_t)n_blocks * sizeof(FoldBlock) + (size_t)n_tab * kQBins * sizeof(double);
+}
+inline int chain_tabs(int n_blocks, size_t lds_max) {
+  const size_t base = chain_lds(n_blocks, 0) + kChainStatic;
+  return base >= lds_max ? 0 : (int)std::min<size_t>(kChainTabs, (lds_max - base) / (kQBins * sizeof(double)));
 }
 
 __device__ __forceinline__ int expo(double x) {
@@ -188,10 +196,12 @@
 }
 
 constexpr int kFtWaves = 4, kFtCopies = 8, kFtStride = kQBins + 1;
-extern "C" __global__ void __launch_bounds__(kFtWaves * 64) bqsr_fold_tiles(FoldParams P, int64_t max_tpb) {
+extern "C" __global__ void __launch_bounds__(kFtWaves * 64) __attribute__((amdgpu_waves_per_eu(4, 4)))
+bqsr_fold_tiles(FoldParams P, int64_t max_tpb) {
   __shared__ double t[kQBins];
   __shared__ uint32_t hist[kFtWaves][kFtCopies * kFtStride];
   __shared__ uint32_t bm[kFtWaves][kTileSlots / 32];
+  __shared__ uint32_t hs[kFtWaves][kQBins];
   for (int q = threadIdx.x; q < kQBins; q += blockDim.x) t[q] = P.pow10[q];
   __syncthreads();
   const int lane = threadIdx.x & 63, wv = threadIdx.x >> 6;
@@ -265,22 +275,32 @@
       P.rtile[tl] = re;
       P.ntile[tl] = (int32_t)cnt;
     }
+    hs[wv][lane] = h2[0];
+    hs[wv][lane + 64] = h2[1];
+    wave_sync();
     const FoldBlock B = P.blk[b];
     const int eb0 = block_eb0(B, *P.delta), nbin = block_nbin(B, *P.delta);
-    for (int k = 0; k < nbin; ++k) {
-      double d = 0.0;
-      bool tie = false;
-#pragma unroll
-      for (int i = 0; i < 2; ++i) {
+    int nk = 1;
+    while (nk < nbin) nk <<= 1;
+    const int per = 2 * nk;
+    const int k = lane & (nk - 1), q0 = (lane / nk) * per;
+    double d = 0.0;
+    bool tie = false;
+    if (k < nbin) {
+      for (int i = 0; i < per; ++i) {
+        const int q = q0 + ((i + lane / nk) & (per - 1));
+        const uint32_t h = hs[wv][q];
         bool tq;
-        const double iq = fold_inc(t[lane + 64 * i], eb0 + k, &tq);
-        d += (double)h2[i] * iq;
-        tie |= h2[i] != 0 && tq;
-      }
-      for (int off = 32; off > 0; off >>= 1) d += __shfl_xor(d, off);
-      const bool anytie = __builtin_amdgcn_ballot_w64(tie) != 0;
-      if (lane == 0) P.dtile[tl * kSegBinades + k] = anytie ? kFoldTie : (d < 0x1p52 ? d : kFoldUnknown);
-    }
+        const double iq = fold_inc(t[q], eb0 + k, &tq);
+        d += (double)h * iq;
+        tie |= h != 0 && tq;
+      }
+    }
+    for (int off = nk; off < 64; off <<= 1) {
+      d += __shfl_xor(d, off);
+      tie |= __shfl_xor((int)tie, off) != 0;
+    }
+    if (lane < nbin) P.dtile[tl * kSegBinades + lane] = tie ? kFoldTie : (d < 0x1p52 ? d : kFoldUnknown);
     wave_sync();
   }
 }
@@ -319,15 +339,15 @@
   __shared__ double t[kQBins];
   __shared__ double wsum[kSegWaves];
   __shared__ int32_t wcount[kSegWaves], wev[kSegWaves];
-  __shared__ int32_t keys[kSegThreads];
+  __shared__ int32_t keys[kSegChunk];
   __shared__ unsigned long long s_inc[kFoldMaxSegs];
   __shared__ int32_t s_n[kFoldMaxSegs], s_t0[kFoldMaxSegs], s_t1[kFoldMaxSegs], s_key[kFoldMaxSegs];
   __shared__ int32_t s_e0[kFoldMaxSegs], s_epos0[kFoldMaxSegs];
   __shared__ int64_t s_off[kFoldMaxSegs];
   __shared__ int32_t carry_sid, chunk_sid0;
   __shared__ double carry_r;
-  __shared__ int32_t ev_tile[kSegThreads];
-  __shared__ int64_t ev_dst[kSegThreads];
+  __shared__ int32_t ev_tile[kSegChunk];
+  __shared__ int64_t ev_dst[kSegChunk];
   __shared__ int32_t seg0;
   const int tid = threadIdx.x, lane = tid & 63, wave = tid >> 6;
   for (int q = tid; q < kQBins; q += kSegThreads) t[q] = P.pow10[q];
@@ -338,7 +358,7 @@
   const int64_t nt = P.rd.n_tiles;
   const int64_t c0 = nt * b / P.n_blocks, c1 = nt * (b + 1) / P.n_blocks;
   constexpr int kEvent = INT32_MIN + 1;
-  constexpr int kLast = kFoldMaxSegs - 1;
+  const int kLast = P.max_segs - 1;
   if (tid < kFoldMaxSegs) {
     s_inc[tid] = 0;
     s_n[tid] = 0;
@@ -352,12 +372,25 @@
     carry_r = B.r0;
   }
   __syncthreads();
-  for (int64_t k0 = c0; k0 < c1; k0 += kSegThreads) {
-    const int64_t tl = k0 + tid;
-    const bool live = tl < c1;
-    const double re = live ? P.rtile[tl] : 0.0;
-    const int32_t cnt = live ? P.ntile[tl] : 0;
-    double v = re;
+  for (int64_t k0 = c0; k0 < c1; k0 += kSegChunk) {
+    int64_t tl[kSegTpt];
+    bool live[kSegTpt];
+    double re[kSegTpt];
+    int32_t cnt[kSegTpt];
+#pragma unroll
+    for (int u = 0; u < kSegTpt; ++u) {
+      tl[u] = k0 + (int64_t)tid * kSegTpt + u;
+      live[u] = tl[u] < c1;
+    }
+#pragma unroll
+    for (int u = 0; u < kSegTpt; ++u) {
+      re[u] = live[u] ? P.rtile[tl[u]] : 0.0;
+      cnt[u] = live[u] ? P.ntile[tl[u]] : 0;
+    }
+    double mine = 0.0;
+#pragma unroll
+    for (int u = 0; u < kSegTpt; ++u) mine += re[u];
+    double v = mine;
     for (int off = 1; off < 64; off <<= 1) {
       const double x = __shfl_up(v, off);
       if (lane >= off) v += x;
@@ -366,61 +399,93 @@
     __syncthreads();
     double base = carry_r;
     for (int w = 0; w < wave; ++w) base += wsum[w];
-    const double Rt = base + (v - re), Re = base + v;
-    int key = kEvent;
-    int64_t inc = 0;
-    if (live) {
-      const double lo = Rt * (1.0 - delta), hi = Re * (1.0 + delta);
-      const int e = expo(lo), k = e - eb0;
-      if (lo >= kFoldSeqLimit * (1.0 + delta) && e == expo(hi) && k >= 0 && k < nbin) {
-        const double d = P.dtile[tl * kSegBinades + k];
-        if (d >= 0.0) {
-          key = e;
-          inc = (int64_t)d;
-        }
-      }
-    }
-    keys[tid] = live ? key : INT32_MIN;
-    __syncthreads();
-    const int prev = tid > 0 ? keys[tid - 1] : INT32_MIN;
-    const bool start = live && key != prev;
-    const bool ev = live && key == kEvent;
-    const uint64_t sm = __builtin_amdgcn_ballot_w64(start);
-    int ecnt = ev ? cnt : 0;
+    double Rt[kSegTpt], Re[kSegTpt];
+    Rt[0] = base + (v - mine);
+#pragma unroll
+    for (int u = 0; u < kSegTpt; ++u) {
+      Re[u] = Rt[u] + re[u];
+      if (u + 1 < kSegTpt) Rt[u + 1] = Re[u];
+    }
+    int key[kSegTpt];
+    int64_t inc[kSegTpt];
+#pragma unroll
+    for (int u = 0; u < kSegTpt; ++u) {
+      key[u] = kEvent;
+      inc[u] = 0;
+      if (live[u]) {
+        const double lo = Rt[u] * (1.0 - delta), hi = Re[u] * (1.0 + delta);
+        const int e = expo(lo), k = e - eb0;
+        if (lo >= kFoldSeqLimit * (1.0 + delta) && e == expo(hi) && k >= 0 && k < nbin) {
+          const double d = P.dtile[tl[u] * kSegBinades + k];
+          if (d >= 0.0) {
+            key[u] = e;
+            inc[u] = (int64_t)d;
+          }
+        }
+      }
+      keys[tid * kSegTpt + u] = live[u] ? key[u] : INT32_MIN;
+    }
+    __syncthreads();
+    bool start[kSegTpt], ev[kSegTpt];
+    int nstart = 0, nev = 0;
+#pragma unroll
+    for (int u = 0; u < kSegTpt; ++u) {
+      const int prev = u > 0 ? (live[u - 1] ? key[u - 1] : INT32_MIN) : (tid > 0 ? keys[tid * kSegTpt - 1] : INT32_MIN);
+      start[u] = live[u] && key[u] != prev;
+      ev[u] = live[u] && key[u] == kEvent;
+      nstart += start[u] ? 1 : 0;
+      nev += ev[u] ? cnt[u] : 0;
+    }
+    int scnt = nstart, ecnt = nev;
     for (int off = 1; off < 64; off <<= 1) {
-      const int x = __shfl_up(ecnt, off);
-      if (lane >= off) ecnt += x;
-    }
-    if (lane == 0) wcount[wave] = __popcll(sm);
-    if (lane == 63) wev[wave] = ecnt;
-    __syncthreads();
-    int sid = carry_sid, ebase = 0;
+      const int x = __shfl_up(scnt, off), y = __shfl_up(ecnt, off);
+      if (lane >= off) {
+        scnt += x;
+        ecnt += y;
+      }
+    }
+    if (lane == 63) {
+      wcount[wave] = scnt;
+      wev[wave] = ecnt;
+    }
+    __syncthreads();
+    int sbase = carry_sid, ebase = 0;
     for (int w = 0; w < wave; ++w) {
-      sid += wcount[w];
+      sbase += wcount[w];
       ebase += wev[w];
     }
-    sid += __popcll(sm & ((2ull << lane) - 1ull));
-    const int epos = ebase + ecnt - (ev ? cnt : 0);
+    int sid[kSegTpt], epos[kSegTpt];
+    sbase += scnt - nstart;
+    ebase += ecnt - nev;
+#pragma unroll
+    for (int u = 0; u < kSegTpt; ++u) {
+      sbase += start[u] ? 1 : 0;
+      sid[u] = sbase;
+      epos[u] = ebase;
+      ebase += ev[u] ? cnt[u] : 0;
+    }
     if (tid == 0) chunk_sid0 = carry_sid + 1;
-    if (live) {
-      const int s = min(sid, kLast);
-      atomicMin(&s_t0[s], (int32_t)tl);
-      atomicMax(&s_t1[s], (int32_t)tl);
-      if (sid >= kLast) {
+#pragma unroll
+    for (int u = 0; u < kSegTpt; ++u) {
+      if (!live[u]) continue;
+      const int s = min(sid[u], kLast);
+      atomicMin(&s_t0[s], (int32_t)tl[u]);
+      atomicMax(&s_t1[s], (int32_t)tl[u]);
+      if (sid[u] >= kLast) {
         s_key[kLast] = INT32_MAX;
       } else {
-        if (start) {
-          s_key[s] = key;
-          s_epos0[s] = epos;
-          s_e0[s] = expo(fmax(Rt * (1.0 - delta), kFoldSeqLimit));
-        }
-        if (ev) atomicAdd(&s_n[s], cnt);
-        else atomicAdd(&s_inc[s], (unsigned long long)inc);
-      }
-    }
-    const int last = (int)(min(c1, k0 + kSegThreads) - k0) - 1;
-    __syncthreads();
-    if (tid == last) carry_sid = sid;
+        if (start[u]) {
+          s_key[s] = key[u];
+          s_epos0[s] = epos[u];
+          s_e0[s] = expo(fmax(Rt[u] * (1.0 - delta), kFoldSeqLimit));
+        }
+        if (ev[u]) atomicAdd(&s_n[s], cnt[u]);
+        else atomicAdd(&s_inc[s], (unsigned long long)inc[u]);
+      }
+    }
+    const int last = (int)(min(c1, k0 + kSegChunk) - k0) - 1;
+    __syncthreads();
+    if (tid == last / kSegTpt) carry_sid = sid[last % kSegTpt];
     __syncthreads();
     const int s_lo = chunk_sid0, s_hi = min(carry_sid, kLast - 1);
     if (tid <= s_hi - s_lo) {
@@ -432,19 +497,32 @@
       }
     }
     __syncthreads();
-    const bool cp = ev && sid < kLast && s_off[min(sid, kLast)] >= 0;
-    const uint64_t cm = __builtin_amdgcn_ballot_w64(cp);
-    if (lane == 0) wcount[wave] = __popcll(cm);
+    bool cp[kSegTpt];
+    int ncp = 0;
+#pragma unroll
+    for (int u = 0; u < kSegTpt; ++u) {
+      cp[u] = ev[u] && sid[u] < kLast && s_off[min(sid[u], kLast)] >= 0;
+      ncp += cp[u] ? 1 : 0;
+    }
+    int ccnt = ncp;
+    for (int off = 1; off < 64; off <<= 1) {
+      const int x = __shfl_up(ccnt, off);
+      if (lane >= off) ccnt += x;
+    }
+    if (lane == 63) wcount[wave] = ccnt;
     __syncthreads();
     int cb = 0, ctot = 0;
     for (int w = 0; w < kSegWaves; ++w) {
       if (w < wave) cb += wcount[w];
       ctot += wcount[w];
     }
-    if (cp) {
-      const int i = cb + __popcll(cm & ((1ull << lane) - 1ull));
-      ev_tile[i] = (int32_t)tl;
-      ev_dst[i] = s_off[sid] + (epos - s_epos0[sid]);
+    cb += ccnt - ncp;
+#pragma unroll
+    for (int u = 0; u < kSegTpt; ++u) {
+      if (!cp[u]) continue;
+      ev_tile[cb] = (int32_t)tl[u];
+      ev_dst[cb] = s_off[sid[u]] + (epos[u] - s_epos0[sid[u]]);
+      ++cb;
     }
     __syncthreads();
     for (int k = wave; k < ctot; k += kSegWaves) fold_copy_tile(P, ev_tile[k], P.streams + ev_dst[k], lane);
@@ -486,10 +564,10 @@
       P.csum[(o / 64) * 2] = t0 ? kFoldTie : (d0 < 0x1p52 ? d0 : kFoldUnknown);
       P.csum[(o / 64) * 2 + 1] = t1 ? kFoldTie : (d1 < 0x1p52 ? d1 : kFoldUnknown);
     }
-    if (tid == last) carry_r = Re;
-    __syncthreads();
-  }
-  const int ns = min(carry_sid + 1, kFoldMaxSegs);
+    if (tid == last / kSegTpt) carry_r = Re[last % kSegTpt];
+    __syncthreads();
+  }
+  const int ns = min(carry_sid + 1, kLast + 1);
   if (tid == 0) {
     seg0 = (int32_t)atomicAdd(P.seg_used, (uint32_t)ns);
     P.seg_base[c] = seg0;
@@ -506,6 +584,7 @@
     if (key == INT32_MAX) {
       g.kind = kSegGlobal;
       g.inc = 0;
+      g.off = -2;
     } else if (key == kEvent) {
       g.inc = s_n[tid];
       g.off = s_off[tid];
@@ -544,11 +623,39 @@
   return __longlong_as_double((long long)(((uint64_t)hi << 32) | lo));
 }
 
-#define FPF(i, v) (void)0
 #define LDS __attribute__((address_space(3)))
-__device__ __noinline__ double wave_fold(double S, const LDS uint8_t* q, int n, const LDS double* cs, int e0,
-                                         const LDS double* t, LDS double* inc, LDS int* cur_ep, int lane) {
-  int cur_e = *cur_ep;
+struct ChainCtx {
+  const LDS double* t;
+  const LDS double* tabs;
+  int n_tab;
+  LDS double* inc;
+  LDS int* cur_e;
+  LDS int* cnt;
+};
+__device__ __forceinline__ void chain_count(const ChainCtx& C, int i, int lane) {
+  if (lane == 0) __hip_atomic_fetch_add(C.cnt + i, 1, __ATOMIC_RELAXED, __HIP_MEMORY_SCOPE_WORKGROUP);
+}
+__device__ __forceinline__ double fold_inc_entry(double t, int e) {
+  bool tq;
+  const double d = fold_inc(t, e, &tq);
+  return tq ? -1.0 : d;
+}
+__device__ __forceinline__ bool chain_has_tab(const ChainCtx& C, int e) { return (unsigned)(e - kChainTab0) < (unsigned)C.n_tab; }
+__device__ __forceinline__ const LDS double* chain_tab(const ChainCtx& C, int e, int lane) {
+  if (chain_has_tab(C, e)) return C.tabs + (e - kChainTab0) * kQBins;
+  if (*C.cur_e != e) {
+    wave_sync();
+    for (int k = lane; k < kQBins; k += 64) C.inc[k] = fold_inc_entry(C.t[k], e);
+    if (lane == 0) *C.cur_e = e;
+    chain_count(C, kFsTabRebuilt, lane);
+    wave_sync();
+  }
+  return C.inc;
+}
+
+__device__ __noinline__ double wave_fold(double S, const LDS uint8_t* q, int n, const LDS double* cs, int e0, const ChainCtx C,
+                                         int lane) {
+  const LDS double* t = C.t;
   int pos = 0;
   while (pos < n) {
     if (S < kFoldSeqLimit) {
@@ -556,43 +663,52 @@
       const double x = k < n ? t[q[k] & 0x7F] : 0.0;
       const int m = min(64, n - pos);
       int j = 0;
+      if (m == 64) {
+#pragma unroll
+        for (int g = 0; g < 8; ++g) {
+          if (j == 8 * g && S < kFoldSeqLimit) {
+#pragma unroll
+            for (int i = 0; i < 8; ++i) S = S + readlane_f64(x, 8 * g + i);
+            j += 8;
+          }
+        }
+      }
       for (; j < m && S < kFoldSeqLimit; ++j) S = S + readlane_f64(x, j);
       pos += j;
-      FPF(0, j);
-      FPF(1, clock64() - c0);
       continue;
     }
     const int e = expo(S);
-    if (e != cur_e) {
-      FPF(6, 1);
-      for (int k = lane; k < kQBins; k += 64) {
-        bool tq;
-        const double d = fold_inc(t[k], e, &tq);
-        inc[k] = tq ? -1.0 : d;
-      }
-      cur_e = e;
-      wave_sync();
-    }
+    const LDS double* inc = chain_tab(C, e, lane);
+    const bool have1 = chain_has_tab(C, e + 1);
+    const LDS double* inc1 = C.tabs + (have1 ? e + 1 - kChainTab0 : 0) * kQBins;
     const double N0 = S * pow2i(52 - e);
     const double head = kTwo53 - N0;
     int g0 = pos;
     int gn = 64;
     double excl = 0.0;
     bool element_step = false;
+    bool wnext = false;
+    double wrest = 0.0;
+    int wend = 0;
     if ((pos & 63) != 0) {
       gn = 64 - (pos & 63);
       element_step = true;
     } else {
-      double sum = 0.0;
-      bool bad = false;
+      double sum = 0.0, sum1 = 0.0;
+      bool bad = false, bad1 = false;
       const int a = pos + 64 * lane;
+      const bool two = cs && e == e0 && have1;
       if (cs && (e == e0 || e == e0 + 1)) {
         if (a < n) {
           const double d = cs[(a >> 6) * 2 + (e - e0)];
           bad = d < 0.0;
           sum = bad ? 0.0 : d;
-        }
-        FPF(7, 1);
+          if (two) {
+            const double d1 = cs[(a >> 6) * 2 + 1];
+            bad1 = d1 < 0.0;
+            sum1 = bad1 ? 0.0 : d1;
+          }
+        }
       } else if (a < n) {
         double s4[4] = {0.0, 0.0, 0.0, 0.0};
 #pragma unroll
@@ -611,49 +727,81 @@
         sum = (s4[0] + s4[1]) + (s4[2] + s4[3]);
       }
       const double incl = wave_incl_scan(sum);
+      const double incl1 = two ? wave_incl_scan(sum1) : 0.0;
       const uint64_t hit = __builtin_amdgcn_ballot_w64(a < n && (incl >= head || bad));
       if (!hit) {
         S = (N0 + readlane_f64(incl, 63)) * pow2i(e - 52);
         pos = min(n, pos + 64 * 64);
-        FPF(2, 1);
-        FPF(3, clock64() - c0);
         continue;
       }
       const int L = (int)__builtin_ctzll(hit);
       excl = L > 0 ? readlane_f64(incl, L - 1) : 0.0;
       g0 = pos + 64 * L;
       element_step = true;
+      if (two) {
+        const uint64_t after = ~((2ull << L) - 1ull);
+        const uint64_t b1 = __builtin_amdgcn_ballot_w64(a < n && bad1) & after;
+        const double tot1 = readlane_f64(incl1, 63);
+        wnext = b1 == 0ull && tot1 < 0x1p52;
+        wrest = tot1 - readlane_f64(incl1, L);
+        wend = min(n, pos + 64 * 64);
+      }
     }
     if (element_step) {
       const int k = g0 + lane;
       const bool valid = lane < gn && k < n;
       const int qk = (int)q[k] & 0x7F;
       const double d = inc[qk];
+      const double d1 = have1 ? inc1[qk] : 0.0;
       const bool tk = valid && d < 0.0;
       const double v = valid ? fmax(d, 0.0) : 0.0;
+      const double v1 = valid ? fmax(d1, 0.0) : 0.0;
       const double sc = wave_incl_scan(v);
+      const double sc1 = have1 ? wave_incl_scan(v1) : 0.0;
       const double scx = wave_shr1(sc);
       const uint64_t evm = __builtin_amdgcn_ballot_w64(valid && (tk || excl + sc >= head));
       if (!evm) {
         S = (N0 + excl + readlane_f64(sc, 63)) * pow2i(e - 52);
         pos = min(n, g0 + gn);
-        FPF(5, clock64() - c0);
         continue;
       }
       const int j = (int)__builtin_ctzll(evm);
       const double before = N0 + excl + readlane_f64(scx, j);
       S = before * pow2i(e - 52) + t[__builtin_amdgcn_readlane((uint32_t)qk, j)];
       pos = g0 + j + 1;
-      FPF(4, 1);
-      FPF(5, clock64() - c0);
-    }
-  }
-  *cur_ep = cur_e;
+      chain_count(C, kFsEvents, lane);
+      if (have1 && expo(S) == e + 1) {
+        const int gend = min(n, g0 + gn);
+        bool done = pos == gend;
+        if (!done) {
+          const uint64_t after = ~((2ull << j) - 1ull);
+          const uint64_t tie1 = __builtin_amdgcn_ballot_w64(valid && d1 < 0.0) & after;
+          const double tot1 = readlane_f64(sc1, 63);
+          const double rest = tot1 - readlane_f64(sc1, j);
+          const double N1 = S * pow2i(51 - e);
+          if (tie1 == 0ull && tot1 < 0x1p52 && N1 + rest < kTwo53) {
+            S = (N1 + rest) * pow2i(e - 51);
+            pos = gend;
+            done = true;
+            chain_count(C, kFsCarried, lane);
+          }
+        }
+        if (done && wnext) {
+          const double N1 = S * pow2i(51 - e);
+          if (N1 + wrest < kTwo53) {
+            S = (N1 + wrest) * pow2i(e - 51);
+            pos = wend;
+            chain_count(C, kFsCarried, lane);
+          }
+        }
+      }
+    }
+  }
   return S;
 }
 
-__device__ __noinline__ double fold_tile_global(const FoldParams& P, double S, int64_t tl, LDS uint8_t* scratch,
-                                                const LDS double* t, LDS double* inc, LDS int* cur_e, int lane) {
+__device__ __noinline__ double fold_tile_global(const FoldParams& P, double S, int64_t tl, LDS uint8_t* scratch, const ChainCtx C,
+                                                int lane) {
   const ReadsDev& rd = P.rd;
   const int64_t r0 = tl * (int64_t)rd.reads_per_tile;
   const int nr = (int)min((int64_t)rd.reads_per_tile, rd.n_reads - r0);
@@ -667,7 +815,7 @@
   for (int off = 32; off > 0; off >>= 1) tot += __shfl_xor(tot, off);
   fold_copy_tile(P, tl, (uint8_t*)scratch, lane);
   wave_sync();
-  S = wave_fold(S, scratch, tot, nullptr, 0, t, inc, cur_e, lane);
+  S = wave_fold(S, scratch, tot, nullptr, 0, C, lane);
   wave_sync();
   return S;
 }
@@ -684,9 +832,10 @@
   double* csum = (double*)(chain_smem + kChainLdsStream + 64);
   FoldSeg* segs = (FoldSeg*)(csum + kChainLdsStream / 64 * 2);
   FoldBlock* blk = (FoldBlock*)(segs + kChainLdsSegs);
+  double* tabs = (double*)(blk + nb);
   const int64_t used = (int64_t)*P.stream_used;
-  const int64_t sl = min(used, (int64_t)kChainLdsStream);
-  const int nsl = min((int)*P.seg_used, kChainLdsSegs);
+  const int64_t sl = min(used, (int64_t)P.lds_stream);
+  const int nsl = min((int)*P.seg_used, P.lds_segs);
   typedef const __attribute__((address_space(1))) uint64_t* G64;
   typedef const __attribute__((address_space(1))) double* GF64;
   typedef const __attribute__((address_space(1))) int32_t* G32;
@@ -717,21 +866,27 @@
     const GF64 cs = (GF64)P.csum;
 #pragma unroll 2
     for (int64_t i = tid; i < nc2; i += 1024) csum[i] = cs[i];
-  }
+    for (int i = tid; i < P.n_tab * kQBins; i += 1024)
+      tabs[i] = fold_inc_entry(((GF64)P.pow10)[i & (kQBins - 1)], kChainTab0 + i / kQBins);
+  }
+  __shared__ int cur_e_s, cnt_s[kFoldStats];
+  if (tid == 0) cur_e_s = INT32_MIN;
+  if (tid < kFoldStats) cnt_s[tid] = 0;
   __syncthreads();
   if (tid >= 64) return;
   double S = 0.0;
-  __shared__ int cur_e_s;
-  if (lane == 0) cur_e_s = INT32_MIN;
-  wave_sync();
-  LDS int* cur_e = (LDS int*)&cur_e_s;
+  ChainCtx C;
+  C.t = (const LDS double*)t;
+  C.tabs = (const LDS double*)tabs;
+  C.n_tab = P.n_tab;
+  C.inc = (LDS double*)inc;
+  C.cur_e = (LDS int*)&cur_e_s;
+  C.cnt = (LDS int*)cnt_s;
+  int st_seg_global = 0, st_scratch = 0, st_no_room = 0, st_overflow = 0, st_bound = 0;
   const LDS uint8_t* lstreams = (const LDS uint8_t*)streams;
   const LDS double* lcsum = (const LDS double*)csum;
-  const LDS double* lt = (const LDS double*)t;
-  LDS double* linc = (LDS double*)inc;
   LDS uint8_t* lscratch = (LDS uint8_t*)scratch;
   const int64_t nt = P.rd.n_tiles;
-#define PF(x)
   for (int b = 0; b < nb; ++b) {
     const FoldBlock B = blk[b];
     if (B.cidx < 0) {
@@ -742,13 +897,12 @@
         if (N0 + B.inc < kTwo53) {
           S = (N0 + B.inc) * pow2i(B.e - 52);
           b += nrun - 1;
-          PF(++pf_blk; pf_nc += clock64() - bt0);
           continue;
         }
       }
-      PF(++pf_blk_fb);
+      ++st_bound;
       for (int64_t tl = nt * b / nb; tl < nt * (b + nrun) / nb; ++tl)
-        S = fold_tile_global(P, S, tl, lscratch, lt, linc, cur_e, lane);
+        S = fold_tile_global(P, S, tl, lscratch, C, lane);
       b += nrun - 1;
       continue;
     }
@@ -757,40 +911,51 @@
     for (int s = 0; s < ns; ++s) {
       const int64_t si = (int64_t)sbase_l[c] + s;
       FoldSeg G;
-      if (si < nsl) G = segs[si];
-      else G = P.seg[si];
+      if (si < nsl) {
+        G = segs[si];
+      } else {
+        G = P.seg[si];
+        ++st_seg_global;
+      }
       if (G.kind == kSegRun) {
         if (S >= kFoldSeqLimit && expo(S) == G.e) {
           const double N0 = S * pow2i(52 - G.e);
           if (N0 + (double)G.inc < kTwo53) {
             S = (N0 + (double)G.inc) * pow2i(G.e - 52);
-            PF(++pf_run);
             continue;
           }
         }
-        PF(++pf_run_fb);
+        ++st_bound;
       } else if (G.kind == kSegEvent) {
         if (G.off + G.inc <= sl) {
-          S = wave_fold(S, lstreams + G.off, (int)G.inc, lcsum + G.off / 64 * 2, G.e, lt, linc, cur_e, lane);
-          PF(pf_glob_tiles += clock64() - w0);
+          S = wave_fold(S, lstreams + G.off, (int)G.inc, lcsum + G.off / 64 * 2, G.e, C, lane);
         } else {
+          ++st_scratch;
           for (int64_t o = 0; o < G.inc; o += kTileSlots) {
             const int m = (int)min((int64_t)kTileSlots, G.inc - o);
             for (int i = lane; i < m; i += 64) scratch[i] = P.streams[G.off + o + i];
             wave_sync();
-            S = wave_fold(S, lscratch, m, nullptr, 0, lt, linc, cur_e, lane);
+            S = wave_fold(S, lscratch, m, nullptr, 0, C, lane);
             wave_sync();
           }
         }
-        PF(++pf_ev; pf_ev_el += G.inc);
         continue;
-      }
-      PF(++pf_glob);
-      for (int64_t tl = G.t0; tl <= G.t1; ++tl) S = fold_tile_global(P, S, tl, lscratch, lt, linc, cur_e, lane);
-    }
-    PF(pf_cb += clock64() - bt0);
+      } else if (G.off == -2) {
+        ++st_overflow;
+      } else {
+        ++st_no_room;
+      }
+      for (int64_t tl = G.t0; tl <= G.t1; ++tl) S = fold_tile_global(P, S, tl, lscratch, C, lane);
+    }
   }
   if (lane == 0) P.em_out[0] = S;
-}
-
-}
+  if (lane < kFoldStats && P.stats) {
+    const int v[kFoldStats] = {0, st_seg_global, st_scratch, st_no_room, st_overflow, st_bound, 0, 0};
+    int mine = cnt_s[lane];
+#pragma unroll
+    for (int i = 0; i < kFoldStats; ++i) mine += lane == i ? v[i] : 0;
+    P.stats[lane] = (unsigned long long)mine;
+  }
+}
+
+}
diff --git a/adam_amd/csrc/bqsr_internal.h b/adam_amd/csrc/bqsr_internal.h
--- a/adam_amd/csrc/bqsr_internal.h
+++ b/adam_amd/csrc/bqsr_internal.h
@@ -217,6 +217,22 @@
   unsigned long long* stream_used;
   double* em_out;
   uint32_t* qmask;
+  int32_t max_segs;
+  int32_t lds_segs;
+  int32_t lds_stream;
+  int32_t n_tab;
+  unsigned long long* stats;
+};
+enum : int {
+  kFsTabRebuilt = 0,
+  kFsSegGlobal = 1,
+  kFsScratch = 2,
+  kFsNoRoom = 3,
+  kFsOverflow = 4,
+  kFsBoundFailed = 5,
+  kFsEvents = 6,
+  kFsCarried = 7,
+  kFoldStats = 8
 };
 
 constexpr int kQbElo = -48;
diff --git a/include/adam_bqsr.h b/include/adam_bqsr.h
--- a/include/adam_bqsr.h
+++ b/include/adam_bqsr.h
@@ -93,9 +93,21 @@
   BQSR_TUNE_FUSED_PREP = 4,
   BQSR_TUNE_BGZF = 5,
   BQSR_TUNE_FLAGSTAT_GRID = 6,
-  BQSR_TUNE_PILEUP_GRID = 7
+  BQSR_TUNE_PILEUP_GRID = 7,
+  BQSR_TUNE_FOLD_BLOCKS = 8,
+  BQSR_TUNE_FOLD_LIMITS = 9
+};
+enum {
+  BQSR_FOLD_LIMIT_STREAM = 1,
+  BQSR_FOLD_LIMIT_SEGS = 2,
+  BQSR_FOLD_LIMIT_LDS_SEGS = 4,
+  BQSR_FOLD_LIMIT_LDS_STREAM = 8,
+  BQSR_FOLD_LIMIT_TABLES = 16
 };
 bqsr_status bqsr_context_tune(bqsr_context* ctx, int knob, int64_t value);
+
+#define BQSR_FOLD_STATS 8
+bqsr_status bqsr_context_fold_stats(bqsr_context* ctx, uint64_t* out);
 
 bqsr_status bqsr_sites_create(bqsr_context* ctx, const char* const* contigs, const int64_t* const* pos,
                               const uint64_t* n, int32_t n_contigs, bqsr_sites** out);
```
